# Bismarrck/tensoralloy

Measured on AMD Instinct MI355X. Metric: atom-steps/sec (energy+forces), 4000-atom Ni rcut=6.5 A, higher is better.
Workload: dtype f64

## Files before the change

include/tensoralloy_amd.h:

```cpp
#ifndef TENSORALLOY_AMD_H
#define TENSORALLOY_AMD_H

#include <stddef.h>
#include <stdint.h>

#ifdef __cplusplus
extern "C" {
#endif

typedef struct ta_context *ta_handle;

enum {
  TA_OK = 0,
  TA_ERR_INVALID = -1,
  TA_ERR_UNSUPPORTED = -2,
  TA_ERR_HIP = -3,
  TA_ERR_NOMEM = -4
};

enum {
  TA_WANT_ENERGY = 1,
  TA_WANT_FORCES = 2,
  TA_WANT_VIRIAL = 4,
  TA_WANT_ATOMIC = 8,
// ... 18 lines not shown
  int32_t angular;
  int32_t cutoff_function;

  int32_t n_eta, n_omega, n_beta, n_gamma, n_zeta;
  const double *eta, *omega, *beta, *gamma, *zeta;

  int32_t activation;
  int32_t use_resnet_dt;
  int32_t minmax_scale;
  const int32_t *n_layers;
  const int32_t *layer_sizes;
  const double *weights;
  const double *xlo, *xhi;

  int32_t n_eam_params;
  const double *eam_params;

  double eps;

  int32_t n_grap_params;
  const double *grap_params;

  int32_t n_eam_nets;

  const int32_t *eam_table_n;
  const double *eam_table_dx;
  const double *eam_table_coef;

  int32_t safe_pow;

  int32_t finite_temperature;
} ta_model_desc;

enum { TA_TD_ON = 1, TA_TD_SOMMERFELD = 2, TA_TD_ACT_SHIFT = 8 };

typedef struct {
  int32_t n_atoms;
  const int32_t *species;
  const double *positions;
  const double *cell;
  const int32_t *pbc;
} ta_frame;

typedef struct {
  int32_t n_frames;
  int64_t n_atoms;
  int64_t n_pairs;
  int64_t n_triples;
  int32_t nnl_max;
  int32_t descriptor_dim;
  int32_t nl_on_device;
  int32_t reserved_;
  double nl_ms;
  double set_frames_ms;
} ta_batch_info;

#define TA_N_KERNEL_SLOTS 10
enum {
  TA_K_PAIR_GEOMETRY = 0, TA_K_G4_FORWARD = 1, TA_K_DESCRIPTOR_REDUCE = 2,
  TA_K_MLP = 3, TA_K_BACKWARD = 4, TA_K_FORCE_GATHER = 5, TA_K_FRAME_REDUCE = 6,
  TA_K_EAM = 7,
  TA_K_NEIGHBOR_UPDATE = 8,
  TA_K_GRAP = 9
};

int ta_device_count(void);

#define TA_ABI_VERSION 5
int ta_abi_version(void);
int ta_model_desc_size(void);

int ta_create(const ta_model_desc *model, int device, ta_handle *out);
int ta_destroy(ta_handle h);
const char *ta_last_error(ta_handle h);

int ta_set_frames(ta_handle h, int32_t n_frames, const ta_frame *frames,
                  ta_batch_info *info);

int ta_set_skin(ta_handle h, double skin);
int ta_update_positions(ta_handle h, const double *positions, const double *cells, int32_t *rebuilt);
int ta_list_stats(ta_handle h, int64_t *n_builds, int64_t *n_reuses);
int ta_list_sizes(ta_handle h, int64_t *n_pairs, int64_t *n_triples, int32_t *nnl_max);

int ta_compute(ta_handle h, uint32_t want);

int ta_get_results(ta_handle h, double *energy, double *forces, double *virial,
                   double *atomic, double *descriptors);

int ta_set_electron_temperatures(ta_handle h, int32_t n_frames, const double *T);
int ta_get_td_results(ta_handle h, double *energy, double *eentropy, double *energy_atomic,
                      double *eentropy_atomic);

int ta_eval(ta_handle h, int32_t n_frames, const ta_frame *frames, uint32_t want,
            double *energy, double *forces, double *virial, double *atomic);

int ta_step(ta_handle h, const double *positions, const double *cells, uint32_t want, double *energy,
            double *forces, double *virial, double *atomic, int32_t *rebuilt);

int ta_view_results(ta_handle h, uint32_t want, const double **energy, const double **forces,
                    const double **virial, const double **atomic);
int ta_step_view(ta_handle h, const double *positions, const double *cells, uint32_t want, const double **energy,
                 const double **forces, const double **virial, const double **atomic, int32_t *rebuilt);

int ta_set_stream(ta_handle h, void *stream);

int ta_synchronize(ta_handle h);

int ta_batch_energy_device_ptr(ta_handle h, void **dptr);

int ta_copy_batch_energy(ta_handle h, void *dst_device);
int ta_set_batch_energy_target(ta_handle h, void *dst_device);

int ta_neighbor_list(const ta_frame *frame, int32_t n_elements, double rc, int64_t *n_pairs,
                     int32_t **i, int32_t **j, int32_t **shift , int32_t **rev);
void ta_free(void *p);


int ta_param_count(ta_handle h, int64_t *n_params);

int ta_update_weights(ta_handle h, const double *weights, int64_t n_weights);

int ta_energy_gradient(ta_handle h, const double *frame_coeff, double *grad, int64_t n_grad);

int ta_loss_gradient(ta_handle h, const double *frame_coeff, const double *dR, const double *dh,
                     double *grad, int64_t n_grad, double *dG_out);

int ta_td_loss_gradient(ta_handle h, const double *coeff_free_energy, const double *coeff_energy,
                        const double *coeff_eentropy, const double *dR, const double *dh, double *grad,
                        int64_t n_grad, double *dG_out);

int ta_constant_count(ta_handle h, int64_t *n_constants);
int ta_get_constants(ta_handle h, double *constants, int64_t n_constants);
int ta_update_constants(ta_handle h, const double *constants, int64_t n_constants);
int ta_constant_gradient(ta_handle h, const double *frame_coeff, const double *dR, const double *dh,
                         double *grad, int64_t n_grad);

int ta_hessian_vectors(ta_handle h, int32_t n_dir, int32_t first, const double *dR, const double *dh, double *dF,
                       double *dW);

int ta_set_nn_tables(ta_handle h, int on);

int ta_eam_tabulate(ta_handle h, int32_t n_r, const double *r, int32_t n_rho, const double *rho,
                    double *rho_of_r, double *phi_of_r, double *embed_of_rho, double *u_of_r,
                    double *w_of_r);


int ta_time_compute(ta_handle h, uint32_t want, int32_t warmup, int32_t steps,
                    double *total_ms, double *kernel_ms );

int ta_measure_hbm_copy(ta_handle h, int64_t bytes, int32_t reps, double *gbs);

int ta_count_contributing_triples(ta_handle h, int64_t *n_contributing);

int ta_get_pairs(ta_handle h, int32_t *i, int32_t *j, int32_t *shift );

#ifdef __cplusplus
}
#endif
#endif
```

tensoralloy_amd/_lib.py:

```python
from __future__ import annotations

import ctypes as C
import os
import subprocess
from pathlib import Path

import numpy as np

PKG_DIR = Path(__file__).resolve().parent
REPO_DIR = PKG_DIR.parent
CSRC_DIR = PKG_DIR / "csrc"
INCLUDE_DIR = REPO_DIR / "include"
LIB_PATH = PKG_DIR / "libtensoralloy_amd.so"

SOURCES = ["ta_api.hip", "ta_kernels.hip", "ta_kernels_v2.hip", "ta_mlp.hip", "ta_eam.hip",
           "ta_nlist.hip", "ta_grap.hip", "ta_train.hip", "ta_hvp.hip", "ta_neighbor.cpp", "ta_td.hip",
           "ta_td_train.hip"]
OBJ_DIR = CSRC_DIR / "build"

TA_OK = 0
TA_ERR_INVALID, TA_ERR_UNSUPPORTED, TA_ERR_HIP, TA_ERR_NOMEM = -1, -2, -3, -4
TA_WANT_ENERGY, TA_WANT_FORCES, TA_WANT_VIRIAL, TA_WANT_ATOMIC, TA_WANT_DESCRIPTORS = 1, 2, 4, 8, 16
TA_WANT_REUSE_DESCRIPTORS = 32
TA_MODEL_SF_MLP, TA_MODEL_EAM_ALLOY, TA_MODEL_EAM_ADP, TA_MODEL_GRAP_MLP, TA_MODEL_EAM_FS = 1, 2, 3, 4, 5
TA_CUTOFF = {"cosine": 0, "polynomial": 1}
TA_ACT = {"relu": 0, "softplus": 1, "tanh": 2, "squareplus": 3, "leaky_relu": 4,
          "sigmoid": 5, "softsign": 6, "elu": 7}
TA_N_KERNEL_SLOTS = 10
TA_TD_ON, TA_TD_SOMMERFELD, TA_TD_ACT_SHIFT = 1, 2, 8
TA_ABI_VERSION = 5
KERNEL_SLOTS = ["pair_geometry", "g4_forward", "descriptor_reduce", "mlp", "backward",
                "force_gather", "frame_reduce", "eam", "neighbor_update", "grap_forward"]

EXPORTED_SYMBOLS = [
    "ta_device_count", "ta_create", "ta_destroy", "ta_last_error", "ta_set_frames",
    "ta_compute", "ta_get_results", "ta_eval", "ta_set_stream", "ta_synchronize", "ta_time_compute",
    "ta_batch_energy_device_ptr", "ta_copy_batch_energy", "ta_get_pairs", "ta_neighbor_list", "ta_free",
    "ta_eam_tabulate", "ta_set_batch_energy_target", "ta_param_count", "ta_update_weights",
    "ta_energy_gradient", "ta_measure_hbm_copy", "ta_set_skin", "ta_update_positions", "ta_list_stats",
    "ta_count_contributing_triples", "ta_loss_gradient", "ta_constant_count", "ta_get_constants", "ta_update_constants",
    "ta_constant_gradient", "ta_list_sizes", "ta_abi_version", "ta_model_desc_size", "ta_set_nn_tables", "ta_step", "ta_hessian_vectors", "ta_view_results", "ta_step_view",
    "ta_set_electron_temperatures", "ta_get_td_results", "ta_td_loss_gradient",
]

_dp = C.POINTER(C.c_double)
_ip = C.POINTER(C.c_int32)


class ModelDesc(C.Structure):
    _fields_ = [
        ("kind", C.c_int32), ("n_elements", C.c_int32),
        ("rcut", C.c_double), ("acut", C.c_double),
        ("angular", C.c_int32), ("cutoff_function", C.c_int32),
        ("n_eta", C.c_int32), ("n_omega", C.c_int32), ("n_beta", C.c_int32),
        ("n_gamma", C.c_int32), ("n_zeta", C.c_int32),
        ("eta", _dp), ("omega", _dp), ("beta", _dp), ("gamma", _dp), ("zeta", _dp),
        ("activation", C.c_int32), ("use_resnet_dt", C.c_int32), ("minmax_scale", C.c_int32),
        ("n_layers", _ip), ("layer_sizes", _ip), ("weights", _dp),
        ("xlo", _dp), ("xhi", _dp),
        ("n_eam_params", C.c_int32), ("eam_params", _dp),
        ("eps", C.c_double),
        ("n_grap_params", C.c_int32), ("grap_params", _dp),
        ("n_eam_nets", C.c_int32),
        ("eam_table_n", _ip), ("eam_table_dx", _dp), ("eam_table_coef", _dp),
        ("safe_pow", C.c_int32),
        ("finite_temperature", C.c_int32),
    ]


class Frame(C.Structure):
    _fields_ = [("n_atoms", C.c_int32), ("species", _ip), ("positions", _dp),
                ("cell", _dp), ("pbc", _ip)]


class BatchInfo(C.Structure):
    _fields_ = [("n_frames", C.c_int32), ("n_atoms", C.c_int64), ("n_pairs", C.c_int64),
                ("n_triples", C.c_int64), ("nnl_max", C.c_int32), ("descriptor_dim", C.c_int32),
                ("nl_on_device", C.c_int32), ("reserved_", C.c_int32),
                ("nl_ms", C.c_double), ("set_frames_ms", C.c_double)]


def hipcc_path() -> str:
    for cand in (os.environ.get("HIPCC"), "/opt/rocm/bin/hipcc", "hipcc"):
        if cand and (os.path.isabs(cand) and os.path.exists(cand) or not os.path.isabs(cand)):
            return cand
    return "hipcc"


def _compile_flags():
    return ["--offload-arch=gfx950", "-O3", "-std=c++17", "-fPIC", "-pthread", f"-I{INCLUDE_DIR}",
            f"-I{CSRC_DIR}"] + os.environ.get("TA_EXTRA_HIPCC_FLAGS", "").split()


def build(force: bool = False, verbose: bool = False) -> Path:
    srcs = [CSRC_DIR / s for s in SOURCES]
    headers = list(CSRC_DIR.glob("*.h")) + [INCLUDE_DIR / "tensoralloy_amd.h"]
    deps = srcs + headers
    stamp = OBJ_DIR / "flags.txt"
    flags_same = stamp.exists() and stamp.read_text() == " ".join(_compile_flags())
    if not force and flags_same and LIB_PATH.exists():
        newest = max(p.stat().st_mtime for p in deps)
        if LIB_PATH.stat().st_mtime >= newest:
            return LIB_PATH
    import fcntl
    from concurrent.futures import ThreadPoolExecutor
    lock_path = str(LIB_PATH) + ".lock"
    with open(lock_path, "w") as lock:
        fcntl.flock(lock, fcntl.LOCK_EX)
        try:
            OBJ_DIR.mkdir(exist_ok=True)
            flags = _compile_flags()
            flags_same = stamp.exists() and stamp.read_text() == " ".join(flags)
            if not force and flags_same and LIB_PATH.exists() and \
                    LIB_PATH.stat().st_mtime >= max(p.stat().st_mtime for p in deps):
                return LIB_PATH
            if not flags_same:
                force = True
            hdr_time = max(p.stat().st_mtime for p in headers)

            def compile_one(src):
                obj = OBJ_DIR / (src.stem + ".o")
                if not force and obj.exists() and obj.stat().st_mtime >= max(src.stat().st_mtime, hdr_time):
                    return obj
                cmd = [hipcc_path()] + flags + ["-c", str(src), "-o", str(obj)]
                if verbose:
                    print(" ".join(cmd))
                subprocess.run(cmd, check=True)
                return obj

            try:
                jobs = max(1, min(len(srcs), len(os.sched_getaffinity(0))))
            except AttributeError:
                jobs = 4
            with ThreadPoolExecutor(max_workers=jobs) as pool:
                objs = list(pool.map(compile_one, srcs))
            stamp.write_text(" ".join(flags))
            tmp = str(LIB_PATH) + f".tmp{os.getpid()}"
            cmd = [hipcc_path(), "--offload-arch=gfx950", "-shared", "-fPIC", "-pthread"] + \
                  [str(o) for o in objs] + ["-o", tmp]
            if verbose:
                print(" ".join(cmd))
            subprocess.run(cmd, check=True)
            os.replace(tmp, LIB_PATH)
        finally:
            fcntl.flock(lock, fcntl.LOCK_UN)
    return LIB_PATH


_lib = None


def load():
    global _lib
    if _lib is not None:
        return _lib
    if not LIB_PATH.exists():
        raise ImportError(
            f"{LIB_PATH} is missing: build it with `python -c 'import __graft_entry__ as g; "
            f"g.build()'` (hipcc --offload-arch=gfx950). There is no CPU fallback.")
    path = os.environ.get("TA_LIB_AB") or str(LIB_PATH)
    if path != str(LIB_PATH):
        import sys
        sys.stderr.write(f"tensoralloy_amd: TA_LIB_AB is set, loading {path} instead of {LIB_PATH}\n")
    lib = C.CDLL(path)
    try:
        lib.ta_abi_version.restype = C.c_int
        version, desc_size = lib.ta_abi_version(), lib.ta_model_desc_size()
    except AttributeError:
        version, desc_size = -1, -1
    if version != TA_ABI_VERSION or desc_size != C.sizeof(ModelDesc):
        raise ImportError(f"{path}: ABI version {version} / ta_model_desc of {desc_size} bytes, this binding "
                          f"is version {TA_ABI_VERSION} / {C.sizeof(ModelDesc)} bytes: rebuild the library")
    H = C.c_void_p
    lib.ta_device_count.restype = C.c_int
    lib.ta_create.argtypes = [C.POINTER(ModelDesc), C.c_int, C.POINTER(H)]
    lib.ta_destroy.argtypes = [H]
    lib.ta_last_error.argtypes = [H]
    lib.ta_last_error.restype = C.c_char_p
    lib.ta_set_frames.argtypes = [H, C.c_int32, C.POINTER(Frame), C.POINTER(BatchInfo)]
    lib.ta_compute.argtypes = [H, C.c_uint32]
    lib.ta_get_results.argtypes = [H, _dp, _dp, _dp, _dp, _dp]
    lib.ta_eval.argtypes = [H, C.c_int32, C.POINTER(Frame), C.c_uint32, _dp, _dp, _dp, _dp]
    lib.ta_synchronize.argtypes = [H]
    lib.ta_set_stream.argtypes = [H, C.c_void_p]
    lib.ta_time_compute.argtypes = [H, C.c_uint32, C.c_int32, C.c_int32, _dp, _dp]
    lib.ta_measure_hbm_copy.argtypes = [H, C.c_int64, C.c_int32, _dp]
    lib.ta_batch_energy_device_ptr.argtypes = [H, C.POINTER(C.c_void_p)]
    lib.ta_copy_batch_energy.argtypes = [H, C.c_void_p]
    lib.ta_set_batch_energy_target.argtypes = [H, C.c_void_p]
    lib.ta_param_count.argtypes = [H, C.POINTER(C.c_int64)]
    lib.ta_update_weights.argtypes = [H, _dp, C.c_int64]
    lib.ta_energy_gradient.argtypes = [H, _dp, _dp, C.c_int64]
    lib.ta_loss_gradient.argtypes = [H, _dp, _dp, _dp, _dp, C.c_int64, _dp]
    lib.ta_td_loss_gradient.argtypes = [H, _dp, _dp, _dp, _dp, _dp, _dp, C.c_int64, _dp]
    lib.ta_constant_count.argtypes = [H, C.POINTER(C.c_int64)]
    lib.ta_get_constants.argtypes = [H, _dp, C.c_int64]
    lib.ta_update_constants.argtypes = [H, _dp, C.c_int64]
    lib.ta_constant_gradient.argtypes = [H, _dp, _dp, _dp, _dp, C.c_int64]
    lib.ta_get_pairs.argtypes = [H, _ip, _ip, _ip]
    lib.ta_neighbor_list.argtypes = [C.POINTER(Frame), C.c_int32, C.c_double,
                                     C.POINTER(C.c_int64), C.POINTER(_ip), C.POINTER(_ip),
                                     C.POINTER(_ip), C.POINTER(_ip)]
    lib.ta_count_contributing_triples.argtypes = [H, C.POINTER(C.c_int64)]
    lib.ta_set_skin.argtypes = [H, C.c_double]
    lib.ta_update_positions.argtypes = [H, _dp, _dp, _ip]
    lib.ta_list_stats.argtypes = [H, C.POINTER(C.c_int64), C.POINTER(C.c_int64)]
    lib.ta_list_sizes.argtypes = [H, C.POINTER(C.c_int64), C.POINTER(C.c_int64), C.POINTER(C.c_int32)]
    lib.ta_set_nn_tables.argtypes = [H, C.c_int]
    lib.ta_hessian_vectors.argtypes = [H, C.c_int32, C.c_int32, _dp, _dp, _dp, _dp]
    lib.ta_step.argtypes = [H, _dp, _dp, C.c_uint32, _dp, _dp, _dp, _dp, _ip]
    _dpp = C.POINTER(_dp)
    lib.ta_view_results.argtypes = [H, C.c_uint32, _dpp, _dpp, _dpp, _dpp]
    lib.ta_step_view.argtypes = [H, _dp, _dp, C.c_uint32, _dpp, _dpp, _dpp, _dpp, _ip]
    lib.ta_free.argtypes = [C.c_void_p]
    lib.ta_eam_tabulate.argtypes = [H, C.c_int32, _dp, C.c_int32, _dp, _dp, _dp, _dp, _dp, _dp]
    lib.ta_free.restype = None
    lib.ta_set_electron_temperatures.argtypes = [H, C.c_int32, _dp]
    lib.ta_get_td_results.argtypes = [H, _dp, _dp, _dp, _dp]
    _lib = lib
    return lib


def check(lib, handle, rc):
    if rc == TA_OK:
        return
    msg = lib.ta_last_error(handle)
    msg = msg.decode("utf-8", "replace") if msg else f"error {rc}"
    if rc in (TA_ERR_INVALID, TA_ERR_UNSUPPORTED):
        raise ValueError(msg)
    if rc == TA_ERR_NOMEM:
        raise MemoryError(msg)
    raise RuntimeError(msg)


def as_dp(a: np.ndarray):
    return a.ctypes.data_as(_dp)


def as_ip(a: np.ndarray):
    return a.ctypes.data_as(_ip)


class FrameArrays:

    def __init__(self, species, positions, cell, pbc):
        self.species = np.ascontiguousarray(species, dtype=np.int32)
        self.positions = np.ascontiguousarray(positions, dtype=np.float64).reshape(-1, 3)
        self.cell = np.ascontiguousarray(cell, dtype=np.float64).reshape(3, 3)
        self.pbc = np.ascontiguousarray(np.asarray(pbc).astype(bool), dtype=np.int32).reshape(3)
        if len(self.species) != len(self.positions):
            raise ValueError("species and positions disagree on the number of atoms")

    def as_struct(self) -> Frame:
        return Frame(len(self.species), as_ip(self.species), as_dp(self.positions),
                     as_dp(self.cell), as_ip(self.pbc))


def neighbor_list(species, positions, cell, pbc, n_elements, rc):
    lib = load()
    fa = FrameArrays(species, positions, cell, pbc)
    fr = fa.as_struct()
    n = C.c_int64(0)
    pi, pj, ps, pr = _ip(), _ip(), _ip(), _ip()
    rc_ = lib.ta_neighbor_list(C.byref(fr), n_elements, float(rc), C.byref(n), C.byref(pi),
                               C.byref(pj), C.byref(ps), C.byref(pr))
    check(lib, None, rc_)
    P = n.value
    try:
        i = np.ctypeslib.as_array(pi, shape=(max(P, 1),))[:P].copy()
        j = np.ctypeslib.as_array(pj, shape=(max(P, 1),))[:P].copy()
        s = np.ctypeslib.as_array(ps, shape=(max(3 * P, 1),))[:3 * P].copy().reshape(-1, 3)
        r = np.ctypeslib.as_array(pr, shape=(max(P, 1),))[:P].copy()
    finally:
        for p in (pi, pj, ps, pr):
            lib.ta_free(p)
    return i, j, s, r
```

tensoralloy_amd/csrc/ta_api.hip:

```cpp
#include <hip/hip_runtime.h>

#include <algorithm>
#include <chrono>
#include <climits>
#include <cmath>
#include <cstdio>
#include <cstdlib>
#include <cstring>
#include <stdexcept>
#include <string>
#include <vector>

#include "ta_device.h"
#include "ta_internal.h"

namespace ta {
size_t mlp_scratch_doubles(const MlpDev &mlp);
void launch_mlp_impl(const MlpDev &mlp, int activation, int ndim, const int32_t *atoms, int n_atoms,
                     const DeviceBatch &b, double *scratch, hipStream_t s);
size_t mlp_all_scratch_doubles(const MlpDev *mlps_host, int nel, const int32_t *elem_start);
size_t td_scratch_doubles(const MlpDev *nets, int nel, int K, const int32_t *elem_start);
void launch_td_all(const MlpDev *nets_dev, const MlpDev *nets_host, int nel, int K, int act_h, int act,
                   int sommerfeld, int ndim, const DeviceBatch &b, const double *T, double *u_atom,
                   double *s_atom, double *scratch, hipStream_t s);
// ... 63 lines not shown
                           const double *dh, double *grad, hipStream_t s);
void eam_energy_gradient(EamModel *, const DeviceBatch &b, const double *frame_coeff, double *grad,
                         hipStream_t s);
bool eam_loss_gradient_supported(const EamModel *);
void eam_loss_gradient(EamModel *, const DeviceBatch &b, const double *frame_coeff, const double *dR,
                       const double *dh, double *grad, hipStream_t s);
}

namespace {

thread_local std::string g_create_error;

struct HipError : std::runtime_error {
  using std::runtime_error::runtime_error;
};

#define HIP_CHECK(expr)                                                                      \
  do {                                                                                       \
    hipError_t _e = (expr);                                                                  \
    if (_e != hipSuccess)                                                                    \
      throw HipError(std::string(#expr) + ": " + hipGetErrorString(_e) + " (" __FILE__ ":" + \
                     std::to_string(__LINE__) + ")");                                        \
  } while (0)

template <typename T>
struct DevBuf {
  T *ptr = nullptr;
  size_t cap = 0;
  void ensure(size_t n) {
    if (n <= cap) return;
    size_t want = n + n / 8 + 64;
    T *fresh = nullptr;
    hipError_t e = hipMalloc((void **)&fresh, want * sizeof(T));
    if (e != hipSuccess && ptr) {
      (void)hipGetLastError();
      HIP_CHECK(hipFree(ptr));
      ptr = nullptr;
      cap = 0;
      e = hipMalloc((void **)&fresh, want * sizeof(T));
    }
    if (e != hipSuccess) {
      (void)hipGetLastError();
      throw HipError(std::string("hipMalloc of ") + std::to_string(want * sizeof(T)) + " bytes: " +
                     hipGetErrorString(e));
    }
    if (ptr) HIP_CHECK(hipFree(ptr));
    ptr = fresh;
    cap = want;
  }
  void release() {
    if (ptr) (void)hipFree(ptr);
    ptr = nullptr;
    cap = 0;
  }
};

__global__ __launch_bounds__(256) void staged_copy_kernel(double *__restrict__ dst,
                                                          const double *__restrict__ src, size_t n) {
  for (size_t k = (size_t)blockIdx.x * 256 + threadIdx.x; k < n; k += (size_t)gridDim.x * 256) dst[k] = src[k];
}
constexpr size_t kStagedCopyMaxBytes = 4u << 20;

void staged_copy(double *dst, const double *src, size_t n, bool to_host, hipStream_t s) {
  if (n == 0) return;
  static const bool use_dma = std::getenv("TA_STAGED_COPY_DMA") != nullptr;
  if (n * sizeof(double) > kStagedCopyMaxBytes || use_dma) {
    HIP_CHECK(hipMemcpyAsync(dst, src, n * sizeof(double), to_host ? hipMemcpyDeviceToHost : hipMemcpyHostToDevice, s));
    return;
  }
  const unsigned blocks = (unsigned)std::min<size_t>((n + 255) / 256, 256);
  hipLaunchKernelGGL(staged_copy_kernel, dim3(blocks), dim3(256), 0, s, dst, src, n);
  HIP_CHECK(hipGetLastError());
}

void wait_stream(hipStream_t s) {
  static const bool blocking = std::getenv("TA_SYNC_BLOCKING") && std::getenv("TA_SYNC_BLOCKING")[0] == '1';
  if (!blocking) {
    const auto t0 = std::chrono::steady_clock::now();
    for (;;) {
      const hipError_t e = hipStreamQuery(s);
      if (e == hipSuccess) return;
      if (e != hipErrorNotReady) {
        (void)hipGetLastError();
        break;
      }
      if (std::chrono::steady_clock::now() - t0 > std::chrono::microseconds(400)) break;
    }
  }
  HIP_CHECK(hipStreamSynchronize(s));
}

struct PinnedBuf {
  char *ptr = nullptr;
  size_t cap = 0;
  void ensure(size_t n) {
    if (n <= cap) return;
    if (ptr) HIP_CHECK(hipHostFree(ptr));
    ptr = nullptr;
    cap = 0;
    size_t want = n + n / 8 + 256;
    HIP_CHECK(hipHostMalloc((void **)&ptr, want, hipHostMallocDefault));
    cap = want;
  }
  void release() {
    if (ptr) (void)hipHostFree(ptr);
    ptr = nullptr;
    cap = 0;
  }
};

struct ChunkPlan {
  ta::AngChunk ch;
  int nb, ng, nz;
};

}

struct ta_context {
  int device = 0;
  hipStream_t stream = nullptr;
  hipStream_t own_stream = nullptr;
  int kind = 0;
  int n_elements = 0;
  int activation = 0;
  double rmax = 0.0;
  ta::SFParams sf;
  std::vector<ChunkPlan> chunks;
  std::vector<ChunkPlan> chunks_v2;
  bool use_v2 = false;
  ta::MlpDev *mlp_dev = nullptr;
  ta::MlpDev mlp[ta::kMaxElements];
  bool td = false, td_sommerfeld = false;
  int td_act = 0, td_K = 0;
  ta::MlpDev td_nets[3 * ta::kMaxElements];
  ta::MlpDev *td_dev = nullptr;
  std::vector<void *> model_allocs;
  ta::EamModel *eam = nullptr;
  ta::GrapModel *grap = nullptr;

  ta::HostPairs hp;
  ta::DeviceBatch db;
  bool have_batch = false;
  uint32_t last_want = 0;

  PinnedBuf stage_in, stage_out;
  DevBuf<char> inbuf;
  DevBuf<double> results;
  size_t o_blk = 0;
  DevBuf<double> rec, part4, G, dEdG, g, wat, bpart, fown, benergy, mlp_scratch;
  DevBuf<double> td_T, td_u, td_s;
  DevBuf<unsigned long long> masks;
  DevBuf<uint32_t> job_word;
  DevBuf<int32_t> job_count;
  DevBuf<int32_t> pair_start, seg_start, pair_i, pair_j, pair_shift, pair_rev;
  ta::NlGrid *d_grids = nullptr;
  DevBuf<int32_t> nl_wrap, nl_binid, nl_bin_count, nl_bin_start, nl_bin_cursor, nl_bin_atoms, nl_counts;
  DevBuf<unsigned long long> nl_stats, nl_zero;
  unsigned long long *nl_stats_ptr = nullptr;
  bool nl_sorted = false;
  bool nl_rev_done = false;
  bool nl_zero_clean = false;
  int64_t nl_zero_atoms = -1;
  int nl_zero_bins = -1;
  DevBuf<double> hvp_buf;
#ifdef TA_PHASE_STAMPS
  DevBuf<unsigned long long> stamp_buf;
#endif
  DevBuf<ta::NlRec> nl_recs;
  bool pairs_on_device = false;
  bool descriptors_valid = false;
  DevBuf<double> train_scratch, train_partial, train_grad, train_coeff;
  DevBuf<double> jvp_J, tan_dD, tan_dG, tan_dir;
  bool jvp_valid = false;

  double skin = 0.0;
  double r_list = 0.0;
  std::vector<int32_t> keep_species;
  std::vector<int32_t> keep_natoms, keep_pbc;
  std::vector<double> ref_pos, ref_cells;
  size_t o_pos = 0, o_cells = 0, o_species = 0;
  DevBuf<int32_t> ex_pair_i, ex_pair_j, ex_pair_shift, ex_pair_rev, ex_pair_start, ex_pair_stop, ex_seg_start, ex_counts,
      ex_map, ex_blk, ex_slot_q;
  bool filtered = false;
  bool upload_pending = false;
  bool mirror_next = false;
  uint32_t mirror_want = 0;
  int64_t n_list_builds = 0, n_list_reuses = 0;

  hipEvent_t ev[2 * TA_N_KERNEL_SLOTS + 2] = {nullptr};
  std::string err;
};

namespace {

int fail(ta_context *h, int code, const std::string &msg) {
  if (h)
    h->err = msg;
  else
    g_create_error = msg;
  return code;
}

std::string td_inference_only(const char *fn) {
  return std::string(fn) + ": not available for finite-temperature (temperature-dependent) models "
         "(no analytic Hessian-vector products)";
}

std::string fs_inference_only(const char *fn) {
  return std::string(fn) + ": not available for eam/fs models (inference only: no weight, constant or loss "
         "gradients and no analytic Hessian-vector products; differences of the forces give the latter)";
}

template <typename T>
T *upload(ta_context *h, const std::vector<T> &v) {
  T *d = nullptr;
  size_t n = v.size() ? v.size() : 1;
  HIP_CHECK(hipMalloc((void **)&d, n * sizeof(T)));
  h->model_allocs.push_back(d);
  if (!v.empty()) HIP_CHECK(hipMemcpy(d, v.data(), v.size() * sizeof(T), hipMemcpyHostToDevice));
  return d;
}

int round_up(int x, int m) { return (x + m - 1) / m * m; }

void hd_series(int cutoff, double beta, ta::AngChunk &ch) {
  ch.n_hd = 0;
  for (double &c : ch.hd) c = 0.0;
  if (cutoff != TA_CUTOFF_COSINE || !(beta >= 0.0)) return;
  constexpr int NT = 64;
  const long double pi2 = 9.869604401089358618834490999876151135L;
  long double fc[NT], ex[NT], prod[NT];
  long double t = 1.0L;
  for (int k = 0; k < NT; ++k) {
    fc[k] = 0.5L * t + (k == 0 ? 0.5L : 0.0L);
    t *= -pi2 / (long double)((2 * k + 1) * (2 * k + 2));
  }
  t = 1.0L;
  for (int k = 0; k < NT; ++k) {
    ex[k] = t;
    t *= -(long double)beta / (long double)(k + 1);
  }
  for (int k = 0; k < NT; ++k) {
    long double acc = 0.0L;
    for (int j = 0; j <= k; ++j) acc += fc[j] * ex[k - j];
    prod[k] = acc;
  }
  constexpr int N0 = 40;
  static long double tstar[N0][N0];
  static bool have_t = false;
  if (!have_t) {
    for (auto &row : tstar)
      for (auto &c : row) c = 0.0L;
    tstar[0][0] = 1.0L;
    tstar[1][0] = -1.0L;
    tstar[1][1] = 2.0L;
    for (int n = 1; n + 1 < N0; ++n)
      for (int k = 0; k <= n + 1; ++k)
        tstar[n + 1][k] = (k > 0 ? 4.0L * tstar[n][k - 1] : 0.0L) - 2.0L * tstar[n][k] - tstar[n - 1][k];
    have_t = true;
  }
  long double tail0 = 0.0L, dtail0 = 0.0L;
  for (int k = N0; k < NT; ++k) {
    tail0 += fabsl(prod[k]);
    dtail0 += (long double)k * fabsl(prod[k]);
  }
  for (int n : {12, 16, 24}) {
    long double a[N0];
    for (int k = 0; k < N0; ++k) a[k] = prod[k];
    long double err = tail0, derr = dtail0;
    for (int d = N0 - 1; d >= n; --d) {
      const long double q = a[d] / tstar[d][d];
      for (int k = 0; k <= d; ++k) a[k] -= q * tstar[d][k];
      err += fabsl(q);
      derr += 2.0L * (long double)d * (long double)d * fabsl(q);
    }
    if (err < 1e-17L && derr < 1e-15L) {
      ch.n_hd = n;
      for (int k = 0; k < n; ++k) ch.hd[k] = (double)a[k];
      return;
    }
  }
}

void build_mlp(ta_context *h, const ta_model_desc *m, int ndim);

void build_sf_model(ta_context *h, const ta_model_desc *m) {
  using namespace ta;
  SFParams &sf = h->sf;
  std::memset(&sf, 0, sizeof(sf));
  const int nel = m->n_elements;
  if (m->n_eta < 1 || m->n_omega < 1 || !m->eta || !m->omega)
    throw std::invalid_argument("eta / omega must be non-empty");
  if (m->n_eta * m->n_omega > kMaxRadial)
    throw std::domain_error("more than 64 radial (eta x omega) combinations");
  if (!(m->rcut > 0.0)) throw std::invalid_argument("rcut must be positive");
  sf.rcut = m->rcut;
  sf.acut = m->angular ? m->acut : m->rcut;
  if (m->angular && !(m->acut > 0.0)) throw std::invalid_argument("acut must be positive");
  sf.inv_rc2 = 1.0 / (sf.rcut * sf.rcut);
  sf.inv_ac2 = 1.0 / (sf.acut * sf.acut);
  sf.two_inv_ac2 = 2.0 * sf.inv_ac2;
  sf.eps = m->eps > 0.0 ? m->eps : 1e-14;
  sf.n_elements = nel;
  sf.n_rad = m->n_eta * m->n_omega;
  sf.angular = m->angular ? 1 : 0;
  sf.cutoff = m->cutoff_function;
// ... 259 lines not shown
  if (!two_pass_only) {
    {
      const unsigned long long *before = h->nl_zero.ptr;
      h->nl_zero.ensure(nl_build_zero_words((int)N, n_bins));
      if (h->nl_zero.ptr != before || h->nl_zero_atoms != (int64_t)N || h->nl_zero_bins != n_bins) h->nl_zero_clean = false;
      h->nl_zero_atoms = (int64_t)N;
      h->nl_zero_bins = n_bins;
    }
    h->nl_rev_done = false;
    for (int attempt = 0; attempt < 2 && !h->nl_sorted; ++attempt) {
      const size_t capacity = std::min(std::min(h->pair_i.cap, h->pair_j.cap), h->pair_shift.cap / 3);
      h->pair_rev.ensure(capacity);
      const size_t guess = (hp.n_atoms == (int64_t)N && hp.n_pairs > 0) ? (size_t)hp.n_pairs + (size_t)hp.n_pairs / 4 + 4096
                                                                         : capacity;
      const size_t rev_cover = std::min(std::min(capacity, guess), (size_t)INT32_MAX);
      NlWork w = nl_work(h);
      nl_build((int)N, n_bins, nel, h->r_list, h->db.pos, h->db.species, h->db.frame_of_atom, h->d_grids, w,
               h->nl_zero.ptr, h->nl_zero_clean, (long long)std::min<size_t>(capacity, (size_t)INT32_MAX), h->pair_start.ptr,
               kernel_writes_host ? starts : nullptr, h->pair_i.ptr, h->pair_j.ptr, h->pair_shift.ptr,
               h->pair_rev.ptr, (long long)rev_cover, s);
      HIP_CHECK(hipGetLastError());
      h->nl_zero_clean = false;
      if (!kernel_writes_host)
        staged_copy(reinterpret_cast<double *>(starts), reinterpret_cast<const double *>(h->pair_start.ptr),
                    (N + 2) / 2, true, s);
      staged_copy(reinterpret_cast<double *>(stats), reinterpret_cast<const double *>(h->nl_zero.ptr), 8, true, s);
      wait_stream(s);
      h->nl_zero_clean = N > 0;
      if (si[3] != 0) break;
      if (stats[4] > (unsigned long long)INT32_MAX) throw std::runtime_error("batch too large for 32-bit pair indices");
      if (stats[4] <= capacity) {
        h->nl_sorted = true;
        h->nl_rev_done = stats[4] <= rev_cover;
        if (h->nl_rev_done && si[6] != 0)
          throw std::runtime_error("neighbour list is not symmetric (reverse pair missing)");
      } else {
        h->pair_i.ensure((size_t)stats[4]);
        h->pair_j.ensure((size_t)stats[4]);
        h->pair_shift.ensure(3 * (size_t)stats[4]);
      }
    }
    if (h->nl_sorted) h->nl_stats_ptr = h->nl_zero.ptr;
  }
  if (!h->nl_sorted) {
    h->nl_bin_count.ensure((size_t)n_bins + 1);
    h->nl_bin_cursor.ensure((size_t)n_bins + 1);
    h->nl_counts.ensure(N * (nel + 1) + 1);
    h->nl_stats.ensure(8);
    NlWork w = nl_work(h);
    nl_count((int)N, n_bins, nel, h->r_list, h->db.pos, h->db.species, h->db.frame_of_atom, h->d_grids, w,
             h->pair_start.ptr, s);
    HIP_CHECK(hipGetLastError());
    HIP_CHECK(hipMemcpyAsync(stats, h->nl_stats.ptr, 8 * sizeof(unsigned long long), hipMemcpyDeviceToHost, s));
    HIP_CHECK(hipMemcpyAsync(starts, h->pair_start.ptr, (N + 1) * sizeof(int32_t), hipMemcpyDeviceToHost, s));
    HIP_CHECK(hipStreamSynchronize(s));
    if (stats[4] > (unsigned long long)INT32_MAX || si[4] < 0 || (unsigned long long)si[4] != stats[4])
      throw std::runtime_error("batch too large for 32-bit pair indices");
    h->nl_stats_ptr = h->nl_stats.ptr;
  }
  hp.n_atoms = (int64_t)N;
  hp.n_pairs = (int64_t)stats[4];
  hp.n_triples = (int64_t)stats[0];
  hp.nnl_max = si[2];
  hp.pair_start.assign(starts, starts + N + 1);
  hp.seg_start.clear();
  hp.pair_i.clear();
  hp.pair_j.clear();
  hp.pair_shift.clear();
  hp.pair_rev.clear();
  h->pairs_on_device = true;
}

void fill_pairs_on_device(ta_context *h) {
  using namespace ta;
  if (h->nl_sorted) {
    nl_reverse_sorted(h->hp.n_pairs, h->n_elements, h->db.species, h->seg_start.ptr, h->pair_i.ptr,
                      h->pair_j.ptr, h->pair_shift.ptr, h->pair_rev.ptr, h->nl_stats_ptr, h->stream);
  } else {
    NlWork w = nl_work(h);
    nl_fill((int)h->hp.n_atoms, h->hp.n_pairs, h->n_elements, h->r_list, h->db.pos, h->db.species,
            h->db.frame_of_atom, h->d_grids, w, h->pair_i.ptr, h->pair_j.ptr, h->pair_shift.ptr,
            h->pair_rev.ptr, h->stream);
  }
  HIP_CHECK(hipGetLastError());
}

#ifdef TA_PHASE_STAMPS
static void dump_stamps(ta_context *h) {
  const char *path = std::getenv("TA_PHASE_STAMPS_OUT");
  if (!path || !h->db.stamps || h->db.n_blk <= 0) return;
  const size_t n = (size_t)2 * h->db.n_blk * 8;
  std::vector<unsigned long long> v(n);
  (void)hipStreamSynchronize(h->stream);
  (void)hipMemcpy(v.data(), h->db.stamps, n * sizeof(unsigned long long), hipMemcpyDeviceToHost);
  FILE *fp = std::fopen(path, "w");
  if (!fp) return;
  for (int k = 0; k < 2; ++k)
    for (int b = 0; b < h->db.n_blk; ++b) {
      std::fprintf(fp, "%d %d", k, b);
      for (int q = 0; q < 8; ++q) std::fprintf(fp, " %llu", v[((size_t)k * h->db.n_blk + b) * 8 + q]);
      std::fprintf(fp, "\n");
    }
  std::fclose(fp);
}
#endif

void launch_head(ta_context *h, const ta::DeviceBatch &db, hipStream_t s) {
  if (h->td)
    ta::launch_td_all(h->td_dev, h->td_nets, h->n_elements, h->td_K, h->td_act, h->activation,
                      h->td_sommerfeld ? 1 : 0, h->sf.ndim, db, h->td_T.ptr, h->td_u.ptr, h->td_s.ptr,
                      h->mlp_scratch.ptr, s);
  else
    ta::launch_mlp_all(h->mlp_dev, h->mlp, h->n_elements, h->activation, h->sf.ndim, db, h->mlp_scratch.ptr, s);
}

void compute_impl(ta_context *h, uint32_t want, bool timed, double *slot_ms) {
  using namespace ta;
#ifdef TA_PHASE_STAMPS
  if (h->db.n_blk > 0) {
    h->stamp_buf.ensure((size_t)2 * h->db.n_blk * 8 + 8);
    h->db.stamps = h->stamp_buf.ptr;
    (void)hipMemsetAsync(h->db.stamps, 0, (size_t)2 * h->db.n_blk * 8 * sizeof(unsigned long long), h->stream);
  }
#endif
  h->db.rec4 = nullptr;
  h->db.own_sums = 0;
  const DeviceBatch &db = h->db;
  hipStream_t s = h->stream;
  const bool need_forces = (want & (TA_WANT_FORCES | TA_WANT_VIRIAL)) != 0;
  auto begin = [&](int slot) {
    if (timed) HIP_CHECK(hipEventRecord(h->ev[2 * slot], s));
  };
  auto end = [&](int slot) {
    if (timed) HIP_CHECK(hipEventRecord(h->ev[2 * slot + 1], s));
  };
  bool used[TA_N_KERNEL_SLOTS] = {false};

  const bool has_mlp = h->kind == TA_MODEL_SF_MLP || h->kind == TA_MODEL_GRAP_MLP;
  if ((want & TA_WANT_REUSE_DESCRIPTORS) && has_mlp && h->descriptors_valid && !need_forces) {
    begin(TA_K_MLP);
    launch_head(h, db, s);
    end(TA_K_MLP);
    used[TA_K_MLP] = true;
  } else if (h->kind == TA_MODEL_SF_MLP) {
    static const bool full_records = getenv("TA_FULL_RECORDS") != nullptr;
    h->db.rec4 = (h->sf.angular && h->use_v2 && !full_records) ? h->db.rec : nullptr;
    if (!h->use_v2) {
      begin(TA_K_PAIR_GEOMETRY);
      launch_pair_geometry(h->sf, db, s);
      end(TA_K_PAIR_GEOMETRY);
      used[TA_K_PAIR_GEOMETRY] = true;
    }
    h->sf.ang_scale = h->use_v2 ? 1.0 : 0.5;
    const bool reduce_in_forward = h->sf.angular && h->use_v2;
    if (h->sf.angular) {
      begin(TA_K_G4_FORWARD);
      if (h->use_v2) {
        bool geometry = true;
        size_t left = h->chunks_v2.size();
        for (const ChunkPlan &cp : h->chunks_v2) {
          --left;
          launch_g4_forward_v2(h->sf, cp.ch, cp.ng, cp.nz, geometry, left == 0, db, s);
          geometry = false;
        }
      } else
        for (const ChunkPlan &cp : h->chunks) launch_g4_forward(h->sf, cp.ch, cp.nb, cp.ng, cp.nz, db, s);
      end(TA_K_G4_FORWARD);
      used[TA_K_G4_FORWARD] = true;
    }
    if (!reduce_in_forward) {
      begin(TA_K_DESCRIPTOR_REDUCE);
      launch_descriptor_reduce(h->sf, db, s);
      end(TA_K_DESCRIPTOR_REDUCE);
      used[TA_K_DESCRIPTOR_REDUCE] = true;
    }
    begin(TA_K_MLP);
    launch_head(h, db, s);
    end(TA_K_MLP);
    used[TA_K_MLP] = true;
    if (need_forces) {
      begin(TA_K_BACKWARD);
      if (h->sf.angular) {
        bool first = true;
        if (h->use_v2)
          for (const ChunkPlan &cp : h->chunks_v2) {
            launch_backward_v2(h->sf, cp.ch, cp.ng, cp.nz, first, db, s);
            first = false;
          }
        else
          for (const ChunkPlan &cp : h->chunks) {
            launch_backward(h->sf, cp.ch, cp.nb, cp.ng, cp.nz, first, false, db, s);
            first = false;
          }
      } else {
        AngChunk dummy;
        std::memset(&dummy, 0, sizeof(dummy));
        launch_backward(h->sf, dummy, 1, 1, 1, true, true, db, s);
      }
      end(TA_K_BACKWARD);
      used[TA_K_BACKWARD] = true;
      begin(TA_K_FORCE_GATHER);
      launch_force_gather(h->sf, db, s);
      end(TA_K_FORCE_GATHER);
      used[TA_K_FORCE_GATHER] = true;
    }
  } else if (h->kind == TA_MODEL_GRAP_MLP) {
    h->db.rec4 = (!ta::grap_uses_filter_net(h->grap) && !getenv("TA_FULL_RECORDS")) ? h->db.rec : nullptr;
    begin(TA_K_GRAP);
    launch_grap_forward(h->grap, db, h->sf.eps, s);
    end(TA_K_GRAP);
    used[TA_K_GRAP] = true;
    begin(TA_K_MLP);
    launch_head(h, db, s);
    end(TA_K_MLP);
    used[TA_K_MLP] = true;
    if (need_forces) {
      begin(TA_K_BACKWARD);
      h->db.own_sums = getenv("TA_NO_OWN_SUMS") ? 0 : 1;
      launch_grap_backward(h->grap, db, s);
      end(TA_K_BACKWARD);
      used[TA_K_BACKWARD] = true;
      begin(TA_K_FORCE_GATHER);
      launch_force_gather(h->sf, db, s);
      end(TA_K_FORCE_GATHER);
      used[TA_K_FORCE_GATHER] = true;
    }
  } else {
    h->db.rec4 = getenv("TA_FULL_RECORDS") ? nullptr : h->db.rec;
    begin(TA_K_EAM);
    eam_compute(h->eam, db, want, s, nullptr);
    end(TA_K_EAM);
    used[TA_K_EAM] = true;
  }
  begin(TA_K_FRAME_REDUCE);
  {
    double *mirror = nullptr;
    int64_t n_tail = 0;
    h->mirror_want = 0;
    if (h->mirror_next && !timed) {
      const size_t N = (size_t)db.n_atoms, F = (size_t)db.n_frames;
      h->stage_out.ensure((10 * F + 4 * N + 2) * sizeof(double));
      mirror = reinterpret_cast<double *>(h->stage_out.ptr);
      n_tail = (int64_t)(need_forces ? 4 * N : N);
      h->mirror_want = want | TA_WANT_ENERGY | TA_WANT_ATOMIC;
    }
    launch_frame_reduce(db, need_forces, mirror, n_tail, s);
  }
  end(TA_K_FRAME_REDUCE);
  used[TA_K_FRAME_REDUCE] = true;
  HIP_CHECK(hipGetLastError());
  h->last_want = want;
  h->descriptors_valid = true;

  if (timed) {
    HIP_CHECK(hipStreamSynchronize(s));
    for (int k = 0; k < TA_N_KERNEL_SLOTS; ++k) {
      if (!used[k]) continue;
      float ms = 0.f;
      HIP_CHECK(hipEventElapsedTime(&ms, h->ev[2 * k], h->ev[2 * k + 1]));
      slot_ms[k] += ms;
    }
  }
}

template <typename F>
int guarded(ta_context *h, F &&fn) {
  try {
    if (h) HIP_CHECK(hipSetDevice(h->device));
    fn();
    return TA_OK;
  } catch (const HipError &e) {
    return fail(h, TA_ERR_HIP, e.what());
  } catch (const std::domain_error &e) {
    return fail(h, TA_ERR_UNSUPPORTED, e.what());
  } catch (const std::invalid_argument &e) {
    return fail(h, TA_ERR_INVALID, e.what());
  } catch (const std::bad_alloc &) {
    return fail(h, TA_ERR_NOMEM, "host allocation failed");
  } catch (const std::exception &e) {
    return fail(h, TA_ERR_INVALID, e.what());
  }
}

}

extern "C" {

int ta_abi_version(void) { return TA_ABI_VERSION; }
int ta_model_desc_size(void) { return (int)sizeof(ta_model_desc); }

int ta_device_count(void) {
  int n = 0;
  if (hipGetDeviceCount(&n) != hipSuccess) return 0;
  return n;
}

const char *ta_last_error(ta_handle h) { return h ? h->err.c_str() : g_create_error.c_str(); }

int ta_create(const ta_model_desc *model, int device, ta_handle *out) {
  if (!model || !out) return fail(nullptr, TA_ERR_INVALID, "null argument");
  *out = nullptr;
  int ndev = 0;
  if (hipGetDeviceCount(&ndev) != hipSuccess || ndev <= 0)
    return fail(nullptr, TA_ERR_HIP, "no HIP device available: this library has no CPU fallback");
  if (device < 0 || device >= ndev) return fail(nullptr, TA_ERR_INVALID, "device index out of range");
  if (model->n_elements < 1 || model->n_elements > ta::kMaxElements)
    return fail(nullptr, TA_ERR_UNSUPPORTED, "n_elements must be in 1..8");
  ta_context *h = new ta_context();
  h->device = device;
  h->kind = model->kind;
  h->n_elements = model->n_elements;
  int rc = guarded(h, [&]() {
    hipDeviceProp_t prop;
    HIP_CHECK(hipGetDeviceProperties(&prop, device));
    if (std::strncmp(prop.gcnArchName, "gfx950", 6) != 0)
      throw HipError(std::string("device is ") + prop.gcnArchName +
                     ", this library is built for gfx950 only");
    HIP_CHECK(hipStreamCreateWithFlags(&h->own_stream, hipStreamNonBlocking));
    h->stream = h->own_stream;
    for (auto &e : h->ev) HIP_CHECK(hipEventCreate(&e));
    if (model->kind == TA_MODEL_SF_MLP) {
      build_sf_model(h, model);
    } else if (model->kind == TA_MODEL_GRAP_MLP) {
      if (model->cutoff_function != TA_CUTOFF_COSINE && model->cutoff_function != TA_CUTOFF_POLYNOMIAL)
        throw std::invalid_argument("unknown cutoff function");
      std::string err;
      h->grap = ta::grap_create(model, err);
      if (!h->grap) throw std::invalid_argument(err);
      h->rmax = model->rcut;
      std::memset(&h->sf, 0, sizeof(h->sf));
      h->sf.n_elements = model->n_elements;
      h->sf.eps = model->eps > 0.0 ? model->eps : 1e-14;
      h->sf.ndim = ta::grap_ndim(h->grap);
      build_mlp(h, model, h->sf.ndim);
    } else if (model->kind == TA_MODEL_EAM_ALLOY || model->kind == TA_MODEL_EAM_ADP || model->kind == TA_MODEL_EAM_FS) {
      std::string err;
      h->eam = ta::eam_create(model, err);
      if (!h->eam) throw std::invalid_argument(err);
      h->rmax = model->rcut;
      std::memset(&h->sf, 0, sizeof(h->sf));
      h->sf.n_elements = model->n_elements;
      h->sf.eps = model->eps > 0.0 ? model->eps : 1e-14;
    } else {
      throw std::invalid_argument("unknown model kind");
    }
  });
  if (rc != TA_OK) {
    g_create_error = h->err;
    ta_destroy(h);
    return rc;
  }
  *out = h;
  return TA_OK;
}

int ta_destroy(ta_handle h) {
  if (!h) return TA_OK;
  (void)hipSetDevice(h->device);
#ifdef TA_PHASE_STAMPS
  dump_stamps(h);
#endif
  if (h->stream) (void)hipStreamSynchronize(h->stream);
  for (void *p : h->model_allocs) (void)hipFree(p);
  if (h->eam) ta::eam_destroy(h->eam);
  if (h->grap) ta::grap_destroy(h->grap);
  h->stage_in.release(); h->stage_out.release(); h->inbuf.release(); h->results.release();
  h->rec.release(); h->part4.release(); h->G.release();
  h->dEdG.release(); h->g.release(); h->wat.release(); h->bpart.release(); h->fown.release();
  h->benergy.release(); h->mlp_scratch.release();
  h->train_scratch.release(); h->train_partial.release(); h->train_grad.release(); h->train_coeff.release();
  h->jvp_J.release(); h->tan_dD.release(); h->tan_dG.release(); h->tan_dir.release();
  h->pair_start.release(); h->seg_start.release(); h->pair_i.release(); h->pair_j.release();
  h->pair_shift.release(); h->pair_rev.release();
  for (auto *b : {&h->ex_pair_i, &h->ex_pair_j, &h->ex_pair_shift, &h->ex_pair_rev, &h->ex_pair_start, &h->ex_pair_stop,
                  &h->ex_seg_start, &h->ex_counts, &h->ex_map, &h->ex_blk, &h->ex_slot_q})
    b->release();
  h->masks.release(); h->job_word.release(); h->job_count.release();
  for (auto *b : {&h->nl_wrap, &h->nl_binid, &h->nl_bin_count, &h->nl_bin_start, &h->nl_bin_cursor,
                  &h->nl_bin_atoms, &h->nl_counts})
    b->release();
  h->nl_stats.release();
  h->nl_zero.release();
  h->hvp_buf.release();
  h->nl_recs.release();
  for (auto &e : h->ev)
    if (e) (void)hipEventDestroy(e);
  if (h->own_stream) (void)hipStreamDestroy(h->own_stream);
  delete h;
  return TA_OK;
}

}

namespace {
void ensure_job_lists(ta_context *h, size_t n_blk) {
  static const bool off = std::getenv("TA_NO_JOBS") != nullptr;
  if (off || !h->use_v2 || n_blk == 0) {
    h->db.job_count = nullptr;
    return;
  }
  const int stride = ta::v2_job_stride(h->db.cap);
  h->job_word.ensure(n_blk * (size_t)stride + 8);
  h->job_count.ensure(n_blk + 8);
  h->db.job_word = h->job_word.ptr;
  h->db.job_count = h->job_count.ptr;
  h->db.job_stride = stride;
}

bool filter_applies(const ta_context *h) {
  if (!(h->skin > 0.0) || h->hp.n_atoms == 0 || std::getenv("TA_NO_LIST_FILTER")) return false;
  if (h->kind == TA_MODEL_SF_MLP) return h->use_v2;
  if (h->kind == TA_MODEL_EAM_ALLOY || h->kind == TA_MODEL_EAM_FS) return ta::eam_is_plain(h->eam);
  return false;
}

void apply_filter(ta_context *h) {
  using namespace ta;
  const size_t N = (size_t)h->hp.n_atoms, P = (size_t)h->hp.n_pairs;
  const int nel = h->n_elements;
  h->ex_pair_i.ensure(P + 1);
  h->ex_pair_j.ensure(P + 1);
  h->ex_pair_shift.ensure(3 * P + 3);
  h->ex_pair_rev.ensure(P + 1);
  h->ex_pair_start.ensure(N + 1);
  h->ex_pair_stop.ensure(N + 1);
  h->ex_seg_start.ensure(N * (nel + 1) + 1);
  h->ex_map.ensure(P + 1);
  const int n_run_slots = nl_filter_blocks((int)N);
  h->ex_blk.ensure((size_t)n_run_slots + 4);
  const bool blocks = h->kind == TA_MODEL_SF_MLP;
  const bool indirect = blocks && !std::getenv("TA_FILTER_REV_KERNEL");
  if (indirect) h->ex_slot_q.ensure(P + 1);
  nl_filter((int)N, (int64_t)P, nel, h->rmax, h->db.pos, h->db.cells, h->db.frame_of_atom,
            h->pair_start.ptr, h->seg_start.ptr, h->pair_j.ptr, h->pair_shift.ptr, h->pair_rev.ptr, h->ex_map.ptr,
            h->ex_seg_start.ptr, h->ex_pair_start.ptr, h->ex_pair_stop.ptr, h->ex_pair_i.ptr, h->ex_pair_j.ptr,
            h->ex_pair_shift.ptr, h->ex_pair_rev.ptr, indirect ? h->ex_slot_q.ptr : nullptr, h->db.cap,
            blocks ? h->ex_blk.ptr : nullptr, h->stream);
  h->db.slot_q = indirect ? h->ex_slot_q.ptr : nullptr;
  h->db.rev_super = indirect ? h->pair_rev.ptr : nullptr;
  h->db.rev_map = indirect ? h->ex_map.ptr : nullptr;
  HIP_CHECK(hipGetLastError());
  h->db.pair_start = h->ex_pair_start.ptr;
  h->db.pair_stop = h->ex_pair_stop.ptr;
  h->db.seg_start = h->ex_seg_start.ptr;
  h->db.pair_i = h->ex_pair_i.ptr;
  h->db.pair_j = h->ex_pair_j.ptr;
  h->db.pair_shift = h->ex_pair_shift.ptr;
  h->db.pair_rev = h->ex_pair_rev.ptr;
  if (blocks) {
    h->db.blk_center = h->ex_blk.ptr;
    h->db.n_blk = n_run_slots;
    h->db.blk_groups = n_run_slots / 16;
    h->db.n_blk_dev = nullptr;
    ensure_job_lists(h, (size_t)n_run_slots);
  }
  h->filtered = true;
}

void set_frames_impl(ta_context *h, int32_t n_frames, const ta_frame *frames, ta_batch_info *info) {
  for (int f = 0; f < n_frames; ++f) {
    const ta_frame &fr = frames[f];
    if (fr.n_atoms < 0 || (fr.n_atoms > 0 && (!fr.species || !fr.positions)) || !fr.cell || !fr.pbc)
      throw std::invalid_argument("frame " + std::to_string(f) + ": null array");
  }
  const auto t_begin = std::chrono::steady_clock::now();
  if (h->upload_pending) {
    HIP_CHECK(hipStreamSynchronize(h->stream));
    h->upload_pending = false;
  }
  h->have_batch = false;
  h->descriptors_valid = false;
  h->jvp_valid = false;
  h->mirror_want = 0;
  h->filtered = false;
  h->db.slot_q = h->db.rev_super = h->db.rev_map = nullptr;
  h->db.pair_stop = nullptr;
  h->db.blk_groups = 0;
  h->db.n_blk_dev = nullptr;
  h->r_list = h->rmax + h->skin;
  size_t N = 0;
  for (int f = 0; f < n_frames; ++f) N += (size_t)frames[f].n_atoms;
  if (N >= (1u << 30)) throw std::runtime_error("batch too large for 32-bit atom indices");
  const size_t F = (size_t)n_frames;
  const int nel = h->n_elements;
  auto align16 = [](size_t x) { return (x + 15) & ~(size_t)15; };
  const size_t o_pos = 0;
  const size_t o_cells = align16(o_pos + 3 * N * sizeof(double));
  const size_t o_grids = align16(o_cells + 9 * F * sizeof(double));
  const size_t o_species = align16(o_grids + F * sizeof(ta::NlGrid));
  const size_t o_foa = align16(o_species + N * sizeof(int32_t));
  const size_t o_astart = align16(o_foa + N * sizeof(int32_t));
  const size_t o_elem = align16(o_astart + (F + 1) * sizeof(int32_t));
  const size_t o_blk = align16(o_elem + N * sizeof(int32_t));
  const size_t total = align16(o_blk + (N + 2) * sizeof(int32_t));
  h->stage_in.ensure(total);
  h->inbuf.ensure(total);
  char *hb = h->stage_in.ptr;
  double *pos = reinterpret_cast<double *>(hb + o_pos);
  double *cells = reinterpret_cast<double *>(hb + o_cells);
  ta::NlGrid *grids = reinterpret_cast<ta::NlGrid *>(hb + o_grids);
  int32_t *species = reinterpret_cast<int32_t *>(hb + o_species);
  int32_t *foa = reinterpret_cast<int32_t *>(hb + o_foa);
  int32_t *astart = reinterpret_cast<int32_t *>(hb + o_astart);
  int32_t *elem_atoms = reinterpret_cast<int32_t *>(hb + o_elem);
  size_t a = 0;
  astart[0] = 0;
  for (int f = 0; f < n_frames; ++f) {
    const ta_frame &fr = frames[f];
    const size_t n = (size_t)fr.n_atoms;
    if (n) {
      std::memcpy(&pos[3 * a], fr.positions, 3 * n * sizeof(double));
      std::memcpy(&species[a], fr.species, n * sizeof(int32_t));
    }
    std::memcpy(&cells[9 * (size_t)f], fr.cell, 9 * sizeof(double));
    for (size_t i = a; i < a + n; ++i) {
      foa[i] = f;
      if (species[i] < 0 || species[i] >= nel)
        throw std::runtime_error("frame " + std::to_string(f) + ": species index out of range");
      if (!std::isfinite(pos[3 * i]) || !std::isfinite(pos[3 * i + 1]) || !std::isfinite(pos[3 * i + 2]))
        throw std::runtime_error("frame " + std::to_string(f) + ": non-finite position");
    }
    a += n;
    astart[f + 1] = (int32_t)a;
  }
  {
    std::vector<int32_t> count(nel + 1, 0);
    for (size_t i = 0; i < N; ++i) count[species[i] + 1]++;
    for (int e = 0; e < nel; ++e) count[e + 1] += count[e];
    for (int e = 0; e <= nel; ++e) h->db.elem_start[e] = count[e];
    std::vector<int32_t> fill(count.begin(), count.end() - 1);
    for (size_t i = 0; i < N; ++i) elem_atoms[fill[species[i]]++] = (int32_t)i;
  }
  const auto t_nl = std::chrono::steady_clock::now();
  int n_bins = 0;
  bool device_nl = N > 0 && !(std::getenv("TA_HOST_NL") && std::getenv("TA_HOST_NL")[0] == '1');
  for (int f = 0; f < n_frames && device_nl; ++f) {
    device_nl = ta::nl_make_grid(frames[f], h->r_list, n_bins, grids[f]);
    if (device_nl) n_bins += ta::nl_bins(grids[f]);
    if (n_bins > (1 << 24)) device_nl = false;
  }
  if (!device_nl) std::memset(static_cast<void *>(grids), 0, F * sizeof(ta::NlGrid));
  if (o_blk)
    staged_copy(reinterpret_cast<double *>(h->inbuf.ptr), reinterpret_cast<const double *>(hb), o_blk / sizeof(double),
                false, h->stream);
  char *db_ = h->inbuf.ptr;
  h->db.n_frames = n_frames;
  h->db.pos = reinterpret_cast<double *>(db_ + o_pos);
  h->db.cells = reinterpret_cast<double *>(db_ + o_cells);
  h->d_grids = reinterpret_cast<ta::NlGrid *>(db_ + o_grids);
  h->db.species = reinterpret_cast<int32_t *>(db_ + o_species);
  h->db.frame_of_atom = reinterpret_cast<int32_t *>(db_ + o_foa);
  h->db.atom_start = reinterpret_cast<int32_t *>(db_ + o_astart);
  h->db.elem_atoms = reinterpret_cast<int32_t *>(db_ + o_elem);
  h->db.blk_center = reinterpret_cast<int32_t *>(db_ + o_blk);
  if (device_nl) {
    h->hp.atom_start.assign(astart, astart + F + 1);
    h->hp.frame_of_atom.assign(foa, foa + N);
    build_pairs_on_device(h, N, n_bins);
  } else {
    h->pairs_on_device = false;
    ta::build_pairs(n_frames, frames, nel, h->r_list, h->hp);
  }
  double nl_ms = std::chrono::duration<double, std::milli>(std::chrono::steady_clock::now() - t_nl).count();
  upload_batch(h);
  const auto t_fill = std::chrono::steady_clock::now();
  const bool list_done = h->pairs_on_device && h->nl_sorted && h->nl_rev_done;
  if (h->pairs_on_device && !list_done) {
    fill_pairs_on_device(h);
    staged_copy(reinterpret_cast<double *>(h->stage_out.ptr), reinterpret_cast<const double *>(h->nl_stats_ptr),
                8, true, h->stream);
  }
  bool shapes_ok = h->n_elements <= 3;
  if (h->n_elements == 4 || h->n_elements == 5) {
    shapes_ok = !h->chunks_v2.empty();
    for (const ChunkPlan &cp : h->chunks_v2) shapes_ok = shapes_ok && cp.ng == 2 && cp.nz == 2;
  }
  h->use_v2 = h->kind == TA_MODEL_SF_MLP && h->sf.angular && shapes_ok &&
              h->hp.nnl_max <= ta::kCapMax && std::getenv("TA_FORCE_V1") == nullptr;
  const int cap = std::max(ta::kCapMin, (h->hp.nnl_max + 63) / 64 * 64);
  h->db.cap = cap;
  {
    int32_t *blk = reinterpret_cast<int32_t *>(hb + o_blk);
    int nb = 0;
    if (h->use_v2 && N) {
      blk[nb++] = 0;
      int32_t load = 0, ncent = 0;
      for (size_t i = 0; i < N; ++i) {
        const int32_t cnt = h->hp.pair_start[i + 1] - h->hp.pair_start[i];
        if (load + cnt > cap || ncent >= ta::kMaxCentersPerBlock) {
          blk[nb++] = (int32_t)i;
          load = 0;
          ncent = 0;
        }
        load += cnt;
        ++ncent;
      }
      blk[nb++] = (int32_t)N;
    }
    h->db.n_blk = nb ? nb - 1 : 0;
    ensure_job_lists(h, (size_t)h->db.n_blk);
    if (nb) {
      if (list_done)
        staged_copy(reinterpret_cast<double *>(db_ + o_blk), reinterpret_cast<const double *>(blk), ((size_t)nb + 1) / 2,
                    false, h->stream);
      else
        HIP_CHECK(hipMemcpyAsync(db_ + o_blk, blk, (size_t)nb * sizeof(int32_t), hipMemcpyHostToDevice, h->stream));
    }
  }
  if (h->kind == TA_MODEL_SF_MLP) {
    if (!h->use_v2 && ta::g4_lds_bytes(h->hp.nnl_max) > 160 * 1024 && h->sf.angular)
      throw std::domain_error("more than 1150 neighbours per atom exceed the LDS staging buffer");
    size_t need = ta::mlp_all_scratch_doubles(h->mlp, h->n_elements, h->db.elem_start);
    h->mlp_scratch.ensure(need);
  } else if (h->kind == TA_MODEL_GRAP_MLP) {
    h->mlp_scratch.ensure(ta::mlp_all_scratch_doubles(h->mlp, h->n_elements, h->db.elem_start));
    ta::grap_ensure(h->grap, h->db);
  } else {
    ta::eam_ensure(h->eam, h->db);
  }
  if (h->td) {
    const size_t N = (size_t)h->db.n_atoms;
    h->mlp_scratch.ensure(ta::td_scratch_doubles(h->td_nets, h->n_elements, h->td_K, h->db.elem_start));
    h->td_u.ensure(N + 1);
    h->td_s.ensure(N + 1);
    h->td_T.ensure((size_t)h->db.n_frames + 1);
  }
  h->o_pos = o_pos;
  h->o_cells = o_cells;
  h->o_species = o_species;
  h->ref_pos.assign(pos, pos + 3 * N);
  h->ref_cells.assign(cells, cells + 9 * F);
  h->keep_species.assign(species, species + N);
// ... 197 lines not shown
    hi = std::max(hi, off + n);
  };
  need(energy, 0, F);
  need(virial, F, 9 * F);
  need(atomic, 10 * F, N);
  need(forces, 10 * F + N, 3 * N);
  const double *stage = nullptr;
  const bool fv = (h->mirror_want & (TA_WANT_FORCES | TA_WANT_VIRIAL)) != 0;
  if (hi > lo && h->mirror_want && (!(forces || virial) || fv)) {
    stage = reinterpret_cast<const double *>(h->stage_out.ptr);
  } else if (hi > lo) {
    h->mirror_want = 0;
    h->stage_out.ensure((hi - lo) * sizeof(double));
    stage = reinterpret_cast<const double *>(h->stage_out.ptr) - lo;
    staged_copy(reinterpret_cast<double *>(h->stage_out.ptr), h->results.ptr + lo, hi - lo, true, s);
  }
  if (descriptors && N)
    HIP_CHECK(hipMemcpyAsync(descriptors, h->db.G, N * h->sf.ndim * sizeof(double), hipMemcpyDeviceToHost, s));
  wait_stream(s);
  h->upload_pending = false;
  return stage;
}
}

int ta_get_results(ta_handle h, double *energy, double *forces, double *virial, double *atomic,
                   double *descriptors) {
  if (!h) return TA_ERR_INVALID;
  if (!h->have_batch) return fail(h, TA_ERR_INVALID, "no resident batch");
  return guarded(h, [&]() {
    const size_t N = (size_t)h->db.n_atoms, F = (size_t)h->db.n_frames;
    const double *stage = results_to_stage(h, energy != nullptr, forces != nullptr, virial != nullptr,
                                           atomic != nullptr, descriptors);
    if (energy && F) std::memcpy(energy, stage, F * sizeof(double));
    if (virial && F) std::memcpy(virial, stage + F, 9 * F * sizeof(double));
    if (atomic && N) std::memcpy(atomic, stage + 10 * F, N * sizeof(double));
    if (forces && N) std::memcpy(forces, stage + 10 * F + N, 3 * N * sizeof(double));
  });
}

int ta_view_results(ta_handle h, uint32_t want, const double **energy, const double **forces,
                    const double **virial, const double **atomic) {
  if (!h) return TA_ERR_INVALID;
  if (!h->have_batch) return fail(h, TA_ERR_INVALID, "no resident batch");
  return guarded(h, [&]() {
    const size_t N = (size_t)h->db.n_atoms, F = (size_t)h->db.n_frames;
    const bool fv = (want & (TA_WANT_FORCES | TA_WANT_VIRIAL)) != 0;
    const double *stage = results_to_stage(h, energy != nullptr, forces && fv, virial && fv,
                                           atomic && (want & TA_WANT_ATOMIC), nullptr);
    if (energy) *energy = (stage && F) ? stage : nullptr;
    if (virial) *virial = (stage && fv && F) ? stage + F : nullptr;
    if (atomic) *atomic = (stage && (want & TA_WANT_ATOMIC) && N) ? stage + 10 * F : nullptr;
    if (forces) *forces = (stage && fv && N) ? stage + 10 * F + N : nullptr;
  });
}

int ta_step(ta_handle h, const double *positions, const double *cells, uint32_t want, double *energy,
            double *forces, double *virial, double *atomic, int32_t *rebuilt) {
  int rc = ta_update_positions(h, positions, cells, rebuilt);
  if (rc != TA_OK) return rc;
  h->mirror_next = true;
  rc = ta_compute(h, want);
  h->mirror_next = false;
  if (rc != TA_OK) return rc;
  return ta_get_results(h, energy, forces, virial, atomic, nullptr);
}

int ta_step_view(ta_handle h, const double *positions, const double *cells, uint32_t want, const double **energy,
                 const double **forces, const double **virial, const double **atomic, int32_t *rebuilt) {
  int rc = ta_update_positions(h, positions, cells, rebuilt);
  if (rc != TA_OK) return rc;
  h->mirror_next = true;
  rc = ta_compute(h, want);
  h->mirror_next = false;
  if (rc != TA_OK) return rc;
  return ta_view_results(h, want, energy, forces, virial, atomic);
}

int ta_eval(ta_handle h, int32_t n_frames, const ta_frame *frames, uint32_t want, double *energy,
            double *forces, double *virial, double *atomic) {
  int rc = ta_set_frames(h, n_frames, frames, nullptr);
  if (rc != TA_OK) return rc;
  rc = ta_compute(h, want);
  if (rc != TA_OK) return rc;
  return ta_get_results(h, energy, forces, virial, atomic, nullptr);
}

int ta_time_compute(ta_handle h, uint32_t want, int32_t warmup, int32_t steps, double *total_ms,
                    double *kernel_ms) {
  if (!h) return TA_ERR_INVALID;
  if (!h->have_batch) return fail(h, TA_ERR_INVALID, "no resident batch");
  if (steps < 1 || warmup < 0) return fail(h, TA_ERR_INVALID, "steps must be >= 1, warmup >= 0");
  return guarded(h, [&]() {
    hipStream_t s = h->stream;
    for (int k = 0; k < warmup; ++k) compute_impl(h, want, false, nullptr);
    HIP_CHECK(hipStreamSynchronize(s));
    hipEvent_t e0 = h->ev[2 * TA_N_KERNEL_SLOTS], e1 = h->ev[2 * TA_N_KERNEL_SLOTS + 1];
    HIP_CHECK(hipEventRecord(e0, s));
    for (int k = 0; k < steps; ++k) compute_impl(h, want, false, nullptr);
    HIP_CHECK(hipEventRecord(e1, s));
    HIP_CHECK(hipStreamSynchronize(s));
    float ms = 0.f;
    HIP_CHECK(hipEventElapsedTime(&ms, e0, e1));
    if (total_ms) *total_ms = ms;
    if (kernel_ms) {
      double acc[TA_N_KERNEL_SLOTS] = {0};
      for (int k = 0; k < steps; ++k) compute_impl(h, want, true, acc);
      for (int k = 0; k < TA_N_KERNEL_SLOTS; ++k) kernel_ms[k] = acc[k] / steps;
    }
  });
}

int ta_batch_energy_device_ptr(ta_handle h, void **dptr) {
  if (!h || !dptr) return TA_ERR_INVALID;
  if (!h->have_batch) return fail(h, TA_ERR_INVALID, "no resident batch");
  *dptr = h->db.batch_energy;
  return TA_OK;
}

namespace {
__global__ __launch_bounds__(256) void hbm_copy_kernel(const double2 *__restrict__ src,
                                                       double2 *__restrict__ dst, size_t n) {
  const size_t stride = (size_t)gridDim.x * blockDim.x;
  size_t k = (size_t)blockIdx.x * blockDim.x + threadIdx.x;
  for (; k + 3 * stride < n; k += 4 * stride) {
    const double2 a = src[k], b = src[k + stride], c = src[k + 2 * stride], d = src[k + 3 * stride];
    dst[k] = a;
    dst[k + stride] = b;
    dst[k + 2 * stride] = c;
    dst[k + 3 * stride] = d;
  }
  for (; k < n; k += stride) dst[k] = src[k];
}
__global__ __launch_bounds__(256) void hbm_copy_nt_kernel(const double2 *__restrict__ src,
                                                          double2 *__restrict__ dst, size_t n) {
  typedef double d2 __attribute__((ext_vector_type(2)));
  const d2 *s = reinterpret_cast<const d2 *>(src);
  d2 *d = reinterpret_cast<d2 *>(dst);
  const size_t stride = (size_t)gridDim.x * blockDim.x;
  size_t k = (size_t)blockIdx.x * blockDim.x + threadIdx.x;
  for (; k + 3 * stride < n; k += 4 * stride) {
    const d2 a = __builtin_nontemporal_load(s + k), b = __builtin_nontemporal_load(s + k + stride),
             c = __builtin_nontemporal_load(s + k + 2 * stride), e = __builtin_nontemporal_load(s + k + 3 * stride);
    __builtin_nontemporal_store(a, d + k);
    __builtin_nontemporal_store(b, d + k + stride);
    __builtin_nontemporal_store(c, d + k + 2 * stride);
    __builtin_nontemporal_store(e, d + k + 3 * stride);
  }
  for (; k < n; k += stride) d[k] = s[k];
}
}

namespace {
__global__ __launch_bounds__(256) void count_triples_kernel(ta::DeviceBatch b, double ac2, double eps,
                                                            unsigned long long *out) {
  const int64_t i = ((int64_t)blockIdx.x * 256 + threadIdx.x) >> 6;
  const int lane = threadIdx.x & 63;
  if (i >= b.n_atoms) return;
  const int p0 = b.pair_start[i], p1 = ta::pair_stop_of(b, i);
  unsigned long long n = 0;
  for (int pa = p0 + lane; pa < p1; pa += 64) {
    const double2 *ra = ta::pair_geom(b, (size_t)pa);
    const double ax = ra[0].x, ay = ra[0].y, az = ra[1].x;
    if (!(ra[1].y < ac2)) continue;
    for (int pb = pa + 1; pb < p1; ++pb) {
      const double2 *rb = ta::pair_geom(b, (size_t)pb);
      const double ex = rb[0].x - ax, ey = rb[0].y - ay, ez = rb[1].x - az;
      n += (rb[1].y < ac2 && ex * ex + ey * ey + ez * ez + eps < ac2) ? 1ull : 0ull;
    }
  }
  for (int off = 32; off; off >>= 1) n += __shfl_xor(n, off);
  if (lane == 0 && n) atomicAdd(out, n);
}
}

int ta_count_contributing_triples(ta_handle h, int64_t *n_contributing) {
  if (!h || !n_contributing) return fail(h, TA_ERR_INVALID, "null argument");
  if (!h->have_batch) return fail(h, TA_ERR_INVALID, "no resident batch");
  if (h->kind != TA_MODEL_SF_MLP || !h->sf.angular)
    return fail(h, TA_ERR_INVALID, "only symmetry-function models with angular terms have triples");
  return guarded(h, [&]() {
    compute_impl(h, TA_WANT_ENERGY, false, nullptr);
    h->nl_stats.ensure(8);
    hipStream_t s = h->stream;
    HIP_CHECK(hipMemsetAsync(h->nl_stats.ptr, 0, sizeof(unsigned long long), s));
    const int64_t N = h->db.n_atoms;
    if (N)
      hipLaunchKernelGGL(count_triples_kernel, dim3((unsigned)((N * 64 + 255) / 256)), dim3(256), 0, s, h->db,
                         h->sf.acut * h->sf.acut, h->sf.eps, h->nl_stats.ptr);
    HIP_CHECK(hipGetLastError());
    unsigned long long v = 0;
    HIP_CHECK(hipMemcpyAsync(&v, h->nl_stats.ptr, sizeof(v), hipMemcpyDeviceToHost, s));
    HIP_CHECK(hipStreamSynchronize(s));
    *n_contributing = (int64_t)v;
  });
}

int ta_measure_hbm_copy(ta_handle h, int64_t bytes, int32_t reps, double *gbs) {
  if (!h || !gbs || bytes < 16 || reps < 1) return fail(h, TA_ERR_INVALID, "bad argument");
  return guarded(h, [&]() {
    const size_t n = (size_t)bytes / 16;
    double2 *src = nullptr, *dst = nullptr;
    HIP_CHECK(hipMalloc((void **)&src, n * 16));
    if (hipMalloc((void **)&dst, n * 16) != hipSuccess) {
      (void)hipFree(src);
      throw std::bad_alloc();
    }
    hipStream_t s = h->stream;
    hipEvent_t e0, e1;
    HIP_CHECK(hipEventCreate(&e0));
    HIP_CHECK(hipEventCreate(&e1));
    HIP_CHECK(hipMemsetAsync(src, 0, n * 16, s));
    static const int per_cu = std::getenv("TA_COPY_WG_PER_CU") ? std::atoi(std::getenv("TA_COPY_WG_PER_CU")) : 8;
    const unsigned blocks = (unsigned)std::min<size_t>((n + 255) / 256, (size_t)256 * std::max(1, per_cu));
    static const int only = std::getenv("TA_COPY_MODE") ? std::atoi(std::getenv("TA_COPY_MODE")) : -1;
    double best = 0.0;
    for (int mode = 0; mode < 3; ++mode) {
      if (only >= 0 && mode != only) continue;
      auto one = [&]() {
        if (mode == 1) (void)hipMemcpyAsync(dst, src, n * 16, hipMemcpyDeviceToDevice, s);
        else if (mode == 2) hipLaunchKernelGGL(hbm_copy_nt_kernel, dim3(blocks), dim3(256), 0, s, src, dst, n);
        else hipLaunchKernelGGL(hbm_copy_kernel, dim3(blocks), dim3(256), 0, s, src, dst, n);
      };
      for (int k = 0; k < 2; ++k) one();
      HIP_CHECK(hipEventRecord(e0, s));
      for (int k = 0; k < reps; ++k) one();
      HIP_CHECK(hipEventRecord(e1, s));
      HIP_CHECK(hipEventSynchronize(e1));
      float ms = 0.f;
      HIP_CHECK(hipEventElapsedTime(&ms, e0, e1));
      if (ms > 0.f) best = std::max(best, 2.0 * (double)(n * 16) * reps / (ms * 1e-3) / 1e9);
    }
    (void)hipEventDestroy(e0);
    (void)hipEventDestroy(e1);
    (void)hipFree(src);
    (void)hipFree(dst);
    *gbs = best;
  });
}

int ta_set_stream(ta_handle h, void *stream) {
  if (!h) return TA_ERR_INVALID;
  return guarded(h, [&]() {
    HIP_CHECK(hipStreamSynchronize(h->stream));
    h->upload_pending = false;
    h->stream = stream ? (hipStream_t)stream : h->own_stream;
  });
}

int ta_copy_batch_energy(ta_handle h, void *dst_device) {
  if (!h || !dst_device) return TA_ERR_INVALID;
  if (!h->have_batch) return fail(h, TA_ERR_INVALID, "no resident batch");
  return guarded(h, [&]() {
    HIP_CHECK(hipMemcpyAsync(dst_device, h->db.batch_energy, sizeof(double),
                             hipMemcpyDeviceToDevice, h->stream));
  });
}

int ta_param_count(ta_handle h, int64_t *n_params) {
  if (!h || !n_params) return TA_ERR_INVALID;
  if (h->td) {
    *n_params = ta::td_param_count(h->td_nets, h->n_elements);
    return TA_OK;
  }
  if (h->eam) {
    *n_params = ta::eam_param_count(h->eam);
    return TA_OK;
  }
  if (h->kind != TA_MODEL_SF_MLP && h->kind != TA_MODEL_GRAP_MLP)
    return fail(h, TA_ERR_INVALID, "the model has no MLP");
  int64_t n = 0;
  for (int e = 0; e < h->n_elements; ++e) n += ta::mlp_param_count(h->mlp[e]);
  *n_params = n;
  return TA_OK;
}

namespace {
void upload_net_weights(ta::MlpDev &md, const double *&src) {
  for (int l = 0; l < md.n_layers; ++l) {
    ta::MlpLayerDev &ly = md.layer[l];
    std::vector<double> w((size_t)ly.kp * ly.np, 0.0), wt((size_t)ly.np * ly.kp, 0.0), bb(ly.np, 0.0);
    for (int k = 0; k < ly.k; ++k)
      for (int n = 0; n < ly.n; ++n) {
        const double v = src[(size_t)k * ly.n + n];
        w[(size_t)k * ly.np + n] = v;
        wt[(size_t)n * ly.kp + k] = v;
      }
    src += (size_t)ly.k * ly.n;
    for (int n = 0; n < ly.n; ++n) bb[n] = src[n];
    src += ly.n;
    HIP_CHECK(hipMemcpy(ly.w, w.data(), w.size() * sizeof(double), hipMemcpyHostToDevice));
    HIP_CHECK(hipMemcpy(ly.wt, wt.data(), wt.size() * sizeof(double), hipMemcpyHostToDevice));
    HIP_CHECK(hipMemcpy(ly.b, bb.data(), bb.size() * sizeof(double), hipMemcpyHostToDevice));
  }
}
}

int ta_update_weights(ta_handle h, const double *weights, int64_t n_weights) {
  if (!h || !weights) return TA_ERR_INVALID;
  if (h->td)
    return guarded(h, [&]() {
      const int64_t want = ta::td_param_count(h->td_nets, h->n_elements);
      if (n_weights != want)
        throw std::invalid_argument("ta_update_weights: expected " + std::to_string(want) + " values");
      HIP_CHECK(hipStreamSynchronize(h->stream));
      const double *src = weights;
      for (int j = 0; j < 3 * h->n_elements; ++j) upload_net_weights(h->td_nets[j], src);
    });
  if (h->eam)
    return guarded(h, [&]() {
      HIP_CHECK(hipStreamSynchronize(h->stream));
      ta::eam_update_weights(h->eam, weights, n_weights);
    });
  if (h->kind != TA_MODEL_SF_MLP && h->kind != TA_MODEL_GRAP_MLP)
    return fail(h, TA_ERR_INVALID, "the model has no MLP");
  return guarded(h, [&]() {
    int64_t want = 0;
    for (int e = 0; e < h->n_elements; ++e) want += ta::mlp_param_count(h->mlp[e]);
    if (n_weights != want)
      throw std::invalid_argument("ta_update_weights: expected " + std::to_string(want) + " values");
    HIP_CHECK(hipStreamSynchronize(h->stream));
    const double *src = weights;
    for (int e = 0; e < h->n_elements; ++e) upload_net_weights(h->mlp[e], src);
  });
}

int ta_energy_gradient(ta_handle h, const double *frame_coeff, double *grad, int64_t n_grad) {
  if (!h || !frame_coeff || !grad) return TA_ERR_INVALID;
  if (h->td)
    return ta_td_loss_gradient(h, frame_coeff, nullptr, nullptr, nullptr, nullptr, grad, n_grad, nullptr);
  if (h->kind == TA_MODEL_EAM_FS) return fail(h, TA_ERR_INVALID, fs_inference_only("ta_energy_gradient"));
  if (!h->have_batch) return fail(h, TA_ERR_INVALID, "no resident batch");
  if (h->eam)
    return guarded(h, [&]() {
      const int64_t total = ta::eam_param_count(h->eam);
      if (n_grad != total)
        throw std::invalid_argument("ta_energy_gradient: expected room for " + std::to_string(total) + " values");
      if (total == 0) return;
      if (h->filtered)
        throw std::domain_error("ta_energy_gradient: not available on a skin-filtered batch; "
                                "ta_set_skin(h, 0) and ta_set_frames first");
      if (ta::eam_nn_tables_on(h->eam)) HIP_CHECK(hipStreamSynchronize(h->stream));
      ta::eam_mark_trained(h->eam);
      ta::eam_ensure(h->eam, h->db);
      compute_impl(h, TA_WANT_ENERGY, false, nullptr);
      hipStream_t s = h->stream;
      const size_t F = (size_t)h->db.n_frames;
      h->train_grad.ensure((size_t)total + 8);
      h->train_coeff.ensure(F + 8);
      if (F) HIP_CHECK(hipMemcpyAsync(h->train_coeff.ptr, frame_coeff, F * sizeof(double), hipMemcpyHostToDevice, s));
      ta::eam_energy_gradient(h->eam, h->db, h->train_coeff.ptr, h->train_grad.ptr, s);
      HIP_CHECK(hipGetLastError());
      HIP_CHECK(hipMemcpyAsync(grad, h->train_grad.ptr, (size_t)total * sizeof(double), hipMemcpyDeviceToHost, s));
      HIP_CHECK(hipStreamSynchronize(s));
    });
  if (h->kind != TA_MODEL_SF_MLP && h->kind != TA_MODEL_GRAP_MLP)
    return fail(h, TA_ERR_INVALID, "the model has no MLP");
  return guarded(h, [&]() {
    int64_t total = 0;
    for (int e = 0; e < h->n_elements; ++e) total += ta::mlp_param_count(h->mlp[e]);
    if (n_grad != total)
      throw std::invalid_argument("ta_energy_gradient: expected room for " + std::to_string(total) + " values");
    if (!h->descriptors_valid) compute_impl(h, TA_WANT_ENERGY, false, nullptr);
    hipStream_t s = h->stream;
    const size_t F = (size_t)h->db.n_frames;
    size_t scratch = 0, partial = 0;
    for (int e = 0; e < h->n_elements; ++e) {
      const int n_el = h->db.elem_start[e + 1] - h->db.elem_start[e];
      scratch = std::max(scratch, ta::mlp_grad_scratch_doubles(h->mlp[e], n_el));
      partial = std::max(partial, ta::mlp_grad_partial_doubles(h->mlp[e], n_el));
    }
    h->train_scratch.ensure(scratch + 8);
    h->train_partial.ensure(partial + 8);
    h->train_grad.ensure((size_t)total + 8);
    h->train_coeff.ensure(F + 8);
    if (F) HIP_CHECK(hipMemcpyAsync(h->train_coeff.ptr, frame_coeff, F * sizeof(double), hipMemcpyHostToDevice, s));
    size_t off = 0;
    for (int e = 0; e < h->n_elements; ++e) {
      const int n_el = h->db.elem_start[e + 1] - h->db.elem_start[e];
      ta::launch_mlp_grad(h->mlp[e], h->activation, h->sf.ndim, h->db.elem_atoms + h->db.elem_start[e], n_el,
                          h->db, h->train_coeff.ptr, h->train_scratch.ptr, h->train_partial.ptr,
                          h->train_grad.ptr + off, s);
      off += (size_t)ta::mlp_param_count(h->mlp[e]);
    }
    HIP_CHECK(hipGetLastError());
    HIP_CHECK(hipMemcpyAsync(grad, h->train_grad.ptr, (size_t)total * sizeof(double), hipMemcpyDeviceToHost, s));
    HIP_CHECK(hipStreamSynchronize(s));
  });
}

namespace {
void backward_only(ta_context *h) {
  using namespace ta;
  const DeviceBatch &db = h->db;
  hipStream_t s = h->stream;
  if (h->kind == TA_MODEL_SF_MLP) {
    if (h->sf.angular) {
      bool first = true;
      if (h->use_v2)
        for (const ChunkPlan &cp : h->chunks_v2) {
          launch_backward_v2(h->sf, cp.ch, cp.ng, cp.nz, first, db, s);
          first = false;
        }
      else
        for (const ChunkPlan &cp : h->chunks) {
          launch_backward(h->sf, cp.ch, cp.nb, cp.ng, cp.nz, first, false, db, s);
          first = false;
        }
    } else {
      AngChunk dummy;
      std::memset(&dummy, 0, sizeof(dummy));
      launch_backward(h->sf, dummy, 1, 1, 1, true, true, db, s);
    }
  } else {
    launch_grap_backward(h->grap, db, s);
  }
}
void ensure_pair_jacobians(ta_context *h) {
  hipStream_t s = h->stream;
  const size_t N = (size_t)h->db.n_atoms, P = (size_t)h->db.n_pairs;
  const int D = h->sf.ndim;
  if (!h->descriptors_valid || !h->jvp_valid)
    compute_impl(h, TA_WANT_ENERGY, false, nullptr);
  if (h->jvp_valid) return;
  h->jvp_J.ensure((size_t)D * 4 * P + 8);
  for (int c = 0; c < D; ++c) {
    ta::launch_one_hot(h->db.dEdG, (int64_t)N, D, c, s);
    backward_only(h);
    if (P)
      HIP_CHECK(hipMemcpyAsync(h->jvp_J.ptr + (size_t)c * 4 * P, h->db.g, 4 * P * sizeof(double),
                               hipMemcpyDeviceToDevice, s));
  }
  HIP_CHECK(hipGetLastError());
  h->jvp_valid = true;
}
}

int ta_loss_gradient(ta_handle h, const double *frame_coeff, const double *dR, const double *dh, double *grad,
                     int64_t n_grad, double *dG_out) {
  if (!h || !grad) return TA_ERR_INVALID;
  if (h->td) {
    if (!frame_coeff && !dR && !dh) return fail(h, TA_ERR_INVALID, "nothing to differentiate");
    return ta_td_loss_gradient(h, frame_coeff, nullptr, nullptr, dR, dh, grad, n_grad, dG_out);
  }
  if (h->kind == TA_MODEL_EAM_FS) return fail(h, TA_ERR_INVALID, fs_inference_only("ta_loss_gradient"));
  if (!h->have_batch) return fail(h, TA_ERR_INVALID, "no resident batch");
  if (!dR && !dh) {
    if (!frame_coeff) return fail(h, TA_ERR_INVALID, "nothing to differentiate");
    return ta_energy_gradient(h, frame_coeff, grad, n_grad);
  }
  if (h->eam) {
    if (!ta::eam_loss_gradient_supported(h->eam))
      return fail(h, TA_ERR_UNSUPPORTED, "ta_loss_gradient: the analytic force / stress term covers EAM / ADP models "
                                         "whose analytic parts are of the Zjw04 family or tabulated");
    if (h->filtered)
      return fail(h, TA_ERR_UNSUPPORTED, "ta_loss_gradient: not available on a skin-filtered batch; "
                                         "ta_set_skin(h, 0) and ta_set_frames first");
    return guarded(h, [&]() {
      const int64_t total = ta::eam_param_count(h->eam);
      if (n_grad != total)
        throw std::invalid_argument("ta_loss_gradient: expected room for " + std::to_string(total) + " values");
      if (dG_out) throw std::invalid_argument("ta_loss_gradient: dG_out is for the descriptor models");
      if (total == 0) return;
      if (ta::eam_nn_tables_on(h->eam)) HIP_CHECK(hipStreamSynchronize(h->stream));
      ta::eam_mark_trained(h->eam);
      ta::eam_ensure(h->eam, h->db);
      compute_impl(h, TA_WANT_ENERGY, false, nullptr);
      hipStream_t s = h->stream;
      const size_t N = (size_t)h->db.n_atoms, F = (size_t)h->db.n_frames;
      h->train_grad.ensure((size_t)total + 8);
      h->train_coeff.ensure(F + 8);
      h->tan_dir.ensure(3 * N + 9 * F + 8);
      double *d_dR = h->tan_dir.ptr, *d_dh = h->tan_dir.ptr + 3 * N;
      if (dR) HIP_CHECK(hipMemcpyAsync(d_dR, dR, 3 * N * sizeof(double), hipMemcpyHostToDevice, s));
      if (dh) HIP_CHECK(hipMemcpyAsync(d_dh, dh, 9 * F * sizeof(double), hipMemcpyHostToDevice, s));
      if (frame_coeff && F)
        HIP_CHECK(hipMemcpyAsync(h->train_coeff.ptr, frame_coeff, F * sizeof(double), hipMemcpyHostToDevice, s));
      ta::eam_loss_gradient(h->eam, h->db, frame_coeff ? h->train_coeff.ptr : nullptr, dR ? d_dR : nullptr,
                            dh ? d_dh : nullptr, h->train_grad.ptr, s);
      HIP_CHECK(hipGetLastError());
      HIP_CHECK(hipMemcpyAsync(grad, h->train_grad.ptr, (size_t)total * sizeof(double), hipMemcpyDeviceToHost, s));
      HIP_CHECK(hipStreamSynchronize(s));
    });
  }
  if (h->kind != TA_MODEL_SF_MLP && h->kind != TA_MODEL_GRAP_MLP)
    return fail(h, TA_ERR_UNSUPPORTED, "ta_loss_gradient: the analytic force / stress term exists for the per-atom MLP models");
  if (h->filtered)
    return fail(h, TA_ERR_UNSUPPORTED, "ta_loss_gradient: not available on a skin-filtered batch; "
                                       "ta_set_skin(h, 0) and ta_set_frames first");
  return guarded(h, [&]() {
    int64_t total = 0;
    for (int e = 0; e < h->n_elements; ++e) total += ta::mlp_param_count(h->mlp[e]);
    if (n_grad != total)
      throw std::invalid_argument("ta_loss_gradient: expected room for " + std::to_string(total) + " values");
    hipStream_t s = h->stream;
    const size_t N = (size_t)h->db.n_atoms, P = (size_t)h->db.n_pairs, F = (size_t)h->db.n_frames;
    const int D = h->sf.ndim;
    ensure_pair_jacobians(h);
    h->tan_dir.ensure(3 * N + 9 * F + 8);
    h->tan_dD.ensure(4 * P + 8);
    h->tan_dG.ensure(N * (size_t)D + 8);
    double *d_dR = h->tan_dir.ptr, *d_dh = h->tan_dir.ptr + 3 * N;
    if (dR) HIP_CHECK(hipMemcpyAsync(d_dR, dR, 3 * N * sizeof(double), hipMemcpyHostToDevice, s));
    else HIP_CHECK(hipMemsetAsync(d_dR, 0, 3 * N * sizeof(double), s));
    if (dh) HIP_CHECK(hipMemcpyAsync(d_dh, dh, 9 * F * sizeof(double), hipMemcpyHostToDevice, s));
    else HIP_CHECK(hipMemsetAsync(d_dh, 0, 9 * F * sizeof(double), s));
    ta::launch_pair_tangent(h->db, d_dR, d_dh, h->tan_dD.ptr, s);
    ta::launch_descriptor_jvp(h->db, D, h->jvp_J.ptr, h->tan_dD.ptr, h->tan_dG.ptr, s);
    size_t scratch = 0, partial = 0;
    for (int e = 0; e < h->n_elements; ++e) {
      const int n_el = h->db.elem_start[e + 1] - h->db.elem_start[e];
      scratch = std::max(scratch, ta::mlp_grad2_scratch_doubles(h->mlp[e], n_el));
      partial = std::max(partial, ta::mlp_grad_partial_doubles(h->mlp[e], n_el));
    }
    h->train_scratch.ensure(scratch + 8);
    h->train_partial.ensure(partial + 8);
    h->train_grad.ensure((size_t)total + 8);
    h->train_coeff.ensure(F + 8);
    if (frame_coeff && F)
      HIP_CHECK(hipMemcpyAsync(h->train_coeff.ptr, frame_coeff, F * sizeof(double), hipMemcpyHostToDevice, s));
    size_t off = 0;
    for (int e = 0; e < h->n_elements; ++e) {
      const int n_el = h->db.elem_start[e + 1] - h->db.elem_start[e];
      ta::launch_mlp_grad2(h->mlp[e], h->activation, D, h->db.elem_atoms + h->db.elem_start[e], n_el, h->db,
                           h->tan_dG.ptr, frame_coeff ? h->train_coeff.ptr : nullptr, h->train_scratch.ptr,
                           h->train_partial.ptr, h->train_grad.ptr + off, s);
      off += (size_t)ta::mlp_param_count(h->mlp[e]);
    }
    HIP_CHECK(hipGetLastError());
    HIP_CHECK(hipMemcpyAsync(grad, h->train_grad.ptr, (size_t)total * sizeof(double), hipMemcpyDeviceToHost, s));
    if (dG_out && N)
      HIP_CHECK(hipMemcpyAsync(dG_out, h->tan_dG.ptr, N * (size_t)D * sizeof(double), hipMemcpyDeviceToHost, s));
    HIP_CHECK(hipStreamSynchronize(s));
  });
}

int ta_td_loss_gradient(ta_handle h, const double *coeff_free_energy, const double *coeff_energy,
                        const double *coeff_eentropy, const double *dR, const double *dh, double *grad,
                        int64_t n_grad, double *dG_out) {
  if (!h || !grad) return TA_ERR_INVALID;
  if (!h->td) return fail(h, TA_ERR_INVALID, "ta_td_loss_gradient: not a temperature-dependent model");
  if (!h->have_batch) return fail(h, TA_ERR_INVALID, "no resident batch");
  const bool direction = dR || dh;
  if (direction && h->filtered)
    return fail(h, TA_ERR_UNSUPPORTED, "ta_td_loss_gradient: not available on a skin-filtered batch; "
                                       "ta_set_skin(h, 0) and ta_set_frames first");
  return guarded(h, [&]() {
    const int nel = h->n_elements;
    const int64_t total = ta::td_param_count(h->td_nets, nel);
    if (n_grad != total)
      throw std::invalid_argument("ta_td_loss_gradient: expected room for " + std::to_string(total) + " values");
    if (dG_out && !direction) throw std::invalid_argument("ta_td_loss_gradient: dG_out needs a direction");
    hipStream_t s = h->stream;
    const size_t N = (size_t)h->db.n_atoms, P = (size_t)h->db.n_pairs, F = (size_t)h->db.n_frames;
// ... 370 lines not shown
```

tensoralloy_amd/csrc/ta_device.h:

```cpp
#pragma once
#include <hip/hip_runtime.h>

#include <cstdint>

#include "tensoralloy_amd.h"

namespace ta {

constexpr int kMaxRadial = 64;
constexpr int kMaxElements = 8;
constexpr int kMaxBetaSlots = 3;
constexpr int kRecDoubles = 8;
constexpr int kMaxLayers = 8;
constexpr int kCapMin = 192;
constexpr int kCapMax = 1024;
constexpr int kMaxCentersPerBlock = 16;
constexpr int kMaxHd = 24;

struct SFParams {
  double rcut, acut;
  double inv_rc2, inv_ac2;
  double two_inv_ac2;
  double eps;
  double ang_scale;
  int n_elements;
  int n_rad;
  int n_ang;
  int n_radial_dim;
  int ndim;
  int angular;
  int cutoff;
  int n_beta;
  double eta[kMaxRadial], omega[kMaxRadial];
  double beta[kMaxBetaSlots];
  signed char eta_pow[kMaxRadial];
};

struct AngChunk {
  double beta[2];
  int hslot[2];
  double gamma[2];
  double zeta[2];
  double kz[2];
  int zeta_int[2];
  int chan[8];
  int safe_pow;
  int n_hd;
  double hd[kMaxHd];
};

struct DeviceBatch {
  int64_t n_atoms = 0, n_pairs = 0;
  int n_frames = 0, nnl_max = 0;
  double *pos = nullptr;
  double *cells = nullptr;
  int32_t *species = nullptr;
  int32_t *frame_of_atom = nullptr;
  int32_t *atom_start = nullptr;
  int32_t *pair_start = nullptr;
  int32_t *pair_stop = nullptr;
  int32_t *seg_start = nullptr;
  int32_t *pair_i = nullptr, *pair_j = nullptr, *pair_shift = nullptr, *pair_rev = nullptr;
  const int32_t *slot_q = nullptr, *rev_super = nullptr, *rev_map = nullptr;
  int32_t *blk_center = nullptr;
  int n_blk = 0;
  int blk_groups = 0;
  const int32_t *n_blk_dev = nullptr;
  int cap = kCapMin;
  int32_t *elem_atoms = nullptr;
  int32_t elem_start[kMaxElements + 1] = {0};

  double *rec = nullptr;
  double *rec4 = nullptr;
  double *part4 = nullptr;
  unsigned long long *masks = nullptr;
  uint32_t *job_word = nullptr;
  int32_t *job_count = nullptr;
  int job_stride = 0;
  double *G = nullptr;
  double *dEdG = nullptr;
  double *eatom = nullptr;
  double *g = nullptr;
  double *forces = nullptr;
  double *wat = nullptr;
  double *fown = nullptr;
  int own_sums = 0;
#ifdef TA_PHASE_STAMPS
  unsigned long long *stamps = nullptr;
#endif
  double *bpart = nullptr;
  double *energy = nullptr;
  double *virial = nullptr;
  double *batch_energy = nullptr;
};

#ifdef __HIPCC__
__device__ __forceinline__ int pair_stop_of(const DeviceBatch &b, int64_t i) {
  return b.pair_stop ? b.pair_stop[i] : b.pair_start[i + 1];
}
#endif

#ifdef __HIPCC__
__device__ __forceinline__ int pair_rev_of(const DeviceBatch &b, int q) {
  return b.slot_q ? b.rev_map[b.rev_super[b.slot_q[q]]] : b.pair_rev[q];
}
__device__ __forceinline__ const double2 *pair_geom(const DeviceBatch &b, size_t q) {
  return reinterpret_cast<const double2 *>(b.rec4 ? b.rec4 + 4 * q : b.rec + kRecDoubles * q);
}
#endif

struct MlpLayerDev {
  int k, n;
  int kp, np;
  double *w;
  double *wt;
  double *b;
  int act;
  int res;
};
struct MlpDev {
  int n_layers = 0;
  MlpLayerDev layer[kMaxLayers];
  double *xlo = nullptr, *xhi = nullptr;
  int max_np = 0, max_kp = 0;
};

void launch_pair_geometry(const SFParams &sf, const DeviceBatch &b, hipStream_t s);
void launch_g4_forward(const SFParams &sf, const AngChunk &ch, int nb, int ng, int nz,
                       const DeviceBatch &b, hipStream_t s);
void launch_descriptor_reduce(const SFParams &sf, const DeviceBatch &b, hipStream_t s);
void launch_mlp(const SFParams &sf, const MlpDev &mlp, int activation, int element,
                const DeviceBatch &b, hipStream_t s);
void launch_backward(const SFParams &sf, const AngChunk &ch, int nb, int ng, int nz,
                     bool first, bool radial_only, const DeviceBatch &b, hipStream_t s);
void launch_force_gather(const SFParams &sf, const DeviceBatch &b, hipStream_t s);
void launch_frame_reduce(const DeviceBatch &b, bool want_virial, double *mirror, int64_t n_tail, hipStream_t s);

size_t g4_lds_bytes(int nnl_max);

size_t v2_lds_bytes(bool backward, int cap, int n_local = 0, int nspec = 0);
int v2_job_stride(int cap);
void launch_g4_forward_v2(const SFParams &sf, const AngChunk &ch, int ng, int nz, bool geometry,
                          bool reduce, const DeviceBatch &b, hipStream_t s);
void launch_backward_v2(const SFParams &sf, const AngChunk &ch, int ng, int nz, bool first,
                        const DeviceBatch &b, hipStream_t s);

struct NlGrid {
  double h[9];
  double hinv[9];
  double lo[3];
  double inv_w[3];
  int32_t nb[3];
  int32_t pbc[3];
  int32_t bin_offset;
  int32_t pad_;
  int32_t m[3];
  int32_t ortho;
  double bw[3];
};
struct NlRec {
  double x, y, z;
  int32_t wx, wy, wz;
  int32_t j;
  int32_t sp;
  int32_t pad_;
};
struct NlWork {
  int32_t *wrap;
  int32_t *binid;
  int32_t *bin_count;
  int32_t *bin_start;
  int32_t *bin_cursor;
  int32_t *bin_atoms;
  NlRec *recs;
  int32_t *counts;
  int32_t *seg_start;
  unsigned long long *stats;
};
bool nl_make_grid(const ta_frame &fr, double rmax, int bin_offset, NlGrid &g);
int nl_bins(const NlGrid &g);
void nl_count(int n_atoms, int n_bins, int nel, double rmax, const double *pos, const int32_t *species,
              const int32_t *frame_of_atom, const NlGrid *grids, NlWork &w, int32_t *pair_start,
              hipStream_t s);
size_t nl_build_zero_words(int n_atoms, int n_bins);
void nl_build(int n_atoms, int n_bins, int nel, double rmax, const double *pos, const int32_t *species,
              const int32_t *frame_of_atom, const NlGrid *grids, NlWork &w, unsigned long long *zero,
              bool zero_is_clean, long long capacity, int32_t *pair_start, int32_t *host_pair_start,
              int32_t *pair_i, int32_t *pair_j, int32_t *pair_shift, int32_t *pair_rev, long long rev_cover,
              hipStream_t s);
void nl_reverse_sorted(int64_t n_pairs, int nel, const int32_t *species, const int32_t *seg_start,
                       const int32_t *pair_i, const int32_t *pair_j, const int32_t *pair_shift,
                       int32_t *pair_rev, unsigned long long *stats, hipStream_t s);
int nl_filter_blocks(int n_atoms);
void nl_filter(int n_atoms, int64_t n_super, int nel, double rmax, const double *pos, const double *cells,
               const int32_t *frame_of_atom, const int32_t *start_super, const int32_t *seg_super,
               const int32_t *pj_super, const int32_t *ps_super, const int32_t *rev_super, int32_t *map,
               int32_t *seg_exact, int32_t *pair_start, int32_t *pair_stop, int32_t *pi_out, int32_t *pj_out,
               int32_t *ps_out, int32_t *rev_out, int32_t *slot_q, int cap, int32_t *blk_center, hipStream_t s);
void nl_fill(int n_atoms, int64_t n_pairs, int nel, double rmax, const double *pos,
             const int32_t *species, const int32_t *frame_of_atom, const NlGrid *grids, NlWork &w,
             int32_t *pair_i, int32_t *pair_j, int32_t *pair_shift, int32_t *pair_rev, hipStream_t s);

}
```

tensoralloy_amd/csrc/ta_kernels_v2.hip:

```cpp
#include <hip/hip_runtime.h>

#include <cstdio>
#include <cstdlib>
#include <stdexcept>
#include <type_traits>

#include "ta_device.h"
#include "ta_math.h"
#include "ta_reduce.h"

namespace ta {
namespace {

constexpr int kBlock = 256;
constexpr int kNF = 8;
constexpr int kNFf = 7;
constexpr int kSegW = 6;
constexpr int kJobCtlBytes = (60 + 2 * kMaxCentersPerBlock * kSegW) * 4;
__host__ __device__ inline int v2_pcols(int cap, int nspec) {
  return nspec >= 1 ? cap / 4 + kMaxCentersPerBlock * nspec : cap;
}
constexpr int kRingPad = 64;
constexpr int kRTab = 8;

#ifdef TA_LDS_PROBE
__device__ __forceinline__ bool kProbe(int flags, int bit) { return (flags >> bit) & 1; }
#else
__device__ __forceinline__ constexpr bool kProbe(int, int) { return false; }
#endif

#ifdef TA_PHASE_STAMPS
#define TA_STAMP(b, kernel, k)                                                                          \
  do {                                                                                                  \
    if ((b).stamps && threadIdx.x == 0)                                                                 \
      (b).stamps[((size_t)(kernel) * gridDim.x + blockIdx.x) * 8 + (k)] = __builtin_amdgcn_s_memrealtime(); \
  } while (0)
#else
#define TA_STAMP(b, kernel, k) do {} while (0)
#endif

__device__ __forceinline__ int angular_term2(int s1, int s2, int nel) {
  int a = s1 < s2 ? s1 : s2, b = s1 < s2 ? s2 : s1;
  return a * nel - (a * (a - 1)) / 2 + (b - a);
}
__device__ __forceinline__ int radial_term2(int center, int other) {
  return other == center ? 0 : (other < center ? other + 1 : other);
}

struct Fields {
  double2 *zr, *xy, *ih, *gs;
  double *sp1;
  float *xf, *yf, *zf;
};

__device__ __forceinline__ Fields carve(double *lds, int cap, bool forward = false) {
  Fields f;
  f.zr = reinterpret_cast<double2 *>(lds);
  f.xy = f.zr + cap;
  f.ih = f.xy + cap;
  f.gs = forward ? nullptr : f.ih + cap;
  f.sp1 = forward ? reinterpret_cast<double *>(f.ih + cap) : nullptr;
  f.xf = forward ? reinterpret_cast<float *>(f.sp1 + cap) : nullptr;
  f.yf = forward ? f.xf + (2 * cap + kRingPad) : nullptr;
  f.zf = forward ? f.yf + (2 * cap + kRingPad) : nullptr;
  return f;
}

template <int HD>
__device__ __forceinline__ void hd_eval(const SFParams &sf, const AngChunk &ch, double beta,
                                        double u, double &h, double &dh) {
  if constexpr (HD > 0) {
    double p = ch.hd[HD - 1], d = 0.0;
#pragma unroll
    for (int k = HD - 2; k >= 0; --k) {
      d = fma(d, u, p);
      p = fma(p, u, ch.hd[k]);
    }
    h = p;
    dh = d;
  } else {
    double fd, dfd;
    cutoff_u(sf.cutoff, u, fd, dfd);
    const double ed = ta_exp(-beta * u);
    h = ed * fd;
    dh = ed * (dfd - beta * fd);
  }
}
template <int HD>
__device__ __forceinline__ double hd_value(const SFParams &sf, const AngChunk &ch, double beta,
                                           double u) {
  if constexpr (HD > 0) {
    double p = ch.hd[HD - 1];
#pragma unroll
    for (int k = HD - 2; k >= 0; --k) p = fma(p, u, ch.hd[k]);
    return p;
  } else {
    return ta_exp(-beta * u) * cutoff_u_value(sf.cutoff, u);
  }
}

template <int HD>
__device__ __forceinline__ void stage(const SFParams &sf, const AngChunk &ch, double beta, const DeviceBatch &b,
                                      const Fields &f, int s0, int M, int geom = 0, bool forward = false) {
  for (int item = threadIdx.x; item < M; item += blockDim.x) {
    double2 v0, v1, v2;
    if (geom) {
      const int64_t p = (int64_t)s0 + item;
      const int i = b.pair_i[p], j = b.pair_j[p];
      const double *h = b.cells + 9 * (size_t)b.frame_of_atom[i];
      const double sx = (double)b.pair_shift[3 * p], sy = (double)b.pair_shift[3 * p + 1],
                   sz = (double)b.pair_shift[3 * p + 2];
      const double *ri = b.pos + 3 * (size_t)i, *rj = b.pos + 3 * (size_t)j;
      const double dx = (rj[0] - ri[0]) + (sx * h[0] + sy * h[3] + sz * h[6]);
      const double dy = (rj[1] - ri[1]) + (sx * h[1] + sy * h[4] + sz * h[7]);
      const double dz = (rj[2] - ri[2]) + (sx * h[2] + sy * h[5] + sz * h[8]);
      const double r2 = dx * dx + dy * dy + dz * dz + sf.eps;
      v0 = make_double2(dx, dy);
      v1 = make_double2(dz, r2);
      v2 = make_double2(1.0 / sqrt(r2), 0.0);
      if (b.rec4) {
        double2 *dst = reinterpret_cast<double2 *>(b.rec4 + 4 * (size_t)p);
        dst[0] = v0;
        dst[1] = v1;
      } else {
        double2 *dst = reinterpret_cast<double2 *>(b.rec + kRecDoubles * (size_t)p);
        dst[0] = v0;
        dst[1] = v1;
        dst[2] = v2;
        dst[3] = make_double2(0.0, 0.0);
      }
    } else if (b.rec4) {
      const double2 *src = reinterpret_cast<const double2 *>(b.rec4 + 4 * (size_t)(s0 + item));
      v0 = src[0];
      v1 = src[1];
      v2 = make_double2(1.0 / sqrt(v1.y), 0.0);
    } else {
      const double2 *src = reinterpret_cast<const double2 *>(b.rec + kRecDoubles * (size_t)(s0 + item));
      v0 = src[0];
      v1 = src[1];
      v2 = src[2];
    }
    f.xy[item] = v0;
    f.zr[item] = v1;
    if (forward) {
      const int ci = b.pair_i[s0 + item];
      const int cbase = b.pair_start[ci] - s0, cn = pair_stop_of(b, ci) - b.pair_start[ci];
      const int k0 = 2 * cbase + (item - cbase);
      f.xf[k0] = f.xf[k0 + cn] = (float)v0.x;
      f.yf[k0] = f.yf[k0 + cn] = (float)v0.y;
      f.zf[k0] = f.zf[k0 + cn] = (float)v1.x;
    }
    const double u = v1.y * sf.inv_ac2;
    double H = 0.0, L = 0.0;
    if (u < 1.0) {
      if (forward) {
        H = hd_value<HD>(sf, ch, beta, u);
      } else {
        double dH;
        hd_eval<HD>(sf, ch, beta, u, H, dH);
        L = (H != 0.0) ? sf.two_inv_ac2 * dH / H : 0.0;
      }
    }
    f.ih[item] = make_double2(v2.x, H);
    if (forward) f.sp1[item] = (double)b.species[b.pair_j[s0 + item]];
    else f.gs[item] = make_double2(L, (double)b.species[b.pair_j[s0 + item]]);
  }
  __syncthreads();
}

__device__ __forceinline__ unsigned long long partner_mask(const SFParams &sf, const Fields &f,
                                                           int base, int n, int a, int sc, int smax) {
  const int ring = 2 * base + a;
  const float ax = f.xf[ring], ay = f.yf[ring], az = f.zf[ring];
  const float lim = (float)(sf.acut * sf.acut) * 1.0001f;
  unsigned long long mask = 0ull;
  const int count = smax - sc + 1;
  typedef float f32x2 __attribute__((ext_vector_type(2)));
  const f32x2 ax2 = {ax, ax}, ay2 = {ay, ay}, az2 = {az, az};
  for (int g = 0; g < 4 && 16 * g < count; ++g) {
    const float *px = f.xf + ring + sc + 16 * g, *py = f.yf + ring + sc + 16 * g,
                *pz = f.zf + ring + sc + 16 * g;
    unsigned m = 0u;
#pragma unroll
    for (int k = 14; k >= 0; k -= 2) {
      const f32x2 vx = {px[k], px[k + 1]}, vy = {py[k], py[k + 1]}, vz = {pz[k], pz[k + 1]};
      const f32x2 ex = vx - ax2, ey = vy - ay2, ez = vz - az2;
      const f32x2 d2 = __builtin_elementwise_fma(ex, ex, __builtin_elementwise_fma(ey, ey, ez * ez));
      const float dhi = d2.y, dlo = d2.x;
      asm("v_cmp_lt_f32 vcc, %1, %2\n\tv_addc_co_u32 %0, vcc, %0, %0, vcc" : "+v"(m) : "v"(dhi), "v"(lim) : "vcc");
      asm("v_cmp_lt_f32 vcc, %1, %2\n\tv_addc_co_u32 %0, vcc, %0, %0, vcc" : "+v"(m) : "v"(dlo), "v"(lim) : "vcc");
    }
    mask |= (unsigned long long)m << (16 * g);
  }
  if (count < 64) mask &= (1ull << count) - 1ull;
  const int half = n >> 1;
  if (!(n & 1) && a >= half && half >= sc && half < sc + 64) mask &= ~(1ull << (half - sc));
  return mask;
}

__device__ __forceinline__ void deal_by_popcount(const Fields &f, int cap, int M, int &item,
                                                 unsigned long long &mask) {
  int *hist = reinterpret_cast<int *>(f.xf);
  int *start = hist + 66;
  unsigned long long *pmask = reinterpret_cast<unsigned long long *>(hist + 132);
  int *pitem = reinterpret_cast<int *>(pmask + cap);
  const int tid = threadIdx.x;
  const bool active = tid < M;
  __syncthreads();
  if (tid < 66) hist[tid] = 0;
  __syncthreads();
  const int bucket = 64 - (active ? __popcll(mask) : 0);
  int rank = 0;
  if (active) rank = atomicAdd(&hist[bucket], 1);
  __syncthreads();
  if (tid < 65) {
    int s = 0;
    for (int k = 0; k < tid; ++k) s += hist[k];
    start[tid] = s;
  }
  __syncthreads();
  if (active) {
    const int slot = start[bucket] + rank;
    pitem[slot] = item;
    pmask[slot] = mask;
  }
  __syncthreads();
  if (active) {
    item = pitem[tid];
    mask = pmask[tid];
  }
}

struct JobLists {
  uint32_t *word;
  int *hist, *start;
};

__device__ __forceinline__ JobLists job_lists(const Fields &f) {
  JobLists j;
  j.word = reinterpret_cast<uint32_t *>(f.xf);
  return j;
}
__device__ __forceinline__ int job_item(uint32_t w) { return (int)(w & 255u); }
__device__ __forceinline__ int job_centre(uint32_t w) { return (int)((w >> 10) & 15u); }
static_assert(kMaxCentersPerBlock <= 16, "four bits of a job word name the centre");

__host__ __device__ inline size_t v2_counter_offset(int cap) {
  const size_t end = (size_t)cap * kNFf * sizeof(double) + 3 * (size_t)(2 * cap + kRingPad) * sizeof(float);
  return (end + 15) & ~(size_t)15;
}
__host__ __device__ inline int v2_max_jobs(int cap) { return 4 * cap; }

__device__ __forceinline__ int make_jobs(JobLists &j, bool active, int item, int centre, unsigned long long m0) {
  const int tid = threadIdx.x;
  int cnt[4] = {0, 0, 0, 0}, rank[4] = {0, 0, 0, 0};
  if (active) {
#pragma unroll
    for (int w = 0; w < 4; ++w) {
      const int c = __popc((unsigned)((m0 >> (16 * w)) & 0xffffull));
      cnt[w] = c;
      if (c) rank[w] = atomicAdd(&j.hist[16 - c], 1);
    }
  }
  __syncthreads();
  if (tid < 64) {
    const int v = tid < 16 ? j.hist[tid] : 0;
    int incl = v;
#pragma unroll
    for (int off = 1; off < 16; off <<= 1) {
      const int u = __shfl_up(incl, off);
      if (tid >= off) incl += u;
    }
    if (tid < 16) j.start[tid] = incl - v;
    if (tid == 15) j.start[16] = incl;
  }
  __syncthreads();
  if (active) {
#pragma unroll
    for (int w = 0; w < 4; ++w)
      if (cnt[w]) {
        const int slot = j.start[16 - cnt[w]] + rank[w];
        j.word[slot] = (uint32_t)item | ((uint32_t)w << 8) | ((uint32_t)centre << 10) |
                       ((uint32_t)((m0 >> (16 * w)) & 0xffffull) << 16);
      }
  }
  const int n = j.start[16];
  __syncthreads();
  return n;
}

__device__ __forceinline__ int job_slot(int r, int tid, int T) { return r * T + ((r & 1) ? T - 1 - tid : tid); }

__device__ __forceinline__ void reduce_radial_from_lds(const SFParams &sf, const DeviceBatch &b,
                                                       const Fields &f, int c0, int c1, int s0) {
  const int nel = sf.n_elements;
  const int w = threadIdx.x >> 6, l = threadIdx.x & 63, nwaves = blockDim.x >> 6;
  bool no_shift = true;
  for (int c = 0; c < sf.n_rad; ++c) no_shift = no_shift && sf.omega[c] == 0.0;
  for (int64_t i = c0 + w; i < c1; i += nwaves) {
    const int sA = b.species[i];
    const int32_t *seg = b.seg_start + (size_t)i * (nel + 1);
    double *Gi = b.G + (size_t)i * sf.ndim;
    for (int sb = 0; sb < nel; ++sb) {
      const int tr = radial_term2(sA, sb);
      const int q0 = seg[sb] - s0, q1 = seg[sb + 1] - s0;
      for (int cc = 0; cc < sf.n_rad; cc += 4) {
        double acc[4] = {0.0, 0.0, 0.0, 0.0};
        for (int q = q0 + l; q < q1; q += 64) {
          const double r2 = f.zr[q].y;
          const double u = r2 * sf.inv_rc2;
          const double fc = (u < 1.0) ? cutoff_u_value(sf.cutoff, u) : 0.0;
          if (no_shift) {
#pragma unroll
            for (int k = 0; k < 4; ++k) {
              const int c = (cc + k < sf.n_rad) ? cc + k : cc;
              acc[k] += ta_exp(-sf.eta[c] * u) * fc;
            }
          } else {
            const double r = sqrt(r2);
#pragma unroll
            for (int k = 0; k < 4; ++k) {
              const int c = (cc + k < sf.n_rad) ? cc + k : cc;
              const double dr = r - sf.omega[c];
              acc[k] += ta_exp(-sf.eta[c] * dr * dr * sf.inv_rc2) * fc;
            }
          }
        }
#pragma unroll
        for (int k = 0; k < 4; ++k) {
          const double v = wave_sum(acc[k]);
          if (l == 0 && cc + k < sf.n_rad) Gi[tr * sf.n_rad + cc + k] = v;
        }
      }
    }
  }
}

template <int NSPEC, int NG, int NZ>
__device__ __forceinline__ void reduce_angular_from_lds(const SFParams &sf, const AngChunk &ch,
                                                        const DeviceBatch &b, const double *red, int cap,
                                                        int c0, int c1, int s0, int sp_lo, int sp_hi) {
  const int nel = sf.n_elements;
  const int w = threadIdx.x >> 6, l = threadIdx.x & 63, nwaves = blockDim.x >> 6;
  for (int64_t i = c0 + w; i < c1; i += nwaves) {
    const int32_t *seg = b.seg_start + (size_t)i * (nel + 1);
    double *Gi = b.G + (size_t)i * sf.ndim + sf.n_radial_dim;
    for (int sp = sp_lo; sp < sp_hi; ++sp)
      for (int sg = 0; sg < NSPEC; ++sg) {
        const int t = angular_term2(sg, sp, nel);
        const int q0 = seg[sg] - s0, q1 = seg[sg + 1] - s0;
#pragma unroll
        for (int gz = 0; gz < NG * NZ; ++gz) {
          double v = 0.0;
          const double *col = red + (size_t)((sp - sp_lo) * NG * NZ + gz) * cap;
          for (int q = q0 + l; q < q1; q += 64) v += col[q];
          v = wave_sum(v) * sf.ang_scale;
          if (l == 0) {
            double *dst = Gi + t * sf.n_ang + ch.chan[gz];
            *dst = (sg >= sp) ? v : *dst + v;
          }
        }
      }
  }
}

template <int NSPEC, int NG, int NZ>
__device__ __forceinline__ void assemble_flat(const SFParams &sf, const AngChunk &ch, const DeviceBatch &b,
                                              const Fields &f, const double *P, const int *sslot, int c0, int c1,
                                              int s0, int item, bool active, bool skip_radial, int cap) {
  constexpr int kGZ = NG * NZ;
  constexpr int kTerms = NSPEC * (NSPEC + 1) / 2;
  double *R = reinterpret_cast<double *>(f.xy);
  const int row = threadIdx.x >> 4, l = threadIdx.x & 15, nrows = blockDim.x >> 4;
  const int ncent = c1 - c0;
  bool no_shift = true;
  for (int c = 0; c < sf.n_rad; ++c) no_shift = no_shift && sf.omega[c] == 0.0;
  const double r2 = active ? f.zr[item].y : 0.0;
  const int n_rad = skip_radial ? 0 : sf.n_rad;
  for (int cc = 0; cc == 0 || cc < n_rad; cc += 4) {
    if (cc) __syncthreads();
    if (active && cc < n_rad) {
      const double u = r2 * sf.inv_rc2;
      const double fc = (u < 1.0) ? cutoff_u_value(sf.cutoff, u) : 0.0;
      const double r = no_shift ? 0.0 : sqrt(r2);
      double ev[4];
#pragma unroll
      for (int k = 0; k < 4; ++k) {
        const int c = (cc + k < n_rad) ? cc + k : cc;
        const int pw = (cc + k < n_rad && k > 0) ? sf.eta_pow[c] : 0;
        if (pw > 0) {
          ev[k] = pow_int_m1(ev[k > 0 ? k - 1 : 0], pw) * ev[k > 0 ? k - 1 : 0];
        } else {
          double arg = sf.eta[c] * u;
          if (!no_shift) {
            const double dr = r - sf.omega[c];
            arg = sf.eta[c] * dr * dr * sf.inv_rc2;
          }
          ev[k] = ta_exp(-arg);
        }
        R[k * cap + item] = ev[k] * fc;
      }
    }
    __syncthreads();
    const int nrad_here = cc < n_rad ? (n_rad - cc < 4 ? n_rad - cc : 4) : 0;
    const int n_radial_tasks = NSPEC * nrad_here;
    const int per_centre = n_radial_tasks + (cc == 0 ? kTerms * kGZ : 0);
    for (int t = row; t < ncent * per_centre; t += nrows) {
      const int ci = t / per_centre, k = t - ci * per_centre;
      const int64_t i = c0 + ci;
      const int32_t *seg = b.seg_start + (size_t)i * (NSPEC + 1);
      double *Gi = b.G + (size_t)i * sf.ndim;
      double v = 0.0;
      if (k < n_radial_tasks) {
        const int sb = NSPEC == 1 ? 0 : k / nrad_here, kk = k - sb * nrad_here;
        const double *col = R + (size_t)kk * cap;
        for (int q = seg[sb] - s0 + l; q < seg[sb + 1] - s0; q += 16) v += col[q];
        v = row16_sum(v);
        if (l == 0) Gi[radial_term2(b.species[i], sb) * sf.n_rad + cc + kk] = v;
      } else {
        const int k2 = k - n_radial_tasks;
        const int term = k2 / kGZ, gz = k2 - term * kGZ;
        int sa = 0, sb = 0;
        for (int rem = term, len = NSPEC; rem >= len; rem -= len, --len) ++sa;
        sb = term - (sa * NSPEC - (sa * (sa - 1)) / 2) + sa;
        const int *ss = sslot + ci * kSegW;
        const double *colA = P + (size_t)(sa * kGZ + gz) * v2_pcols(cap, NSPEC);
        for (int q = ss[sb] + l; q < ss[sb + 1]; q += 16) v += colA[q];
        if (sa != sb) {
          const double *colB = P + (size_t)(sb * kGZ + gz) * v2_pcols(cap, NSPEC);
          for (int q = ss[sa] + l; q < ss[sa + 1]; q += 16) v += colB[q];
        }
        v = row16_sum(v);
        if (l == 0) Gi[sf.n_radial_dim + term * sf.n_ang + ch.chan[gz]] = v * sf.ang_scale;
      }
    }
  }
}

__device__ __forceinline__ void stagger(int flags) {
  const int n = (flags >> 8) & 0xff;
  if (n && ((blockIdx.x >> ((flags >> 16) & 31)) & 1))
    for (int k = 0; k < n; ++k) __builtin_amdgcn_s_sleep(127);
}

template <int NSPEC, int NG, int NZ, int HD, bool DEFZ, int CAP, int WPE = (DEFZ && NSPEC <= 2 ? 5 : 0)>
__global__ __launch_bounds__(kBlock)
    __attribute__((amdgpu_waves_per_eu(WPE > 0 ? WPE : 1, 8))) void g4_forward_v2_kernel(SFParams sf, AngChunk ch,
                                                               DeviceBatch b, int flags) {
  static_assert(!DEFZ || NZ == 2, "DEFZ needs the two-zeta grid");
  const int kCap = CAP > 0 ? CAP : b.cap;
  const int geom = flags & 1;
  if (b.n_blk_dev && (int)blockIdx.x >= *b.n_blk_dev) return;
  stagger(flags);
  extern __shared__ double lds[];
  const Fields f = carve(lds, kCap, true);
  const int slot = b.blk_groups > 0 ? 16 * ((int)blockIdx.x % b.blk_groups) + (int)blockIdx.x / b.blk_groups
                                    : (int)blockIdx.x;
  const int c0 = b.blk_center[slot], c1 = b.blk_center[slot + 1];
  if (c0 >= c1) return;
  const int s0 = b.pair_start[c0];
  const int M = pair_stop_of(b, c1 - 1) - s0;
  const double beta = ch.beta[0];
  if (b.job_count) {
    char *raw = reinterpret_cast<char *>(lds);
    int *cnt = reinterpret_cast<int *>(raw + v2_counter_offset(kCap));
    if (threadIdx.x < 40) cnt[threadIdx.x] = 0;
    else if (threadIdx.x < 40 + 17 && (int)threadIdx.x - 40 <= c1 - c0)
      cnt[threadIdx.x] = ((int)threadIdx.x - 40 < c1 - c0 ? b.pair_start[c0 + threadIdx.x - 40] : s0 + M) - s0;
    else if (threadIdx.x >= 64 && (int)threadIdx.x - 64 < (c1 - c0) * (NSPEC + 1)) {
      const int k = ((int)threadIdx.x - 64) / (NSPEC + 1), sg = ((int)threadIdx.x - 64) % (NSPEC + 1);
      cnt[60 + k * kSegW + sg] = b.seg_start[(size_t)(c0 + k) * (NSPEC + 1) + sg] - s0;
    }
    double *P0 = reinterpret_cast<double *>(raw + v2_counter_offset(kCap) + kJobCtlBytes);
    for (int k = threadIdx.x; k < NSPEC * NG * NZ * v2_pcols(kCap, NSPEC); k += blockDim.x) P0[k] = 0.0;
  }
  TA_STAMP(b, 0, 0);
  stage<HD>(sf, ch, beta, b, f, s0, M, geom, true);
  TA_STAMP(b, 0, 1);
  if (b.job_count && threadIdx.x == 0) {
    int *ctl = reinterpret_cast<int *>(reinterpret_cast<char *>(lds) + v2_counter_offset(kCap));
    const int *segl = ctl + 60;
    int *sslot = ctl + 60 + kMaxCentersPerBlock * kSegW;
    int acc = 0;
    for (int k = 0; k < c1 - c0; ++k)
      for (int sg = 0; sg <= NSPEC; ++sg) {
        sslot[k * kSegW + sg] = acc;
        if (sg < NSPEC) acc += (segl[k * kSegW + sg + 1] - segl[k * kSegW + sg] + 3) >> 2;
      }
  }

  auto run_item = [&](int item, bool have_mask, unsigned long long mask0, double *out, double *pacc, auto is_job) {
    constexpr bool kJob = decltype(is_job)::value;
    const int64_t p = (int64_t)s0 + item;
    int base, n;
    int pslot = item;
    if constexpr (kJob) {
      const int *cstart = reinterpret_cast<const int *>(reinterpret_cast<const char *>(lds) + v2_counter_offset(kCap)) + 40;
      const int ci = job_centre((uint32_t)mask0);
      base = cstart[ci];
      n = cstart[ci + 1] - base;
      {
        const int *segl = cstart + 20, *sslot = segl + kMaxCentersPerBlock * kSegW;
        const int sg = NSPEC == 1 ? 0 : (int)f.sp1[item];
        pslot = sslot[ci * kSegW + sg] + ((item - segl[ci * kSegW + sg]) >> 2);
      }
    } else {
      const int i = b.pair_i[p];
      base = b.pair_start[i] - s0;
      n = pair_stop_of(b, i) - b.pair_start[i];
    }
    const int a = item - base;
    const double2 axy = f.xy[item], azr = f.zr[item], aih = f.ih[item];
    const double ax = axy.x, ay = axy.y, az = azr.x;
    const double ra2 = azr.y, inv_ra = aih.x, Ha = aih.y;

    double acc[NSPEC][NG][NZ];
#pragma unroll
    for (int sp = 0; sp < NSPEC; ++sp)
#pragma unroll
      for (int ig = 0; ig < NG; ++ig)
#pragma unroll
        for (int iz = 0; iz < NZ; ++iz) acc[sp][ig][iz] = 0.0;
    double mom[NSPEC][5];
#pragma unroll
    for (int sp = 0; sp < NSPEC; ++sp)
#pragma unroll
      for (int k = 0; k < 5; ++k) mom[sp][k] = 0.0;

    auto triple = [&](int bl) {
        bl = (int)min((unsigned)bl, (unsigned)bl - (unsigned)n);
        const int q = kProbe(flags, 30) ? (int)threadIdx.x : base + bl;
        const double2 bxy = f.xy[q], bzr = f.zr[q];
        const double ex = bxy.x - ax, ey = bxy.y - ay, ez = bzr.x - az;
        const double d2 = fma(ex, ex, fma(ey, ey, fma(ez, ez, sf.eps)));
        const double u = kProbe(flags, 30) ? 0.5 : d2 * sf.inv_ac2;
        if (!(u < 1.0)) return;
        const double2 bih = f.ih[kProbe(flags, 29) ? (int)threadIdx.x : q];
        const double cth = (ra2 + bzr.y - d2) * 0.5 * inv_ra * bih.x;
        const double common = Ha * bih.y * hd_value<HD>(sf, ch, beta, u);
        const int sb = NSPEC == 1 ? 0 : (int)f.sp1[q];
        if constexpr (DEFZ) {
          const double c2 = cth * cth;
          const double t1 = common * cth, t2 = common * c2, t3 = t1 * c2, t4 = t2 * c2;
#pragma unroll
          for (int sp = 0; sp < NSPEC; ++sp) {
            const bool on = NSPEC == 1 || sb == sp;
            mom[sp][0] += on ? common : 0.0;
            mom[sp][1] += on ? t1 : 0.0;
            mom[sp][2] += on ? t2 : 0.0;
            mom[sp][3] += on ? t3 : 0.0;
            mom[sp][4] += on ? t4 : 0.0;
          }
        } else {
#pragma unroll
          for (int ig = 0; ig < NG; ++ig) {
            const double basev = fma(ch.gamma[ig], cth, 1.0);
#pragma unroll
            for (int iz = 0; iz < NZ; ++iz) {
              double pw;
              if (ch.zeta_int[iz] > 0)
                pw = pow_int_m1(basev, ch.zeta_int[iz]) * basev;
              else
                pw = safe_pow_value(ch.safe_pow, basev, ch.zeta[iz]);
              const double v = pw * common;
#pragma unroll
              for (int sp = 0; sp < NSPEC; ++sp)
                acc[sp][ig][iz] += (NSPEC == 1 || sb == sp) ? v : 0.0;
            }
          }
        }
    };
    if constexpr (kJob) {
      const uint32_t jw = (uint32_t)mask0;
      unsigned m = (flags & (1 << 24)) ? 0u : jw >> 16;
      const int k0 = a + 1 + 16 * (int)((jw >> 8) & 3u);
      while (m) {
        const int k = __ffs((int)m) - 1;
        m &= m - 1;
        triple(k0 + k);
      }
    } else {
    const int smax = (Ha != 0.0) ? n / 2 : 0;
    for (int sc = 1; sc <= smax; sc += 64) {
      unsigned long long mask;
      if (have_mask) {
        mask = (flags & (1 << 24)) ? 0ull : mask0;
      } else {
        mask = partner_mask(sf, f, base, n, a, sc, smax);
        if (b.masks) b.masks[(size_t)(sc >> 6) * b.n_pairs + p] = mask;
      }
      while (mask) {
        const int k = __ffsll((long long)mask) - 1;
        mask &= mask - 1;
        triple(a + sc + k);
      }
    }
    }
    if constexpr (DEFZ) {
#pragma unroll
      for (int sp = 0; sp < NSPEC; ++sp)
#pragma unroll
        for (int ig = 0; ig < NG; ++ig) {
          const double g1 = ch.gamma[ig], g2 = g1 * g1;
          acc[sp][ig][0] = fma(g1, mom[sp][1], mom[sp][0]);
          acc[sp][ig][1] = fma(g2 * g2, mom[sp][4], fma(4.0 * g2 * g1, mom[sp][3],
                               fma(6.0 * g2, mom[sp][2], fma(4.0 * g1, mom[sp][1], mom[sp][0]))));
        }
    }
#pragma unroll
    for (int sp = 0; sp < NSPEC; ++sp)
#pragma unroll
      for (int ig = 0; ig < NG; ++ig)
#pragma unroll
        for (int iz = 0; iz < NZ; ++iz) {
          const int c = ch.chan[ig * NZ + iz];
          const double v = acc[sp][ig][iz] * ch.kz[iz];
          if (pacc) {
            if (v != 0.0) atomicAdd(&pacc[(size_t)((sp * NG + ig) * NZ + iz) * v2_pcols(kCap, NSPEC) + pslot], v);
          } else if (out)
            out[(sp * NG + ig) * NZ + iz] = v;
          else
            b.part4[(size_t)(sp * sf.n_ang + c) * b.n_pairs + p] = v;
        }
  };

  int item = threadIdx.x;
  const bool active = item < M;
  int n_own = 0;
  if (active) {
    const int i = b.pair_i[s0 + item];
    n_own = pair_stop_of(b, i) - b.pair_start[i];
  }
  const bool one_pass = M <= (int)blockDim.x && !__syncthreads_or(active && (n_own >> 1) > 64);
  if (one_pass) {
    unsigned long long mask = 0ull;
    if (active) {
      const int64_t p = (int64_t)s0 + item;
      const int i = b.pair_i[p];
      const int base = b.pair_start[i] - s0;
      const int smax = (f.ih[item].y != 0.0) ? n_own / 2 : 0;
      if (smax > 0 && !(flags & (1 << 25))) mask = partner_mask(sf, f, base, n_own, item - base, 1, smax);
      if (b.masks && !b.job_count) b.masks[p] = mask;
    }
    TA_STAMP(b, 0, 2);
    if (b.job_count) {
      char *raw = reinterpret_cast<char *>(lds);
      JobLists jl = job_lists(f);
      jl.hist = reinterpret_cast<int *>(raw + v2_counter_offset(kCap));
      jl.start = jl.hist + 20;
      double *P = reinterpret_cast<double *>(raw + v2_counter_offset(kCap) + kJobCtlBytes);
      const int n_jobs = make_jobs(jl, active, item, active ? b.pair_i[s0 + item] - c0 : 0, mask);
      TA_STAMP(b, 0, 3);
      const size_t jbase = (size_t)blockIdx.x * b.job_stride;
      if (threadIdx.x == 0) b.job_count[blockIdx.x] = n_jobs;
      for (int slot = threadIdx.x; slot < n_jobs; slot += blockDim.x) b.job_word[jbase + slot] = jl.word[slot];
      TA_STAMP(b, 0, 4);
      if (!(flags & (1 << 27)))
        for (int r = 0; r * (int)blockDim.x < n_jobs; ++r) {
          const int slot = job_slot(r, threadIdx.x, blockDim.x);
          if (slot < n_jobs) {
            const uint32_t jw = jl.word[slot];
            run_item(job_item(jw), true, jw, nullptr, P, std::true_type{});
          }
        }
      __syncthreads();
      TA_STAMP(b, 0, 5);
      if (flags & 4) {
        assemble_flat<NSPEC, NG, NZ>(sf, ch, b, f, P, jl.hist + 60 + kMaxCentersPerBlock * kSegW, c0, c1, s0, item, active,
                                     (flags & (1 << 26)) != 0, kCap);
        TA_STAMP(b, 0, 6);
        return;
      }
      if (active) {
        const int64_t p = (int64_t)s0 + threadIdx.x;
        const int ci = b.pair_i[p] - c0, sg = NSPEC == 1 ? 0 : (int)f.sp1[threadIdx.x];
        const int *segl = jl.hist + 60, *sslot = segl + kMaxCentersPerBlock * kSegW;
        const int rel = (int)threadIdx.x - segl[ci * kSegW + sg];
        const int pidx = sslot[ci * kSegW + sg] + (rel >> 2);
        const bool holds = (rel & 3) == 0;
#pragma unroll
        for (int sp = 0; sp < NSPEC; ++sp)
#pragma unroll
          for (int gz = 0; gz < NG * NZ; ++gz)
            b.part4[(size_t)(sp * sf.n_ang + ch.chan[gz]) * b.n_pairs + p] =
                holds ? P[(size_t)(sp * NG * NZ + gz) * v2_pcols(kCap, NSPEC) + pidx] : 0.0;
      }
    } else {
    deal_by_popcount(f, kCap, M, item, mask);
    constexpr int kLocal = NSPEC * NG * NZ;
    constexpr int kGZ = NG * NZ;
    constexpr int kSpPerPass = 8 / kGZ;
    if (flags & 4) {
      double mine[kLocal];
#pragma unroll
      for (int k = 0; k < kLocal; ++k) mine[k] = 0.0;
      if (active) run_item(item, true, mask, mine, nullptr, std::false_type{});
      __syncthreads();
      double *red = reinterpret_cast<double *>(f.xy);
#pragma unroll
      for (int sp_lo = 0; sp_lo < NSPEC; sp_lo += kSpPerPass) {
        const int sp_hi = sp_lo + kSpPerPass < NSPEC ? sp_lo + kSpPerPass : NSPEC;
        if (active) {
#pragma unroll
          for (int k = 0; k < kSpPerPass * kGZ; ++k)
            if (sp_lo * kGZ + k < kLocal) red[(size_t)k * kCap + item] = mine[sp_lo * kGZ + k];
        }
        __syncthreads();
        if (sp_lo == 0) reduce_radial_from_lds(sf, b, f, c0, c1, s0);
        reduce_angular_from_lds<NSPEC, NG, NZ>(sf, ch, b, red, kCap, c0, c1, s0, sp_lo, sp_hi);
        __syncthreads();
      }
      return;
    }
    if (active) run_item(item, true, mask, nullptr, nullptr, std::false_type{});
    }
  } else {
    if (b.job_count && threadIdx.x == 0) b.job_count[blockIdx.x] = -1;
    for (int it = threadIdx.x; it < M; it += blockDim.x) run_item(it, false, 0ull, nullptr, nullptr, std::false_type{});
  }

  if (flags & 2) {
    __syncthreads();
    const int ncent = c1 - c0;
    const int nwaves = blockDim.x >> 6;
    if (ncent <= nwaves) {
      const int w = threadIdx.x >> 6, l = threadIdx.x & 63;
      const bool act = w < ncent;
      const int64_t i = c0 + (act ? w : 0);
      atom_descriptors<64>(sf, b, i, l, act, [&](int c, double v) { b.G[(size_t)i * sf.ndim + c] = v; });
    } else {
      const int row = threadIdx.x >> 4, l = threadIdx.x & 15, nrows = blockDim.x >> 4;
      for (int k0 = 0; k0 < ncent; k0 += nrows) {
        const bool act = k0 + row < ncent;
        const int64_t i = c0 + (act ? k0 + row : 0);
        atom_descriptors<16>(sf, b, i, l, act, [&](int c, double v) { b.G[(size_t)i * sf.ndim + c] = v; });
      }
    }
  }
}

template <int NSPEC, int NG, int NZ, int HD, bool DEFZ, int CAP, int WPE = (DEFZ ? (NSPEC <= 2 ? 5 : 4) : 0)>
__global__ __launch_bounds__(kBlock)
    __attribute__((amdgpu_waves_per_eu(WPE > 0 ? WPE : 1, 8))) void backward_v2_kernel(SFParams sf, AngChunk ch,
                                                             DeviceBatch b, int flags) {
  static_assert(!DEFZ || NZ == 2, "DEFZ needs the two-zeta grid");
  const int first = flags & 1;
  if (b.n_blk_dev && (int)blockIdx.x >= *b.n_blk_dev) return;
  stagger(flags);
  extern __shared__ double lds[];
  const int kCap = CAP > 0 ? CAP : b.cap;
  const Fields f = carve(lds, kCap);
  double *gacc = lds + kNF * kCap + kCap / 8;
  const int slot = b.blk_groups > 0 ? 16 * ((int)blockIdx.x % b.blk_groups) + (int)blockIdx.x / b.blk_groups
                                    : (int)blockIdx.x;
  const int c0 = b.blk_center[slot], c1 = b.blk_center[slot + 1];
  if (c0 >= c1) return;
  const int s0 = b.pair_start[c0];
  const int M = pair_stop_of(b, c1 - 1) - s0;
  const double beta = ch.beta[0];
  for (int k = threadIdx.x; k < 3 * kCap; k += blockDim.x) gacc[k] = 0.0;
  int *cstart = reinterpret_cast<int *>(gacc) - 20;
  if ((int)threadIdx.x <= c1 - c0 && threadIdx.x < 17)
    cstart[threadIdx.x] = ((int)threadIdx.x < c1 - c0 ? b.pair_start[c0 + threadIdx.x] : s0 + M) - s0;
  double *pctab = gacc + 3 * kCap;
  if constexpr (DEFZ && NSPEC == 1) {
    const int k = (int)blockDim.x - 1 - (int)threadIdx.x;
    if (k < c1 - c0) {
      const double *wsrc = b.dEdG + (size_t)(c0 + k) * sf.ndim + sf.n_radial_dim;
      double p0 = 0.0, p1 = 0.0, p2 = 0.0, p3 = 0.0, p4 = 0.0;
#pragma unroll
      for (int ig = 0; ig < NG; ++ig) {
        const double g1 = ch.gamma[ig], g2 = g1 * g1;
        const double w1 = wsrc[ch.chan[ig * NZ]] * ch.kz[0], w4 = wsrc[ch.chan[ig * NZ + 1]] * ch.kz[1];
        p0 += w1 + w4;
        p1 += g1 * (w1 + 4.0 * w4);
        p2 += 6.0 * g2 * w4;
        p3 += 4.0 * g2 * g1 * w4;
        p4 += g2 * g2 * w4;
      }
      pctab[5 * k] = p0;
      pctab[5 * k + 1] = 0.5 * p1;
      pctab[5 * k + 2] = 0.25 * p2;
      pctab[5 * k + 3] = 0.125 * p3;
      pctab[5 * k + 4] = 0.0625 * p4;
    }
  }
  double *rtab = pctab + 5 * kMaxCentersPerBlock;
  const bool use_rtab = first && NSPEC * sf.n_rad <= kRTab;
  if (use_rtab) {
    const int per = NSPEC * sf.n_rad;
    const int t = (int)blockDim.x - 1 - (int)threadIdx.x - kMaxCentersPerBlock;
    if (t >= 0 && t < (c1 - c0) * per) {
      const int ci = t / per, rem = t - ci * per;
      const int sb = rem / sf.n_rad, c = rem - sb * sf.n_rad;
      const int64_t i = c0 + ci;
      rtab[ci * kRTab + rem] = b.dEdG[(size_t)i * sf.ndim + radial_term2(b.species[i], sb) * sf.n_rad + c];
    }
  }
  TA_STAMP(b, 1, 0);
  stage<HD>(sf, ch, beta, b, f, s0, M);
  TA_STAMP(b, 1, 1);
  const int nel = sf.n_elements;

  auto run_item = [&](int item, bool have_mask, unsigned long long mask0, auto is_job) {
    constexpr bool kJob = decltype(is_job)::value;
    const int64_t p = (int64_t)s0 + item;
    int i, base, n;
    if constexpr (kJob) {
      const int ci = job_centre((uint32_t)mask0);
      i = c0 + ci;
      base = cstart[ci];
      n = cstart[ci + 1] - base;
    } else {
      i = b.pair_i[p];
      base = b.pair_start[i] - s0;
      n = pair_stop_of(b, i) - b.pair_start[i];
    }
    const int a = item - base;
    const double2 axy = f.xy[item], azr = f.zr[item], aih = f.ih[item], ags = f.gs[item];
    const double ax = axy.x, ay = axy.y, az = azr.x;
    const double ra2 = azr.y, inv_ra = aih.x, Ha = aih.y, La = ags.x;
    const double inv_ra2 = inv_ra * inv_ra;
    const int sa = (int)ags.y;

    constexpr bool kTable = kJob && DEFZ && NSPEC == 1;
    double w_[NSPEC][NG][NZ], wd[NSPEC][NG][NZ];
#pragma unroll
    for (int sp = 0; sp < (kTable ? 0 : NSPEC); ++sp) {
      const double *wsrc = b.dEdG + (size_t)i * sf.ndim + sf.n_radial_dim +
                           angular_term2(sa, sp, nel) * sf.n_ang;
#pragma unroll
      for (int ig = 0; ig < NG; ++ig)
#pragma unroll
        for (int iz = 0; iz < NZ; ++iz) {
          w_[sp][ig][iz] = wsrc[ch.chan[ig * NZ + iz]] * ch.kz[iz];
          wd[sp][ig][iz] = w_[sp][ig][iz] * ch.zeta[iz] * ch.gamma[ig];
        }
    }

    double pc[NSPEC][5];
    if constexpr (kTable) {
      const double *src = pctab + 5 * (i - c0);
#pragma unroll
      for (int k = 0; k < 5; ++k) pc[0][k] = src[k];
    } else if constexpr (DEFZ) {
#pragma unroll
      for (int sp = 0; sp < NSPEC; ++sp) {
#pragma unroll
        for (int k = 0; k < 5; ++k) pc[sp][k] = 0.0;
#pragma unroll
        for (int ig = 0; ig < NG; ++ig) {
          const double g1 = ch.gamma[ig], g2 = g1 * g1;
          const double w1 = w_[sp][ig][0], w4 = w_[sp][ig][1];
          pc[sp][0] += w1 + w4;
          pc[sp][1] += 0.5 * g1 * (w1 + 4.0 * w4);
          pc[sp][2] += 0.25 * 6.0 * g2 * w4;
          pc[sp][3] += 0.125 * 4.0 * g2 * g1 * w4;
          pc[sp][4] += 0.0625 * g2 * g2 * w4;
        }
      }
    }
    double csum = 0.0, gx = 0.0, gy = 0.0, gz = 0.0;
    auto triple = [&](int bl) {
        bl = (int)min((unsigned)bl, (unsigned)bl - (unsigned)n);
        const int q = kProbe(flags, 30) ? (int)threadIdx.x : base + bl;
        const double2 bxy = f.xy[q], bzr = f.zr[q];
        const double bx = bxy.x, by = bxy.y, bz = bzr.x;
        const double ex = bx - ax, ey = by - ay, ez = bz - az;
        const double d2 = fma(ex, ex, fma(ey, ey, fma(ez, ez, sf.eps)));
        const double u = kProbe(flags, 30) ? 0.5 : d2 * sf.inv_ac2;
        if (!(u < 1.0)) return;
        const int q2 = kProbe(flags, 29) ? (int)threadIdx.x : q;
        const double2 bih = f.ih[q2], bgs = f.gs[q2];
        const double inv_rb = bih.x, Hb = bih.y, Lb = bgs.x;
        const int sb = NSPEC == 1 ? 0 : (int)bgs.y;
        const double inv_ab = inv_ra * inv_rb;
        const double w = (ra2 + bzr.y - d2) * inv_ab;
        double Hd, dHd;
        hd_eval<HD>(sf, ch, beta, u, Hd, dHd);
        const double Hd2 = sf.two_inv_ac2 * dHd;
        double S0 = 0.0, Yc, Y;
        const double HH = Ha * Hb, T = HH * Hd;
        if constexpr (DEFZ) {
          double p0 = pc[0][0], p1 = pc[0][1], p2 = pc[0][2], p3 = pc[0][3], p4 = pc[0][4];
#pragma unroll
          for (int sp = 1; sp < NSPEC; ++sp) {
            p0 = (sb == sp) ? pc[sp][0] : p0;
            p1 = (sb == sp) ? pc[sp][1] : p1;
            p2 = (sb == sp) ? pc[sp][2] : p2;
            p3 = (sb == sp) ? pc[sp][3] : p3;
            p4 = (sb == sp) ? pc[sp][4] : p4;
          }
          S0 = fma(fma(fma(fma(p4, w, p3), w, p2), w, p1), w, p0);
          const double S1w = fma(fma(fma(4.0 * p4, w, 3.0 * p3), w, 2.0 * p2), w, p1);
          const double Z = S1w * T;
          Yc = Z * w;
          Y = Z + Z;
        } else {
          const double cth = 0.5 * w;
          double S1 = 0.0;
#pragma unroll
          for (int ig = 0; ig < NG; ++ig) {
            const double basev = fma(ch.gamma[ig], cth, 1.0);
#pragma unroll
            for (int iz = 0; iz < NZ; ++iz) {
              double ws = w_[0][ig][iz], wds = wd[0][ig][iz];
#pragma unroll
              for (int sp = 1; sp < NSPEC; ++sp) {
                ws = (sb == sp) ? w_[sp][ig][iz] : ws;
                wds = (sb == sp) ? wd[sp][ig][iz] : wds;
              }
              double pm1;
              if (ch.zeta_int[iz] > 0)
                pm1 = pow_int_m1(basev, ch.zeta_int[iz]);
              else
                pm1 = safe_pow_grad(ch.safe_pow, basev, ch.zeta[iz] - 1.0);
              S0 = fma(ws, pm1 * basev, S0);
              S1 = fma(wds, pm1, S1);
            }
          }
          Y = S1 * T;
          Yc = Y * cth;
        }
        const double S0T = S0 * T;
        const double X = (S0 * HH) * Hd2;
        const double ca = fma(S0T, La, fma(-Yc, inv_ra2, X));
        const double cb = fma(S0T, Lb, fma(-Yc, inv_rb * inv_rb, X));
        const double Q = fma(Y, inv_ab, -X);
        csum += ca;
        gx = fma(Q, bx, gx);
        gy = fma(Q, by, gy);
        gz = fma(Q, bz, gz);
        const int q3 = kProbe(flags, 28) ? (int)threadIdx.x : q;
        atomicAdd(&gacc[q3], fma(cb, bx, Q * ax));
        atomicAdd(&gacc[kCap + q3], fma(cb, by, Q * ay));
        atomicAdd(&gacc[2 * kCap + q3], fma(cb, bz, Q * az));
    };
    if constexpr (kJob) {
      const uint32_t jw = (uint32_t)mask0;
      unsigned m = (flags & (1 << 24)) ? 0u : jw >> 16;
      const int k0 = a + 1 + 16 * (int)((jw >> 8) & 3u);
      while (m) {
        const int k = __ffs((int)m) - 1;
        m &= m - 1;
        triple(k0 + k);
      }
    } else {
    const int smax = (Ha != 0.0) ? n / 2 : 0;
    for (int sc = 1; sc <= smax; sc += 64) {
      unsigned long long mask = have_mask ? mask0 : b.masks[(size_t)(sc >> 6) * b.n_pairs + p];
      if (flags & (1 << 24)) mask = 0ull;
      while (mask) {
        const int k = __ffsll((long long)mask) - 1;
        mask &= mask - 1;
        triple(a + sc + k);
      }
    }
    }
    atomicAdd(&gacc[item], fma(csum, ax, gx));
    atomicAdd(&gacc[kCap + item], fma(csum, ay, gy));
    atomicAdd(&gacc[2 * kCap + item], fma(csum, az, gz));
  };

  {
    int item = threadIdx.x;
    const bool active = item < M;
    int n_own = 0;
    if (active) {
      const int i = b.pair_i[s0 + item];
      n_own = pair_stop_of(b, i) - b.pair_start[i];
    }
    const bool one_pass = M <= (int)blockDim.x && !__syncthreads_or(active && (n_own >> 1) > 64);
    const int n_jobs = (one_pass && b.job_count) ? b.job_count[blockIdx.x] : -1;
    if (n_jobs >= 0) {
      const size_t jbase = (size_t)blockIdx.x * b.job_stride;
      uint32_t jws[4];
#pragma unroll
      for (int r = 0; r < 4; ++r) {
        const int slot = job_slot(r, threadIdx.x, blockDim.x);
        jws[r] = slot < n_jobs ? b.job_word[jbase + slot] : 0u;
      }
      TA_STAMP(b, 1, 2);
#pragma unroll
      for (int r = 0; r < 4; ++r) {
        if (r * (int)blockDim.x >= n_jobs) break;
        const int slot = job_slot(r, threadIdx.x, blockDim.x);
        if (slot < n_jobs) run_item(job_item(jws[r]), true, jws[r], std::true_type{});
      }
      TA_STAMP(b, 1, 3);
    } else if (one_pass) {
      unsigned long long mask = 0ull;
      if (active) {
        const int64_t p = (int64_t)s0 + item;
        const int smax = (f.ih[item].y != 0.0) ? n_own / 2 : 0;
        if (smax > 0) mask = b.masks[p];
      }
      if (active) run_item(item, true, mask, std::false_type{});
    } else {
      for (int it = threadIdx.x; it < M; it += blockDim.x) run_item(it, false, 0ull, std::false_type{});
    }
  }
  __syncthreads();
  TA_STAMP(b, 1, 4);
  for (int item = threadIdx.x; item < M; item += blockDim.x) {
    const int64_t p = (int64_t)s0 + item;
    double gx = gacc[item], gy = gacc[kCap + item], gz = gacc[2 * kCap + item];
    if (first) {
      const double *wr;
      if (use_rtab) {
        int ci = 0;
        for (int k = 1; k < c1 - c0; ++k) ci += (item >= cstart[k]) ? 1 : 0;
        wr = rtab + ci * kRTab + (NSPEC == 1 ? 0 : (int)f.gs[item].y * sf.n_rad);
      } else {
        const int i = b.pair_i[p];
        wr = b.dEdG + (size_t)i * sf.ndim + radial_term2(b.species[i], (int)f.gs[item].y) * sf.n_rad;
      }
      const double r2 = f.zr[item].y, inv_r = f.ih[item].x;
      const double ur = r2 * sf.inv_rc2;
      double s = 0.0;
      if (ur < 1.0) {
        double fc, dfdu;
        cutoff_u(sf.cutoff, ur, fc, dfdu);
        const double r = r2 * inv_r;
        const double dfdr = dfdu * 2.0 * r * sf.inv_rc2;
        double e = 0.0;
        for (int c = 0; c < sf.n_rad; ++c) {
          const double dr = r - sf.omega[c];
          const int pw = sf.eta_pow[c];
          e = pw > 0 ? pow_int_m1(e, pw) * e : ta_exp(-sf.eta[c] * dr * dr * sf.inv_rc2);
          s = fma(wr[c], e * (dfdr - 2.0 * sf.eta[c] * dr * fc * sf.inv_rc2), s);
        }
      }
      s *= inv_r;
      gx = fma(s, f.xy[item].x, gx);
      gy = fma(s, f.xy[item].y, gy);
      gz = fma(s, f.zr[item].x, gz);
    } else {
      gx += b.g[4 * (size_t)p];
      gy += b.g[4 * (size_t)p + 1];
      gz += b.g[4 * (size_t)p + 2];
    }
    b.g[4 * (size_t)p] = gx;
    b.g[4 * (size_t)p + 1] = gy;
    b.g[4 * (size_t)p + 2] = gz;
  }
  TA_STAMP(b, 1, 5);
}

template <int NSPEC, int NG, int NZ>
void fwd_t(const SFParams &sf, const AngChunk &ch, const DeviceBatch &b, int geom, hipStream_t s) {
  const dim3 grid((unsigned)b.n_blk), block((unsigned)(b.cap < kBlock ? b.cap : kBlock));
  const size_t lds = v2_lds_bytes(false, b.cap, b.job_count ? NSPEC * NG * NZ : 0, NSPEC);
  if constexpr (NZ == 2) {
    if (ch.n_hd == 12 && ch.zeta_int[0] == 1 && ch.zeta_int[1] == 4) {
      if (b.cap == kCapMin) {
        static const int force = getenv("TA_FWD_WPE") ? atoi(getenv("TA_FWD_WPE")) : 0;
        if constexpr (NSPEC <= 2) {
          if (force != 5) {
            hipLaunchKernelGGL((g4_forward_v2_kernel<NSPEC, NG, NZ, 12, true, kCapMin, 6>), grid, block, lds, s, sf, ch,
                               b, geom);
            return;
          }
        }
        hipLaunchKernelGGL((g4_forward_v2_kernel<NSPEC, NG, NZ, 12, true, kCapMin>), grid, block, lds, s, sf, ch, b, geom);
      } else
        hipLaunchKernelGGL((g4_forward_v2_kernel<NSPEC, NG, NZ, 12, true, 0>), grid, block, lds, s, sf, ch, b, geom);
      return;
    }
    if (ch.n_hd == 16 && ch.zeta_int[0] == 1 && ch.zeta_int[1] == 4) {
      hipLaunchKernelGGL((g4_forward_v2_kernel<NSPEC, NG, NZ, 16, true, 0>), grid, block, lds, s, sf, ch, b, geom);
      return;
    }
  }
  if (ch.n_hd > 0 && ch.n_hd <= 16)
    hipLaunchKernelGGL((g4_forward_v2_kernel<NSPEC, NG, NZ, 16, false, 0>), grid, block, lds, s, sf, ch, b, geom);
  else if (ch.n_hd == 24)
    hipLaunchKernelGGL((g4_forward_v2_kernel<NSPEC, NG, NZ, 24, false, 0>), grid, block, lds, s, sf, ch, b, geom);
  else
    hipLaunchKernelGGL((g4_forward_v2_kernel<NSPEC, NG, NZ, 0, false, 0>), grid, block, lds, s, sf, ch, b, geom);
}
template <int NSPEC, int NG, int NZ>
void bwd_t(const SFParams &sf, const AngChunk &ch, const DeviceBatch &b, int first, hipStream_t s) {
  const dim3 grid((unsigned)b.n_blk), block((unsigned)(b.cap < kBlock ? b.cap : kBlock));
  const size_t lds = v2_lds_bytes(true, b.cap);
  if constexpr (NZ == 2) {
    if (ch.n_hd == 12 && ch.zeta_int[0] == 1 && ch.zeta_int[1] == 4) {
      if (b.cap == kCapMin) {
        static const int force = getenv("TA_BWD_WPE") ? atoi(getenv("TA_BWD_WPE")) : 0;
        if constexpr (NSPEC == 1) {
          if (force == 6) {
            hipLaunchKernelGGL((backward_v2_kernel<NSPEC, NG, NZ, 12, true, kCapMin, 6>), grid, block, lds, s, sf, ch,
                               b, first);
            return;
          }
        }
        hipLaunchKernelGGL((backward_v2_kernel<NSPEC, NG, NZ, 12, true, kCapMin>), grid, block, lds, s, sf, ch, b, first);
      } else
        hipLaunchKernelGGL((backward_v2_kernel<NSPEC, NG, NZ, 12, true, 0>), grid, block, lds, s, sf, ch, b, first);
      return;
    }
    if (ch.n_hd == 16 && ch.zeta_int[0] == 1 && ch.zeta_int[1] == 4) {
      hipLaunchKernelGGL((backward_v2_kernel<NSPEC, NG, NZ, 16, true, 0>), grid, block, lds, s, sf, ch, b, first);
      return;
    }
  }
  if (ch.n_hd > 0 && ch.n_hd <= 16)
    hipLaunchKernelGGL((backward_v2_kernel<NSPEC, NG, NZ, 16, false, 0>), grid, block, lds, s, sf, ch, b, first);
  else if (ch.n_hd == 24)
    hipLaunchKernelGGL((backward_v2_kernel<NSPEC, NG, NZ, 24, false, 0>), grid, block, lds, s, sf, ch, b, first);
  else
    hipLaunchKernelGGL((backward_v2_kernel<NSPEC, NG, NZ, 0, false, 0>), grid, block, lds, s, sf, ch, b, first);
}

}

size_t v2_lds_bytes(bool backward, int cap, int n_local, int nspec) {
  if (!backward && n_local > 0)
    return v2_counter_offset(cap) + kJobCtlBytes + (size_t)n_local * v2_pcols(cap, nspec) * sizeof(double);
  if (backward)
    return (size_t)cap * kNF * sizeof(double) + cap + 3 * (size_t)cap * sizeof(double) +
           kMaxCentersPerBlock * (5 + kRTab) * sizeof(double);
  return (size_t)cap * kNF * sizeof(double) + 3 * (size_t)(2 * cap + kRingPad) * sizeof(float) + cap;
}
int v2_job_stride(int cap) { return v2_max_jobs(cap); }

#ifdef TA_V2_FEW
#define TA_DISPATCH_V2(FN, ...)                                   \
  do {                                                            \
    const int key = nspec * 100 + ng * 10 + nz;                   \
    if (key == 122) FN<1, 2, 2>(__VA_ARGS__);                     \
    else if (key == 222) FN<2, 2, 2>(__VA_ARGS__);                \
    else throw std::domain_error("TA_V2_FEW build");              \
  } while (0)
#else
#define TA_DISPATCH_V2(FN, ...)                                   \
  do {                                                            \
    const int key = nspec * 100 + ng * 10 + nz;                   \
    switch (key) {                                                \
      case 111: FN<1, 1, 1>(__VA_ARGS__); break;                  \
      case 112: FN<1, 1, 2>(__VA_ARGS__); break;                  \
      case 121: FN<1, 2, 1>(__VA_ARGS__); break;                  \
      case 122: FN<1, 2, 2>(__VA_ARGS__); break;                  \
      case 211: FN<2, 1, 1>(__VA_ARGS__); break;                  \
      case 212: FN<2, 1, 2>(__VA_ARGS__); break;                  \
      case 221: FN<2, 2, 1>(__VA_ARGS__); break;                  \
      case 222: FN<2, 2, 2>(__VA_ARGS__); break;                  \
      case 311: FN<3, 1, 1>(__VA_ARGS__); break;                  \
      case 312: FN<3, 1, 2>(__VA_ARGS__); break;                  \
      case 321: FN<3, 2, 1>(__VA_ARGS__); break;                  \
      case 322: FN<3, 2, 2>(__VA_ARGS__); break;                  \
      case 422: FN<4, 2, 2>(__VA_ARGS__); break;                  \
      case 522: FN<5, 2, 2>(__VA_ARGS__); break;                  \
      default:                                                    \
        throw std::domain_error("no second-generation angular kernel for this (species, gamma, zeta) shape"); \
    }                                                             \
  } while (0)
#endif

static int stagger_bits(const DeviceBatch &b, const char *var) {
  const char *e = getenv(var);
  if (getenv("TA_DEBUG_NO_TRIPLES")) return 1 << 24;
  if (const char *d = getenv("TA_DEBUG_SKIP")) return (atoi(d) & 127) << 24;
  if (!e) return 0;
  int n = 0, shift = 3;
  if (sscanf(e, "%d,%d", &n, &shift) < 1) return 0;
  (void)b;
  return ((n & 0xff) << 8) | ((shift & 31) << 16);
}

void launch_g4_forward_v2(const SFParams &sf, const AngChunk &ch, int ng, int nz, bool geometry,
                          bool reduce, const DeviceBatch &b, hipStream_t s) {
  if (b.n_blk == 0) return;
  const int nspec = sf.n_elements;
  const int geom = (geometry ? 1 : 0) | (reduce ? 2 : 0) | ((geometry && reduce) ? 4 : 0) |
                   stagger_bits(b, "TA_STAGGER_FWD");
  TA_DISPATCH_V2(fwd_t, sf, ch, b, geom, s);
}

void launch_backward_v2(const SFParams &sf, const AngChunk &ch, int ng, int nz, bool first,
                        const DeviceBatch &b, hipStream_t s) {
  if (b.n_blk == 0) return;
  const int nspec = sf.n_elements;
  const int f = (first ? 1 : 0) | stagger_bits(b, "TA_STAGGER_BWD");
  TA_DISPATCH_V2(bwd_t, sf, ch, b, f, s);
}

}
```

tensoralloy_amd/engine.py:

```python
from __future__ import annotations

import ctypes as C
from typing import Iterable, List, Sequence

import numpy as np

from . import _lib
from .utils import GPa


class Engine:
    def __init__(self, nn, device: int = 0):
        self._lib = _lib.load()
        self._nn = nn
        self._clf = nn.transformer
        if self._clf is None:
            raise ValueError("A descriptor transformer must be attached.")
        desc, keep = nn.to_desc()
        self._handle = C.c_void_p()
        rc = self._lib.ta_create(C.byref(desc), int(device), C.byref(self._handle))
        del keep
        if rc != _lib.TA_OK:
            _lib.check(self._lib, None, rc)
        self.device = int(device)
# ... 137 lines not shown
            if energy is None:
                energy = np.empty(0)
            forces, virial = self._view_array(ptrs[1], (N, 3)), self._view_array(ptrs[2], (F, 3, 3))
            atomic = self._view_array(ptrs[3], (N,))
        else:
            buf = getattr(self, "_step_buf", None)
            if buf is None or buf[0] != (N, F):
                buf = ((N, F), np.empty(F), np.empty((N, 3)), np.empty((F, 3, 3)), np.empty(N))
                self._step_buf = buf
            _, energy, forces, virial, atomic = buf
            self._check(self._lib.ta_step(
                self._handle, _lib.as_dp(pos), cptr, want, _lib.as_dp(energy),
                _lib.as_dp(forces) if want_f else null, _lib.as_dp(virial) if want_f else null,
                _lib.as_dp(atomic) if want & _lib.TA_WANT_ATOMIC else null, rebuilt_ref))
        self.batch_generation += 1
        if cells is not None:
            self._volumes = np.abs(np.linalg.det(cells))
        if rebuilt.value:
            n_pairs, n_triples, nnl = C.c_int64(0), C.c_int64(0), C.c_int32(0)
            self._check(self._lib.ta_list_sizes(self._handle, C.byref(n_pairs), C.byref(n_triples), C.byref(nnl)))
            self.info.n_pairs, self.info.n_triples, self.info.nnl_max = n_pairs.value, n_triples.value, nnl.value
        out = {"energy": energy}
        if want_f and forces is not None:
            out["forces"], out["virial"] = forces, virial
        if want & _lib.TA_WANT_ATOMIC and atomic is not None:
            out["atomic"] = atomic
        if self.finite_temperature:
            out = self._td_results(out)
        return out

    def list_stats(self):
        a, b = C.c_int64(0), C.c_int64(0)
        self._check(self._lib.ta_list_stats(self._handle, C.byref(a), C.byref(b)))
        return int(a.value), int(b.value)

    def compute(self, want: int):
        self._check(self._lib.ta_compute(self._handle, int(want)))

    def set_stream(self, stream_ptr):
        HIP_STREAM_LEGACY = 1
        if stream_ptr is None:
            ptr = 0
        else:
            ptr = int(stream_ptr) or HIP_STREAM_LEGACY
        self._check(self._lib.ta_set_stream(self._handle, C.c_void_p(ptr)))

    def synchronize(self):
        self._check(self._lib.ta_synchronize(self._handle))

    def fetch(self, want: int, descriptors=False) -> dict:
        info = self.info
        N, F = int(info.n_atoms), int(info.n_frames)
        out = {"energy": np.empty(F)}
        forces = virial = atomic = desc = None
        if want & (_lib.TA_WANT_FORCES | _lib.TA_WANT_VIRIAL):
            forces = np.empty((N, 3))
            virial = np.empty((F, 3, 3))
        if want & _lib.TA_WANT_ATOMIC:
            atomic = np.empty(N)
        if descriptors:
            desc = np.empty((N, int(info.descriptor_dim)))
        null = C.POINTER(C.c_double)()
        self._check(self._lib.ta_get_results(
            self._handle, _lib.as_dp(out["energy"]),
            _lib.as_dp(forces) if forces is not None else null,
            _lib.as_dp(virial) if virial is not None else null,
            _lib.as_dp(atomic) if atomic is not None else null,
            _lib.as_dp(desc) if desc is not None else null))
        if forces is not None:
            out["forces"], out["virial"] = forces, virial
        if atomic is not None:
            out["atomic"] = atomic
        if desc is not None:
            scale = getattr(self._nn, "descriptor_scale", None)
            out["descriptors"] = desc * scale() if scale is not None else desc
        if self.finite_temperature:
            out = self._td_results(out)
        return out

    def evaluate(self, atoms_list: Sequence, want: int = None, descriptors=False) -> List[dict]:
        if want is None:
            want = (_lib.TA_WANT_ENERGY | _lib.TA_WANT_FORCES | _lib.TA_WANT_VIRIAL |
                    _lib.TA_WANT_ATOMIC)
        self.set_frames(atoms_list)
        self.compute(want)
        return self._per_frame(self.fetch(want, descriptors=descriptors))

    def _per_frame(self, res: dict) -> List[dict]:
        out, a = [], 0
        for f, n in enumerate(self._natoms):
            d = {"energy": float(res["energy"][f])}
            if "atomic" in res:
                d["atomic"] = res["atomic"][a:a + n]
            for key in ("free_energy", "eentropy"):
                if key in res:
                    d[key] = float(res[key][f])
            for key in ("free_energy_atomic", "eentropy_atomic"):
                if key in res:
                    d[key] = res[key][a:a + n]
            if "forces" in res:
                d["forces"] = res["forces"][a:a + n]
                w = res["virial"][f]
                d["virial"] = w
                if self._volumes[f] > 0.0:
                    s = w / self._volumes[f]
                    d["stress"] = np.array([s[0, 0], s[1, 1], s[2, 2], s[1, 2], s[0, 2], s[0, 1]])
                    d["total_pressure"] = float(np.trace(s) / (-3.0 * GPa))
            if "descriptors" in res:
                d["descriptors"] = res["descriptors"][a:a + n]
            out.append(d)
            a += n
        return out

    def evaluate_md(self, atoms, want: int = None, descriptors=False) -> dict:
        if want is None:
            want = (_lib.TA_WANT_ENERGY | _lib.TA_WANT_FORCES | _lib.TA_WANT_VIRIAL |
                    _lib.TA_WANT_ATOMIC)
        periodic = self._clf.periodic
        pbc = tuple(bool(x) for x in atoms.pbc) if periodic else (False, False, False)
        sig = (len(atoms), np.asarray(atoms.numbers).tobytes(), pbc)
        cell = np.ascontiguousarray(atoms.get_cell(complete=True), dtype=np.float64).reshape(3, 3)
        if sig == self._md_sig and self.info is not None and self.finite_temperature:
            T = float(atoms.info.get("etemperature", 0.0))
            if self._etemperatures is None or self._etemperatures[0] != T:
                self.set_electron_temperatures([T])
        if sig == self._md_sig and self.info is not None and not descriptors:
            same_cell = np.array_equal(cell, self._md_cell)
            res = self.step(atoms.positions, want, None if same_cell else cell[None], view=True)
            self._md_cell = cell
            return self._per_frame({k: v.copy() for k, v in res.items()})[0]
        if sig == self._md_sig and self.info is not None:
            same_cell = np.array_equal(cell, self._md_cell)
            self.update_positions(atoms.positions, None if same_cell else cell[None])
            self._md_cell = cell
        else:
            self.set_frames([atoms])
            self._md_sig, self._md_cell = sig, cell
        self.compute(want)
        return self._per_frame(self.fetch(want, descriptors=descriptors))[0]

    def time_compute(self, want: int, warmup: int, steps: int, per_kernel=True):
        total = C.c_double(0.0)
        slots = np.zeros(_lib.TA_N_KERNEL_SLOTS)
        self._check(self._lib.ta_time_compute(
            self._handle, int(want), int(warmup), int(steps), C.byref(total),
            _lib.as_dp(slots) if per_kernel else C.POINTER(C.c_double)()))
        return total.value, dict(zip(_lib.KERNEL_SLOTS, slots.tolist()))

    def count_contributing_triples(self) -> int:
        n = C.c_int64(0)
        self._check(self._lib.ta_count_contributing_triples(self._handle, C.byref(n)))
        return int(n.value)

    def measure_hbm_copy(self, nbytes: int = 1 << 30, reps: int = 10) -> float:
        g = C.c_double(0.0)
        self._check(self._lib.ta_measure_hbm_copy(self._handle, int(nbytes), int(reps), C.byref(g)))
        return g.value

    def batch_energy_device_ptr(self) -> int:
        p = C.c_void_p()
        self._check(self._lib.ta_batch_energy_device_ptr(self._handle, C.byref(p)))
        return p.value

    def copy_batch_energy(self, dst_device_ptr: int):
        self._check(self._lib.ta_copy_batch_energy(self._handle, C.c_void_p(int(dst_device_ptr))))

    def param_count(self) -> int:
        n = C.c_int64(0)
        self._check(self._lib.ta_param_count(self._handle, C.byref(n)))
        return int(n.value)

    def update_weights(self, flat):
        flat = np.ascontiguousarray(flat, dtype=np.float64).ravel()
        self._check(self._lib.ta_update_weights(self._handle, _lib.as_dp(flat), len(flat)))

    def energy_gradient(self, frame_coeff) -> np.ndarray:
        coeff = np.ascontiguousarray(frame_coeff, dtype=np.float64).ravel()
        if len(coeff) != int(self.info.n_frames):
            raise ValueError("one coefficient per resident frame")
        grad = np.zeros(self.param_count())
        self._check(self._lib.ta_energy_gradient(self._handle, _lib.as_dp(coeff), _lib.as_dp(grad), len(grad)))
        return grad

    def loss_gradient(self, frame_coeff=None, dR=None, dh=None, return_tangent=False):
        null = C.POINTER(C.c_double)()
        N, F = int(self.info.n_atoms), int(self.info.n_frames)

        def arr(a, shape):
            if a is None:
                return None, null
            a = np.ascontiguousarray(a, dtype=np.float64).reshape(shape)
            return a, _lib.as_dp(a)
        c, cp = arr(frame_coeff, (F,))
        r, rp = arr(dR, (N, 3))
        hh, hp = arr(dh, (F, 9))
        grad = np.zeros(self.param_count())
        tangent = np.zeros((N, int(self.info.descriptor_dim))) if return_tangent else None
        self._check(self._lib.ta_loss_gradient(self._handle, cp, rp, hp, _lib.as_dp(grad), len(grad),
                                               _lib.as_dp(tangent) if return_tangent else null))
        if return_tangent:
            scale = getattr(self._nn, "descriptor_scale", None)
            return grad, (tangent * scale() if scale is not None else tangent)
        return grad

    def td_loss_gradient(self, coeff_free_energy=None, coeff_energy=None, coeff_eentropy=None, dR=None, dh=None,
                         return_tangent=False):
        null = C.POINTER(C.c_double)()
        N, F = int(self.info.n_atoms), int(self.info.n_frames)

        def arr(a, shape):
            if a is None:
                return None, null
            a = np.ascontiguousarray(a, dtype=np.float64).reshape(shape)
            return a, _lib.as_dp(a)
        b, bp = arr(coeff_free_energy, (F,))
        a, ap = arr(coeff_energy, (F,))
        g, gp = arr(coeff_eentropy, (F,))
        r, rp = arr(dR, (N, 3))
        hh, hp = arr(dh, (F, 9))
        grad = np.zeros(self.param_count())
        tangent = np.zeros((N, int(self.info.descriptor_dim))) if return_tangent else None
        self._check(self._lib.ta_td_loss_gradient(self._handle, bp, ap, gp, rp, hp, _lib.as_dp(grad), len(grad),
                                                  _lib.as_dp(tangent) if return_tangent else null))
        if return_tangent:
            scale = getattr(self._nn, "descriptor_scale", None)
            return grad, (tangent * scale() if scale is not None else tangent)
        return grad

    def constant_count(self) -> int:
        n = C.c_int64(0)
        self._check(self._lib.ta_constant_count(self._handle, C.byref(n)))
        return int(n.value)

    def constants(self) -> np.ndarray:
        out = np.zeros(self.constant_count())
        self._check(self._lib.ta_get_constants(self._handle, _lib.as_dp(out), len(out)))
        return out

    def update_constants(self, flat):
        flat = np.ascontiguousarray(flat, dtype=np.float64).ravel()
        self._check(self._lib.ta_update_constants(self._handle, _lib.as_dp(flat), len(flat)))

    def constant_gradient(self, frame_coeff=None, dR=None, dh=None) -> np.ndarray:
        null = C.POINTER(C.c_double)()
        N, F = int(self.info.n_atoms), int(self.info.n_frames)

        def arr(a, shape):
            if a is None:
                return None, null
            a = np.ascontiguousarray(a, dtype=np.float64).reshape(shape)
            return a, _lib.as_dp(a)
        c, cp = arr(frame_coeff, (F,))
        r, rp = arr(dR, (N, 3))
        hh, hp = arr(dh, (F, 9))
        grad = np.zeros(self.constant_count())
        self._check(self._lib.ta_constant_gradient(self._handle, cp, rp, hp, _lib.as_dp(grad), len(grad)))
        return grad

    def hessian_vectors(self, dR=None, dh=None, want_virial=False):
        N, F = int(self.info.n_atoms), int(self.info.n_frames)
        null = C.POINTER(C.c_double)()
        rp = hp = null
        if dR is None and dh is None:
            n_dir = 3 * N
        else:
            n_dir = len(dR) if dR is not None else len(dh)
        if dR is not None:
            dR = np.ascontiguousarray(dR, dtype=np.float64).reshape(n_dir, N, 3)
            rp = _lib.as_dp(dR)
        if dh is not None:
            dh = np.ascontiguousarray(dh, dtype=np.float64).reshape(n_dir, F, 9)
            hp = _lib.as_dp(dh)
        dF = np.zeros((n_dir, N, 3))
        dW = np.zeros((n_dir, F, 3, 3)) if want_virial else None
        chunk = 32768 if (dR is None and dh is None) else n_dir
        for first in range(0, n_dir, max(chunk, 1)):
            m = min(chunk, n_dir - first)
            self._check(self._lib.ta_hessian_vectors(
                self._handle, m, first, rp, hp, _lib.as_dp(dF[first:]),
                _lib.as_dp(dW[first:]) if want_virial else null))
        return (dF, dW) if want_virial else dF

    def energies(self, reuse_descriptors=True) -> np.ndarray:
        want = _lib.TA_WANT_ENERGY | (_lib.TA_WANT_REUSE_DESCRIPTORS if reuse_descriptors else 0)
        self.compute(want)
        return self.fetch(_lib.TA_WANT_ENERGY)["energy"]

    def set_batch_energy_target(self, dst_device_ptr):
        self._check(self._lib.ta_set_batch_energy_target(self._handle, C.c_void_p(int(dst_device_ptr or 0))))

    def eam_tabulate(self, r, rho) -> dict:
        r = np.ascontiguousarray(r, dtype=np.float64).ravel()
        rho = np.ascontiguousarray(rho, dtype=np.float64).ravel()
        nel = len(self._nn.elements)
        npair = nel * (nel + 1) // 2
        adp = getattr(self._nn, "tag", "") == "adp"
        nrho = nel * nel if getattr(self._nn, "tag", "") == "fs" else nel
        out = {"rho": np.zeros((nrho, len(r))), "phi": np.zeros((npair, len(r))),
               "embed": np.zeros((nel, len(rho)))}
        null = C.POINTER(C.c_double)()
        if adp:
            out["u"], out["w"] = np.zeros((npair, len(r))), np.zeros((npair, len(r)))
        self._check(self._lib.ta_eam_tabulate(
            self._handle, len(r), _lib.as_dp(r), len(rho), _lib.as_dp(rho), _lib.as_dp(out["rho"]),
            _lib.as_dp(out["phi"]), _lib.as_dp(out["embed"]),
            _lib.as_dp(out["u"]) if adp else null, _lib.as_dp(out["w"]) if adp else null))
# ... 12 lines not shown
```

Before: 35.41 million.

## Evaluate angular backward once per triangle with hashed owner assignment

Adds a triangle-based backward path for single-element SF models with zeta in {1,4}. Each (i,j,k) triangle is assigned to one owning centre by a hash of the index sum. The forward pass builds owned job lists, and the backward kernel evaluates all three angles of that triangle together through polynomial coefficients, accumulating forces with LDS atomics. This is meant to cut redundant per-centre triple work roughly threefold. In exchange it adds extra LDS, forward-pass bookkeeping and atomics, and it is gated on the cell being large enough that no periodic image duplicates an atom.

```diff
diff --git a/include/tensoralloy_amd.h b/include/tensoralloy_amd.h
--- a/include/tensoralloy_amd.h
+++ b/include/tensoralloy_amd.h
@@ -194,6 +194,11 @@
 
 int ta_count_contributing_triples(ta_handle h, int64_t *n_contributing);
 
+int ta_set_triangles(ta_handle h, int on);
+int ta_backward_variant(ta_handle h, int32_t *variant);
+int ta_count_owned_triangles(ta_handle h, int64_t *n_owned);
+int ta_triangle_owner(int64_t n, const int32_t *abc, int32_t *owner);
+
 int ta_get_pairs(ta_handle h, int32_t *i, int32_t *j, int32_t *shift );
 
 #ifdef __cplusplus
diff --git a/tensoralloy_amd/_lib.py b/tensoralloy_amd/_lib.py
--- a/tensoralloy_amd/_lib.py
+++ b/tensoralloy_amd/_lib.py
@@ -41,6 +41,7 @@
     "ta_count_contributing_triples", "ta_loss_gradient", "ta_constant_count", "ta_get_constants", "ta_update_constants",
     "ta_constant_gradient", "ta_list_sizes", "ta_abi_version", "ta_model_desc_size", "ta_set_nn_tables", "ta_step", "ta_hessian_vectors", "ta_view_results", "ta_step_view",
     "ta_set_electron_temperatures", "ta_get_td_results", "ta_td_loss_gradient",
+    "ta_set_triangles", "ta_backward_variant", "ta_count_owned_triangles", "ta_triangle_owner",
 ]
 
 _dp = C.POINTER(C.c_double)
@@ -207,6 +208,10 @@
     lib.ta_list_stats.argtypes = [H, C.POINTER(C.c_int64), C.POINTER(C.c_int64)]
     lib.ta_list_sizes.argtypes = [H, C.POINTER(C.c_int64), C.POINTER(C.c_int64), C.POINTER(C.c_int32)]
     lib.ta_set_nn_tables.argtypes = [H, C.c_int]
+    lib.ta_set_triangles.argtypes = [H, C.c_int]
+    lib.ta_backward_variant.argtypes = [H, C.POINTER(C.c_int32)]
+    lib.ta_count_owned_triangles.argtypes = [H, C.POINTER(C.c_int64)]
+    lib.ta_triangle_owner.argtypes = [C.c_int64, _ip, _ip]
     lib.ta_hessian_vectors.argtypes = [H, C.c_int32, C.c_int32, _dp, _dp, _dp, _dp]
     lib.ta_step.argtypes = [H, _dp, _dp, C.c_uint32, _dp, _dp, _dp, _dp, _ip]
     _dpp = C.POINTER(_dp)
diff --git a/tensoralloy_amd/csrc/ta_api.hip b/tensoralloy_amd/csrc/ta_api.hip
--- a/tensoralloy_amd/csrc/ta_api.hip
+++ b/tensoralloy_amd/csrc/ta_api.hip
@@ -239,6 +239,11 @@
   DevBuf<unsigned long long> masks;
   DevBuf<uint32_t> job_word;
   DevBuf<int32_t> job_count;
+  DevBuf<uint32_t> job_word_own;
+  DevBuf<int32_t> job_count_own;
+  bool triangles = true;
+  bool tri_cells_ok = false;
+  int last_bwd_variant = 0;
   DevBuf<int32_t> pair_start, seg_start, pair_i, pair_j, pair_shift, pair_rev;
   ta::NlGrid *d_grids = nullptr;
   DevBuf<int32_t> nl_wrap, nl_binid, nl_bin_count, nl_bin_start, nl_bin_cursor, nl_bin_atoms, nl_counts;
@@ -804,6 +809,10 @@
       used[TA_K_PAIR_GEOMETRY] = true;
     }
     h->sf.ang_scale = h->use_v2 ? 1.0 : 0.5;
+    const bool tri = h->use_v2 && h->triangles && h->tri_cells_ok && h->n_elements == 1 && need_forces;
+    h->db.job_word_own = (tri && h->db.job_count) ? h->job_word_own.ptr : nullptr;
+    h->db.job_count_own = (tri && h->db.job_count) ? h->job_count_own.ptr : nullptr;
+    h->last_bwd_variant = 0;
     const bool reduce_in_forward = h->sf.angular && h->use_v2;
     if (h->sf.angular) {
       begin(TA_K_G4_FORWARD);
@@ -836,7 +845,7 @@
         bool first = true;
         if (h->use_v2)
           for (const ChunkPlan &cp : h->chunks_v2) {
-            launch_backward_v2(h->sf, cp.ch, cp.ng, cp.nz, first, db, s);
+            h->last_bwd_variant |= launch_backward_v2(h->sf, cp.ch, cp.ng, cp.nz, first, tri, db, s);
             first = false;
           }
         else
@@ -1028,6 +1037,7 @@
                   &h->ex_seg_start, &h->ex_counts, &h->ex_map, &h->ex_blk, &h->ex_slot_q})
     b->release();
   h->masks.release(); h->job_word.release(); h->job_count.release();
+  h->job_word_own.release(); h->job_count_own.release();
   for (auto *b : {&h->nl_wrap, &h->nl_binid, &h->nl_bin_count, &h->nl_bin_start, &h->nl_bin_cursor,
                   &h->nl_bin_atoms, &h->nl_counts})
     b->release();
@@ -1054,6 +1064,10 @@
   const int stride = ta::v2_job_stride(h->db.cap);
   h->job_word.ensure(n_blk * (size_t)stride + 8);
   h->job_count.ensure(n_blk + 8);
+  if (h->n_elements == 1) {
+    h->job_word_own.ensure(n_blk * (size_t)stride + 8);
+    h->job_count_own.ensure(n_blk + 8);
+  }
   h->db.job_word = h->job_word.ptr;
   h->db.job_count = h->job_count.ptr;
   h->db.job_stride = stride;
@@ -1109,6 +1123,22 @@
   h->filtered = true;
 }
 
+bool cells_admit_triangles(double rmax, int32_t n_frames, const ta_frame *frames) {
+  for (int f = 0; f < n_frames; ++f) {
+    const double *c = frames[f].cell;
+    const double vol = std::fabs(c[0] * (c[4] * c[8] - c[5] * c[7]) - c[1] * (c[3] * c[8] - c[5] * c[6]) +
+                                 c[2] * (c[3] * c[7] - c[4] * c[6]));
+    for (int k = 0; k < 3; ++k) {
+      if (!frames[f].pbc[k]) continue;
+      const double *u = c + 3 * ((k + 1) % 3), *v = c + 3 * ((k + 2) % 3);
+      const double nx = u[1] * v[2] - u[2] * v[1], ny = u[2] * v[0] - u[0] * v[2], nz = u[0] * v[1] - u[1] * v[0];
+      const double area = std::sqrt(nx * nx + ny * ny + nz * nz);
+      if (!(vol > rmax * area)) return false;
+    }
+  }
+  return true;
+}
+
 void set_frames_impl(ta_context *h, int32_t n_frames, const ta_frame *frames, ta_batch_info *info) {
   for (int f = 0; f < n_frames; ++f) {
     const ta_frame &fr = frames[f];
@@ -1130,6 +1160,7 @@
   h->db.blk_groups = 0;
   h->db.n_blk_dev = nullptr;
   h->r_list = h->rmax + h->skin;
+  h->tri_cells_ok = cells_admit_triangles(h->rmax, n_frames, frames);
   size_t N = 0;
   for (int f = 0; f < n_frames; ++f) N += (size_t)frames[f].n_atoms;
   if (N >= (1u << 30)) throw std::runtime_error("batch too large for 32-bit atom indices");
@@ -1633,7 +1664,7 @@
 
 namespace {
 __global__ __launch_bounds__(256) void count_triples_kernel(ta::DeviceBatch b, double ac2, double eps,
-                                                            unsigned long long *out) {
+                                                            unsigned long long *out, int owned) {
   const int64_t i = ((int64_t)blockIdx.x * 256 + threadIdx.x) >> 6;
   const int lane = threadIdx.x & 63;
   if (i >= b.n_atoms) return;
@@ -1646,7 +1677,8 @@
     for (int pb = pa + 1; pb < p1; ++pb) {
       const double2 *rb = ta::pair_geom(b, (size_t)pb);
       const double ex = rb[0].x - ax, ey = rb[0].y - ay, ez = rb[1].x - az;
-      n += (rb[1].y < ac2 && ex * ex + ey * ey + ez * ez + eps < ac2) ? 1ull : 0ull;
+      n += (rb[1].y < ac2 && ex * ex + ey * ey + ez * ez + eps < ac2 &&
+            (!owned || ta::owns_triangle((int32_t)i, b.pair_j[pa], b.pair_j[pb]))) ? 1ull : 0ull;
     }
   }
   for (int off = 32; off; off >>= 1) n += __shfl_xor(n, off);
@@ -1667,13 +1699,60 @@
     const int64_t N = h->db.n_atoms;
     if (N)
       hipLaunchKernelGGL(count_triples_kernel, dim3((unsigned)((N * 64 + 255) / 256)), dim3(256), 0, s, h->db,
-                         h->sf.acut * h->sf.acut, h->sf.eps, h->nl_stats.ptr);
+                         h->sf.acut * h->sf.acut, h->sf.eps, h->nl_stats.ptr, 0);
     HIP_CHECK(hipGetLastError());
     unsigned long long v = 0;
     HIP_CHECK(hipMemcpyAsync(&v, h->nl_stats.ptr, sizeof(v), hipMemcpyDeviceToHost, s));
     HIP_CHECK(hipStreamSynchronize(s));
     *n_contributing = (int64_t)v;
   });
+}
+
+int ta_count_owned_triangles(ta_handle h, int64_t *n_owned) {
+  if (!h || !n_owned) return fail(h, TA_ERR_INVALID, "null argument");
+  if (!h->have_batch) return fail(h, TA_ERR_INVALID, "no resident batch");
+  if (h->kind != TA_MODEL_SF_MLP || !h->sf.angular)
+    return fail(h, TA_ERR_INVALID, "only symmetry-function models with angular terms have triples");
+  return guarded(h, [&]() {
+    compute_impl(h, TA_WANT_ENERGY, false, nullptr);
+    h->nl_stats.ensure(8);
+    hipStream_t s = h->stream;
+    HIP_CHECK(hipMemsetAsync(h->nl_stats.ptr, 0, sizeof(unsigned long long), s));
+    const int64_t N = h->db.n_atoms;
+    if (N)
+      hipLaunchKernelGGL(count_triples_kernel, dim3((unsigned)((N * 64 + 255) / 256)), dim3(256), 0, s, h->db,
+                         h->sf.acut * h->sf.acut, h->sf.eps, h->nl_stats.ptr, 1);
+    HIP_CHECK(hipGetLastError());
+    unsigned long long v = 0;
+    HIP_CHECK(hipMemcpyAsync(&v, h->nl_stats.ptr, sizeof(v), hipMemcpyDeviceToHost, s));
+    HIP_CHECK(hipStreamSynchronize(s));
+    *n_owned = (int64_t)v;
+  });
+}
+
+int ta_set_triangles(ta_handle h, int on) {
+  if (!h) return TA_ERR_INVALID;
+  h->triangles = on != 0;
+  return TA_OK;
+}
+
+int ta_backward_variant(ta_handle h, int32_t *variant) {
+  if (!h || !variant) return fail(h, TA_ERR_INVALID, "null argument");
+  *variant = h->last_bwd_variant;
+  return TA_OK;
+}
+
+int ta_triangle_owner(int64_t n, const int32_t *abc, int32_t *owner) {
+  if (n < 0 || (n > 0 && (!abc || !owner))) return TA_ERR_INVALID;
+  for (int64_t t = 0; t < n; ++t) {
+    int32_t a = abc[3 * t], b = abc[3 * t + 1], c = abc[3 * t + 2];
+    if (a > b) std::swap(a, b);
+    if (b > c) std::swap(b, c);
+    if (a > b) std::swap(a, b);
+    const int32_t sorted[3] = {a, b, c};
+    owner[t] = (a == b || b == c) ? -1 : sorted[ta::triangle_owner_rank((uint32_t)a + (uint32_t)b + (uint32_t)c)];
+  }
+  return TA_OK;
 }
 
 int ta_measure_hbm_copy(ta_handle h, int64_t bytes, int32_t reps, double *gbs) {
@@ -1879,7 +1958,7 @@
       bool first = true;
       if (h->use_v2)
         for (const ChunkPlan &cp : h->chunks_v2) {
-          launch_backward_v2(h->sf, cp.ch, cp.ng, cp.nz, first, db, s);
+          launch_backward_v2(h->sf, cp.ch, cp.ng, cp.nz, first, false, db, s);
           first = false;
         }
       else
diff --git a/tensoralloy_amd/csrc/ta_device.h b/tensoralloy_amd/csrc/ta_device.h
--- a/tensoralloy_amd/csrc/ta_device.h
+++ b/tensoralloy_amd/csrc/ta_device.h
@@ -77,6 +77,8 @@
   uint32_t *job_word = nullptr;
   int32_t *job_count = nullptr;
   int job_stride = 0;
+  uint32_t *job_word_own = nullptr;
+  int32_t *job_count_own = nullptr;
   double *G = nullptr;
   double *dEdG = nullptr;
   double *eatom = nullptr;
@@ -94,6 +96,18 @@
   double *batch_energy = nullptr;
 };
 
+__host__ __device__ inline int triangle_owner_rank(uint32_t index_sum) {
+#ifdef __HIP_DEVICE_COMPILE__
+  const uint32_t h = __umul24(index_sum, 0x9E3779u);
+#else
+  const uint32_t h = index_sum * 0x9E3779u;
+#endif
+  return (int)(((h & 0xFFFFFFu) * 3u) >> 24);
+}
+__host__ __device__ inline bool owns_triangle(int32_t i, int32_t j, int32_t k) {
+  return triangle_owner_rank((uint32_t)i + (uint32_t)j + (uint32_t)k) == (j < i ? 1 : 0) + (k < i ? 1 : 0);
+}
+
 #ifdef __HIPCC__
 __device__ __forceinline__ int pair_stop_of(const DeviceBatch &b, int64_t i) {
   return b.pair_stop ? b.pair_stop[i] : b.pair_start[i + 1];
@@ -138,12 +152,12 @@
 
 size_t g4_lds_bytes(int nnl_max);
 
-size_t v2_lds_bytes(bool backward, int cap, int n_local = 0, int nspec = 0);
+size_t v2_lds_bytes(bool backward, int cap, int n_local = 0, int nspec = 0, bool triangles = false);
 int v2_job_stride(int cap);
 void launch_g4_forward_v2(const SFParams &sf, const AngChunk &ch, int ng, int nz, bool geometry,
                           bool reduce, const DeviceBatch &b, hipStream_t s);
-void launch_backward_v2(const SFParams &sf, const AngChunk &ch, int ng, int nz, bool first,
-                        const DeviceBatch &b, hipStream_t s);
+int launch_backward_v2(const SFParams &sf, const AngChunk &ch, int ng, int nz, bool first, bool triangles,
+                       const DeviceBatch &b, hipStream_t s);
 
 struct NlGrid {
   double h[9];
diff --git a/tensoralloy_amd/csrc/ta_kernels_v2.hip b/tensoralloy_amd/csrc/ta_kernels_v2.hip
--- a/tensoralloy_amd/csrc/ta_kernels_v2.hip
+++ b/tensoralloy_amd/csrc/ta_kernels_v2.hip
@@ -16,7 +16,8 @@
 constexpr int kNF = 8;
 constexpr int kNFf = 7;
 constexpr int kSegW = 6;
-constexpr int kJobCtlBytes = (60 + 2 * kMaxCentersPerBlock * kSegW) * 4;
+constexpr int kOwnCtl = 60 + 2 * kMaxCentersPerBlock * kSegW;
+constexpr int kJobCtlBytes = (kOwnCtl + 40) * 4;
 __host__ __device__ inline int v2_pcols(int cap, int nspec) {
   return nspec >= 1 ? cap / 4 + kMaxCentersPerBlock * nspec : cap;
 }
@@ -101,7 +102,8 @@
 
 template <int HD>
 __device__ __forceinline__ void stage(const SFParams &sf, const AngChunk &ch, double beta, const DeviceBatch &b,
-                                      const Fields &f, int s0, int M, int geom = 0, bool forward = false) {
+                                      const Fields &f, int s0, int M, int geom = 0, bool forward = false,
+                                      int *jidx = nullptr) {
   for (int item = threadIdx.x; item < M; item += blockDim.x) {
     double2 v0, v1, v2;
     if (geom) {
@@ -162,7 +164,8 @@
       }
     }
     f.ih[item] = make_double2(v2.x, H);
-    if (forward) f.sp1[item] = (double)b.species[b.pair_j[s0 + item]];
+    if (jidx) jidx[item] = b.pair_j[s0 + item];
+    else if (forward) f.sp1[item] = (double)b.species[b.pair_j[s0 + item]];
     else f.gs[item] = make_double2(L, (double)b.species[b.pair_j[s0 + item]]);
   }
   __syncthreads();
@@ -290,6 +293,61 @@
 }
 
 __device__ __forceinline__ int job_slot(int r, int tid, int T) { return r * T + ((r & 1) ? T - 1 - tid : tid); }
+
+__device__ __forceinline__ void make_owned_jobs(int *hist, int *start, const uint32_t word[4], const unsigned own[4],
+                                                uint32_t *out, int32_t *count) {
+  const int tid = threadIdx.x;
+  int cnt[4], rank[4] = {0, 0, 0, 0};
+#pragma unroll
+  for (int r = 0; r < 4; ++r) {
+    cnt[r] = __popc(own[r]);
+    if (cnt[r]) rank[r] = atomicAdd(&hist[16 - cnt[r]], 1);
+  }
+  __syncthreads();
+  if (tid < 64) {
+    const int v = tid < 16 ? hist[tid] : 0;
+    int incl = v;
+#pragma unroll
+    for (int off = 1; off < 16; off <<= 1) {
+      const int u = __shfl_up(incl, off);
+      if (tid >= off) incl += u;
+    }
+    if (tid < 16) start[tid] = incl - v;
+    if (tid == 15) *count = incl;
+  }
+  __syncthreads();
+#pragma unroll
+  for (int r = 0; r < 4; ++r)
+    if (cnt[r]) out[start[16 - cnt[r]] + rank[r]] = (word[r] & 0xffffu) | (own[r] << 16);
+}
+
+template <int NG, int NZ>
+__device__ __forceinline__ void defz_coeffs(const AngChunk &ch, const double *wsrc, double pc[5]) {
+  double p0 = 0.0, p1 = 0.0, p2 = 0.0, p3 = 0.0, p4 = 0.0;
+#pragma unroll
+  for (int ig = 0; ig < NG; ++ig) {
+    const double g1 = ch.gamma[ig], g2 = g1 * g1;
+    const double w1 = wsrc[ch.chan[ig * NZ]] * ch.kz[0], w4 = wsrc[ch.chan[ig * NZ + 1]] * ch.kz[1];
+    p0 += w1 + w4;
+    p1 += g1 * (w1 + 4.0 * w4);
+    p2 += 6.0 * g2 * w4;
+    p3 += 4.0 * g2 * g1 * w4;
+    p4 += g2 * g2 * w4;
+  }
+  pc[0] = p0;
+  pc[1] = 0.5 * p1;
+  pc[2] = 0.25 * p2;
+  pc[3] = 0.125 * p3;
+  pc[4] = 0.0625 * p4;
+}
+
+__device__ __forceinline__ double rsqrt_f64(double x) {
+  double y = __builtin_amdgcn_rsq(x);
+  const double hx = 0.5 * x;
+  y = fma(y, fma(-hx * y, y, 0.5), y);
+  y = fma(y, fma(-hx * y, y, 0.5), y);
+  return y;
+}
 
 __device__ __forceinline__ void reduce_radial_from_lds(const SFParams &sf, const DeviceBatch &b,
                                                        const Fields &f, int c0, int c1, int s0) {
@@ -471,11 +529,13 @@
       const int k = ((int)threadIdx.x - 64) / (NSPEC + 1), sg = ((int)threadIdx.x - 64) % (NSPEC + 1);
       cnt[60 + k * kSegW + sg] = b.seg_start[(size_t)(c0 + k) * (NSPEC + 1) + sg] - s0;
     }
+    if (NSPEC == 1 && b.job_word_own && threadIdx.x < 20) cnt[kOwnCtl + threadIdx.x] = 0;
     double *P0 = reinterpret_cast<double *>(raw + v2_counter_offset(kCap) + kJobCtlBytes);
     for (int k = threadIdx.x; k < NSPEC * NG * NZ * v2_pcols(kCap, NSPEC); k += blockDim.x) P0[k] = 0.0;
   }
+  int *jidx = (NSPEC == 1 && b.job_word_own && b.job_count) ? reinterpret_cast<int *>(f.sp1) : nullptr;
   TA_STAMP(b, 0, 0);
-  stage<HD>(sf, ch, beta, b, f, s0, M, geom, true);
+  stage<HD>(sf, ch, beta, b, f, s0, M, geom, true, jidx);
   TA_STAMP(b, 0, 1);
   if (b.job_count && threadIdx.x == 0) {
     int *ctl = reinterpret_cast<int *>(reinterpret_cast<char *>(lds) + v2_counter_offset(kCap));
@@ -494,9 +554,19 @@
     const int64_t p = (int64_t)s0 + item;
     int base, n;
     int pslot = item;
+    unsigned own = 0u;
+    int kbit = 0;
+    uint32_t sij = 0u;
+    int ic = 0, rij = 0;
     if constexpr (kJob) {
       const int *cstart = reinterpret_cast<const int *>(reinterpret_cast<const char *>(lds) + v2_counter_offset(kCap)) + 40;
       const int ci = job_centre((uint32_t)mask0);
+      if (NSPEC == 1 && jidx) {
+        ic = c0 + ci;
+        const int j = jidx[item];
+        sij = (uint32_t)ic + (uint32_t)j;
+        rij = j < ic ? 1 : 0;
+      }
       base = cstart[ci];
       n = cstart[ci + 1] - base;
       {
@@ -535,6 +605,12 @@
         const double d2 = fma(ex, ex, fma(ey, ey, fma(ez, ez, sf.eps)));
         const double u = kProbe(flags, 30) ? 0.5 : d2 * sf.inv_ac2;
         if (!(u < 1.0)) return;
+        if constexpr (kJob && NSPEC == 1) {
+          if (jidx) {
+            const int kk = jidx[q];
+            own |= (triangle_owner_rank(sij + (uint32_t)kk) == rij + (kk < ic ? 1 : 0) ? 1u : 0u) << kbit;
+          }
+        }
         const double2 bih = f.ih[kProbe(flags, 29) ? (int)threadIdx.x : q];
         const double cth = (ra2 + bzr.y - d2) * 0.5 * inv_ra * bih.x;
         const double common = Ha * bih.y * hd_value<HD>(sf, ch, beta, u);
@@ -577,6 +653,7 @@
       while (m) {
         const int k = __ffs((int)m) - 1;
         m &= m - 1;
+        kbit = k;
         triple(k0 + k);
       }
     } else {
@@ -622,6 +699,7 @@
           else
             b.part4[(size_t)(sp * sf.n_ang + c) * b.n_pairs + p] = v;
         }
+    return own;
   };
 
   int item = threadIdx.x;
@@ -655,14 +733,23 @@
       if (threadIdx.x == 0) b.job_count[blockIdx.x] = n_jobs;
       for (int slot = threadIdx.x; slot < n_jobs; slot += blockDim.x) b.job_word[jbase + slot] = jl.word[slot];
       TA_STAMP(b, 0, 4);
+      uint32_t swept[4] = {0u, 0u, 0u, 0u};
+      unsigned owned[4] = {0u, 0u, 0u, 0u};
       if (!(flags & (1 << 27)))
         for (int r = 0; r * (int)blockDim.x < n_jobs; ++r) {
           const int slot = job_slot(r, threadIdx.x, blockDim.x);
           if (slot < n_jobs) {
             const uint32_t jw = jl.word[slot];
-            run_item(job_item(jw), true, jw, nullptr, P, std::true_type{});
+            const unsigned o = run_item(job_item(jw), true, jw, nullptr, P, std::true_type{});
+            if (r < 4) {
+              swept[r] = jw;
+              owned[r] = o;
+            }
           }
         }
+      if (jidx)
+        make_owned_jobs(jl.hist + kOwnCtl, jl.hist + kOwnCtl + 20, swept, owned, b.job_word_own + jbase,
+                        b.job_count_own + blockIdx.x);
       __syncthreads();
       TA_STAMP(b, 0, 5);
       if (flags & 4) {
@@ -716,6 +803,7 @@
     }
   } else {
     if (b.job_count && threadIdx.x == 0) b.job_count[blockIdx.x] = -1;
+    if (jidx && threadIdx.x == 0) b.job_count_own[blockIdx.x] = -1;
     for (int it = threadIdx.x; it < M; it += blockDim.x) run_item(it, false, 0ull, nullptr, nullptr, std::false_type{});
   }
 
@@ -739,11 +827,13 @@
   }
 }
 
-template <int NSPEC, int NG, int NZ, int HD, bool DEFZ, int CAP, int WPE = (DEFZ ? (NSPEC <= 2 ? 5 : 4) : 0)>
+template <int NSPEC, int NG, int NZ, int HD, bool DEFZ, int CAP, int WPE = (DEFZ ? (NSPEC <= 2 ? 5 : 4) : 0),
+          bool TRI = false>
 __global__ __launch_bounds__(kBlock)
     __attribute__((amdgpu_waves_per_eu(WPE > 0 ? WPE : 1, 8))) void backward_v2_kernel(SFParams sf, AngChunk ch,
                                                              DeviceBatch b, int flags) {
   static_assert(!DEFZ || NZ == 2, "DEFZ needs the two-zeta grid");
+  static_assert(!TRI || (NSPEC == 1 && DEFZ && HD > 0), "the triangle build is one-element, default grid, Hd series");
   const int first = flags & 1;
   if (b.n_blk_dev && (int)blockIdx.x >= *b.n_blk_dev) return;
   stagger(flags);
@@ -797,10 +887,125 @@
       rtab[ci * kRTab + rem] = b.dEdG[(size_t)i * sf.ndim + radial_term2(b.species[i], sb) * sf.n_rad + c];
     }
   }
+  double2 *pn01 = reinterpret_cast<double2 *>(rtab + kMaxCentersPerBlock * kRTab), *pn23 = pn01 + kCap;
+  double *pn4 = reinterpret_cast<double *>(pn23 + kCap);
+  if constexpr (TRI) {
+    for (int item = threadIdx.x; item < M; item += blockDim.x) {
+      double pc[5];
+      defz_coeffs<NG, NZ>(ch, b.dEdG + (size_t)b.pair_j[s0 + item] * sf.ndim + sf.n_radial_dim, pc);
+      pn01[item] = make_double2(pc[0], pc[1]);
+      pn23[item] = make_double2(pc[2], pc[3]);
+      pn4[item] = pc[4];
+    }
+  }
   TA_STAMP(b, 1, 0);
   stage<HD>(sf, ch, beta, b, f, s0, M);
   TA_STAMP(b, 1, 1);
   const int nel = sf.n_elements;
+
+  auto run_tri = [&](int item, bool have_mask, unsigned long long mask0, auto is_job) {
+    constexpr bool kJob = decltype(is_job)::value;
+    const int64_t p = (int64_t)s0 + item;
+    int i, base, n;
+    if constexpr (kJob) {
+      const int ci = job_centre((uint32_t)mask0);
+      i = c0 + ci;
+      base = cstart[ci];
+      n = cstart[ci + 1] - base;
+    } else {
+      i = b.pair_i[p];
+      base = b.pair_start[i] - s0;
+      n = pair_stop_of(b, i) - b.pair_start[i];
+    }
+    const int a = item - base;
+    const double2 axy = f.xy[item], azr = f.zr[item], aih = f.ih[item], ags = f.gs[item];
+    const double ax = axy.x, ay = axy.y, az = azr.x;
+    const double A = azr.y, inv_ra = aih.x, Ha = aih.y, La = ags.x;
+    const double inv_A = inv_ra * inv_ra;
+    double pi_[5], pj_[5];
+#pragma unroll
+    for (int k = 0; k < 5; ++k) pi_[k] = pctab[5 * (i - c0) + k];
+    {
+      const double2 p01 = pn01[item], p23 = pn23[item];
+      pj_[0] = p01.x;
+      pj_[1] = p01.y;
+      pj_[2] = p23.x;
+      pj_[3] = p23.y;
+      pj_[4] = pn4[item];
+    }
+    const int ja = kJob ? 0 : b.pair_j[p];
+    double csum = 0.0, gx = 0.0, gy = 0.0, gz = 0.0;
+    auto tri = [&](int bl) {
+      bl = (int)min((unsigned)bl, (unsigned)bl - (unsigned)n);
+      const int q = base + bl;
+      if constexpr (!kJob) {
+        if (!owns_triangle(i, ja, b.pair_j[s0 + q])) return;
+      }
+      const double2 bxy = f.xy[q], bzr = f.zr[q];
+      const double bx = bxy.x, by = bxy.y, bz = bzr.x;
+      const double ex = bx - ax, ey = by - ay, ez = bz - az;
+      const double D = fma(ex, ex, fma(ey, ey, fma(ez, ez, sf.eps)));
+      const double u = D * sf.inv_ac2;
+      if (!(u < 1.0)) return;
+      const double2 bih = f.ih[q], bgs = f.gs[q], p01 = pn01[q], p23 = pn23[q];
+      const double pk4 = pn4[q];
+      const double B = bzr.y, inv_rb = bih.x, Hb = bih.y, Lb = bgs.x;
+      double Hd, dHd;
+      hd_eval<HD>(sf, ch, beta, u, Hd, dHd);
+      const double inv_d = rsqrt_f64(D);
+      const double inv_ab = inv_ra * inv_rb, inv_ad = inv_ra * inv_d, inv_bd = inv_rb * inv_d;
+      const double wi = (A + B - D) * inv_ab, wj = (A + D - B) * inv_ad, wk = (B + D - A) * inv_bd;
+      const double Si = fma(fma(fma(fma(pi_[4], wi, pi_[3]), wi, pi_[2]), wi, pi_[1]), wi, pi_[0]);
+      const double Pi = fma(fma(fma(4.0 * pi_[4], wi, 3.0 * pi_[3]), wi, 2.0 * pi_[2]), wi, pi_[1]);
+      const double Sj = fma(fma(fma(fma(pj_[4], wj, pj_[3]), wj, pj_[2]), wj, pj_[1]), wj, pj_[0]);
+      const double Pj = fma(fma(fma(4.0 * pj_[4], wj, 3.0 * pj_[3]), wj, 2.0 * pj_[2]), wj, pj_[1]);
+      const double Sk = fma(fma(fma(fma(pk4, wk, p23.y), wk, p23.x), wk, p01.y), wk, p01.x);
+      const double Pk = fma(fma(fma(4.0 * pk4, wk, 3.0 * p23.y), wk, 2.0 * p23.x), wk, p01.y);
+      const double HH = Ha * Hb, T = HH * Hd;
+      const double sum = Si + Sj + Sk;
+      const double TS = T * sum;
+      const double X = (sum * HH) * (sf.two_inv_ac2 * dHd);
+      const double Yi = Pi * T, Yj = Pj * T, Yk = Pk * T;
+      const double Ywi = Yi * wi, Ywj = Yj * wj, Ywk = Yk * wk;
+      const double inv_D = inv_d * inv_d;
+      const double ZD = (Ywj + Ywk) * inv_D;
+      const double Yjd = Yj * inv_ad, Ykd = Yk * inv_bd;
+      const double ca = fma(TS, La, fma(-(Ywi + Ywj), inv_A, fma(4.0, Yjd, X - ZD)));
+      const double cb = fma(TS, Lb, fma(-(Ywi + Ywk), inv_rb * inv_rb, fma(4.0, Ykd, X - ZD)));
+      const double Q = fma(2.0, fma(Yi, inv_ab, -(Yjd + Ykd)), ZD - X);
+      csum += ca;
+      gx = fma(Q, bx, gx);
+      gy = fma(Q, by, gy);
+      gz = fma(Q, bz, gz);
+      atomicAdd(&gacc[q], fma(cb, bx, Q * ax));
+      atomicAdd(&gacc[kCap + q], fma(cb, by, Q * ay));
+      atomicAdd(&gacc[2 * kCap + q], fma(cb, bz, Q * az));
+    };
+    if constexpr (kJob) {
+      const uint32_t jw = (uint32_t)mask0;
+      unsigned m = (flags & (1 << 24)) ? 0u : jw >> 16;
+      const int k0 = a + 1 + 16 * (int)((jw >> 8) & 3u);
+      while (m) {
+        const int k = __ffs((int)m) - 1;
+        m &= m - 1;
+        tri(k0 + k);
+      }
+    } else {
+      const int smax = (Ha != 0.0) ? n / 2 : 0;
+      for (int sc = 1; sc <= smax; sc += 64) {
+        unsigned long long mask = have_mask ? mask0 : b.masks[(size_t)(sc >> 6) * b.n_pairs + p];
+        if (flags & (1 << 24)) mask = 0ull;
+        while (mask) {
+          const int k = __ffsll((long long)mask) - 1;
+          mask &= mask - 1;
+          tri(a + sc + k);
+        }
+      }
+    }
+    atomicAdd(&gacc[item], fma(csum, ax, gx));
+    atomicAdd(&gacc[kCap + item], fma(csum, ay, gy));
+    atomicAdd(&gacc[2 * kCap + item], fma(csum, az, gz));
+  };
 
   auto run_item = [&](int item, bool have_mask, unsigned long long mask0, auto is_job) {
     constexpr bool kJob = decltype(is_job)::value;
@@ -971,21 +1176,26 @@
       n_own = pair_stop_of(b, i) - b.pair_start[i];
     }
     const bool one_pass = M <= (int)blockDim.x && !__syncthreads_or(active && (n_own >> 1) > 64);
-    const int n_jobs = (one_pass && b.job_count) ? b.job_count[blockIdx.x] : -1;
+    const int32_t *jcount = TRI ? b.job_count_own : b.job_count;
+    const uint32_t *jword = TRI ? b.job_word_own : b.job_word;
+    const int n_jobs = (one_pass && jcount) ? jcount[blockIdx.x] : -1;
     if (n_jobs >= 0) {
       const size_t jbase = (size_t)blockIdx.x * b.job_stride;
       uint32_t jws[4];
 #pragma unroll
       for (int r = 0; r < 4; ++r) {
         const int slot = job_slot(r, threadIdx.x, blockDim.x);
-        jws[r] = slot < n_jobs ? b.job_word[jbase + slot] : 0u;
+        jws[r] = slot < n_jobs ? jword[jbase + slot] : 0u;
       }
       TA_STAMP(b, 1, 2);
 #pragma unroll
       for (int r = 0; r < 4; ++r) {
         if (r * (int)blockDim.x >= n_jobs) break;
         const int slot = job_slot(r, threadIdx.x, blockDim.x);
-        if (slot < n_jobs) run_item(job_item(jws[r]), true, jws[r], std::true_type{});
+        if (slot < n_jobs) {
+          if constexpr (TRI) run_tri(job_item(jws[r]), true, jws[r], std::true_type{});
+          else run_item(job_item(jws[r]), true, jws[r], std::true_type{});
+        }
       }
       TA_STAMP(b, 1, 3);
     } else if (one_pass) {
@@ -995,9 +1205,15 @@
         const int smax = (f.ih[item].y != 0.0) ? n_own / 2 : 0;
         if (smax > 0) mask = b.masks[p];
       }
-      if (active) run_item(item, true, mask, std::false_type{});
+      if (active) {
+        if constexpr (TRI) run_tri(item, true, mask, std::false_type{});
+        else run_item(item, true, mask, std::false_type{});
+      }
     } else {
-      for (int it = threadIdx.x; it < M; it += blockDim.x) run_item(it, false, 0ull, std::false_type{});
+      for (int it = threadIdx.x; it < M; it += blockDim.x) {
+        if constexpr (TRI) run_tri(it, false, 0ull, std::false_type{});
+        else run_item(it, false, 0ull, std::false_type{});
+      }
     }
   }
   __syncthreads();
@@ -1080,9 +1296,31 @@
     hipLaunchKernelGGL((g4_forward_v2_kernel<NSPEC, NG, NZ, 0, false, 0>), grid, block, lds, s, sf, ch, b, geom);
 }
 template <int NSPEC, int NG, int NZ>
-void bwd_t(const SFParams &sf, const AngChunk &ch, const DeviceBatch &b, int first, hipStream_t s) {
+void bwd_t(const SFParams &sf, const AngChunk &ch, const DeviceBatch &b, int first, bool tri, int &variant,
+           hipStream_t s) {
   const dim3 grid((unsigned)b.n_blk), block((unsigned)(b.cap < kBlock ? b.cap : kBlock));
   const size_t lds = v2_lds_bytes(true, b.cap);
+  variant = 1;
+  if constexpr (NZ == 2 && NSPEC == 1) {
+    if (tri && (ch.n_hd == 12 || ch.n_hd == 16) && ch.zeta_int[0] == 1 && ch.zeta_int[1] == 4) {
+      const size_t lds_t = v2_lds_bytes(true, b.cap, 0, 0, true);
+      variant = 2;
+      static const int force = getenv("TA_BWD_WPE") ? atoi(getenv("TA_BWD_WPE")) : 0;
+      if (ch.n_hd == 12 && b.cap == kCapMin && force == 4)
+        hipLaunchKernelGGL((backward_v2_kernel<1, NG, NZ, 12, true, kCapMin, 4, true>), grid, block, lds_t, s, sf, ch,
+                           b, first);
+      else if (ch.n_hd == 12 && b.cap == kCapMin)
+        hipLaunchKernelGGL((backward_v2_kernel<1, NG, NZ, 12, true, kCapMin, 5, true>), grid, block, lds_t, s, sf, ch,
+                           b, first);
+      else if (ch.n_hd == 12)
+        hipLaunchKernelGGL((backward_v2_kernel<1, NG, NZ, 12, true, 0, 5, true>), grid, block, lds_t, s, sf, ch, b,
+                           first);
+      else
+        hipLaunchKernelGGL((backward_v2_kernel<1, NG, NZ, 16, true, 0, 5, true>), grid, block, lds_t, s, sf, ch, b,
+                           first);
+      return;
+    }
+  }
   if constexpr (NZ == 2) {
     if (ch.n_hd == 12 && ch.zeta_int[0] == 1 && ch.zeta_int[1] == 4) {
       if (b.cap == kCapMin) {
@@ -1114,12 +1352,12 @@
 
 }
 
-size_t v2_lds_bytes(bool backward, int cap, int n_local, int nspec) {
+size_t v2_lds_bytes(bool backward, int cap, int n_local, int nspec, bool triangles) {
   if (!backward && n_local > 0)
     return v2_counter_offset(cap) + kJobCtlBytes + (size_t)n_local * v2_pcols(cap, nspec) * sizeof(double);
   if (backward)
     return (size_t)cap * kNF * sizeof(double) + cap + 3 * (size_t)cap * sizeof(double) +
-           kMaxCentersPerBlock * (5 + kRTab) * sizeof(double);
+           kMaxCentersPerBlock * (5 + kRTab) * sizeof(double) + (triangles ? 5 * (size_t)cap * sizeof(double) : 0);
   return (size_t)cap * kNF * sizeof(double) + 3 * (size_t)(2 * cap + kRingPad) * sizeof(float) + cap;
 }
 int v2_job_stride(int cap) { return v2_max_jobs(cap); }
@@ -1177,12 +1415,14 @@
   TA_DISPATCH_V2(fwd_t, sf, ch, b, geom, s);
 }
 
-void launch_backward_v2(const SFParams &sf, const AngChunk &ch, int ng, int nz, bool first,
-                        const DeviceBatch &b, hipStream_t s) {
-  if (b.n_blk == 0) return;
+int launch_backward_v2(const SFParams &sf, const AngChunk &ch, int ng, int nz, bool first, bool triangles,
+                       const DeviceBatch &b, hipStream_t s) {
+  if (b.n_blk == 0) return 0;
   const int nspec = sf.n_elements;
   const int f = (first ? 1 : 0) | stagger_bits(b, "TA_STAGGER_BWD");
-  TA_DISPATCH_V2(bwd_t, sf, ch, b, f, s);
-}
-
-}
+  int variant = 0;
+  TA_DISPATCH_V2(bwd_t, sf, ch, b, f, triangles, variant, s);
+  return variant;
+}
+
+}
diff --git a/tensoralloy_amd/engine.py b/tensoralloy_amd/engine.py
--- a/tensoralloy_amd/engine.py
+++ b/tensoralloy_amd/engine.py
@@ -313,6 +313,19 @@
         self._check(self._lib.ta_count_contributing_triples(self._handle, C.byref(n)))
         return int(n.value)
 
+    def count_owned_triangles(self) -> int:
+        n = C.c_int64(0)
+        self._check(self._lib.ta_count_owned_triangles(self._handle, C.byref(n)))
+        return int(n.value)
+
+    def set_triangles(self, on: bool):
+        self._check(self._lib.ta_set_triangles(self._handle, 1 if on else 0))
+
+    def backward_variant(self) -> int:
+        v = C.c_int32(0)
+        self._check(self._lib.ta_backward_variant(self._handle, C.byref(v)))
+        return int(v.value)
+
     def measure_hbm_copy(self, nbytes: int = 1 << 30, reps: int = 10) -> float:
         g = C.c_double(0.0)
         self._check(self._lib.ta_measure_hbm_copy(self._handle, int(nbytes), int(reps), C.byref(g)))
```

After: 36.95 million, median of 6. 1.04x the previous value.
